# musket-ml/segmentation_training_pipeline

Hardware: AMD Instinct MI355X
Metric: images/sec U-Net/ResNet34 512x512 bs16 training step (higher is better)
Workload: dtype bf16; 1 GPU; U-Net/ResNet34 512x512x3 1-class, batch 16 per GPU, BCE+Dice, Adam, on-device augment S1 (BASELINE.json configs[1]); global_batch=16, parallelism=dp1, hipgraph=True

## Files before the change

### include/stp_hip.h

```cpp
#ifndef STP_HIP_H
#define STP_HIP_H

#include <stddef.h>
#include <stdint.h>

#ifdef __cplusplus
extern "C" {
#endif

#define STP_OK 0
#define STP_E_BADARG (-1)
#define STP_E_LAUNCH (-2)
#define STP_E_WORKSPACE (-3)

#define STP_F32 0
#define STP_BF16 1
#define STP_F16 3

#define STP_SRC_DIRECT 0
#define STP_SRC_NEAREST2X 1
#define STP_SRC_ZEROINS2X 2

int stp_abi_version(void);
int stp_storage_dtype(void);
// ... 3 lines not shown
  const void* src1;
  const void* weight;
  const float* bias;
  const void* residual;
  void* dst0;
  void* dst1;
  int32_t N, Hs0, Ws0, Hv, Wv, C0, C1;
  int32_t src0_mode;
  int32_t KH, KW, stride, pad;
  int32_t Ho, Wo, Cout, Cd0;
  int32_t accumulate0, accumulate1, relu;
  int32_t dtype;
  int32_t tile;
  int32_t stats_tiles;
  float* stats_partial;
  const void* bnb_x;
  const float* bnb_mean;
  const float* bnb_rstd;
  const float* bnb_gamma;
  const float* bnb_beta;
  int32_t bnb_relu;
  int32_t dst_sum2x2;
  int32_t stats_slots;
  const float* src_bn_mean;
  const float* src_bn_rstd;
  const float* src_bn_gamma;
  const float* src_bn_beta;
  int32_t src_bn_relu;
  const void* weight_up;
  const void* fold_src;
  const void* fold_weight;
  int32_t fold_C;
  float* stats_group_out;
  uint32_t* stats_group_counters;
  int32_t stats_group;
  int32_t s2d_dgrad;
} stp_conv_params;
int stp_conv2d_stats_group_for(const stp_conv_params* p);
size_t stp_conv2d_stats_group_counters(const stp_conv_params* p, int32_t G);
int stp_conv2d_fold_ok(const stp_conv_params* p);

int stp_conv2d(const stp_conv_params* p, void* stream);
int stp_weight_prepare_upcollapse(const float* master, void* weight_up, int32_t Cout, int32_t C0, int32_t C1, int32_t dtype,
                                  void* stream);
size_t stp_weight_prepare_upcollapse_desc_bytes(void);
int stp_weight_prepare_upcollapse_batched(const void* desc_dev, int32_t nlayers, int32_t dtype, void* stream);
int stp_weight_prepare_upcollapse_bwd_batched(const void* desc_dev, int32_t nlayers, int32_t dtype, void* stream);
size_t stp_conv2d_stats_floats(const stp_conv_params* p);
int stp_conv2d_tile_for(const stp_conv_params* p);
int stp_conv2d_sc_eligible(const stp_conv_params* p);
int stp_conv2d_sc_stats_tiles(const stp_conv_params* p);
int stp_conv2d_sc(const stp_conv_params* p, void* stream);
int stp_conv2d_scw_eligible(const stp_conv_params* p);
int stp_conv2d_scw_stats_tiles(const stp_conv_params* p);
int stp_conv2d_scw(const stp_conv_params* p, void* stream);
int stp_conv2d_scn_eligible(const stp_conv_params* p);
int stp_conv2d_scn_stats_tiles(const stp_conv_params* p);
int stp_conv2d_scn(const stp_conv_params* p, void* stream);
int stp_conv2d_s64_eligible(const stp_conv_params* p);
int stp_conv2d_s64_stats_tiles(const stp_conv_params* p);
int stp_conv2d_s64(const stp_conv_params* p, void* stream);
int stp_conv2d_stem_eligible(const stp_conv_params* p);
int stp_conv2d_stem(const stp_conv_params* p, void* stream);
int stp_conv2d_halo_variant(const stp_conv_params* p);
int stp_conv2d_halo_tiles(const stp_conv_params* p, int variant);
int stp_conv2d_halo(const stp_conv_params* p, int variant, void* stream);

typedef struct stp_wgrad_params {
  const void* src0;
  const void* src1;
  const void* dy;
  float* dw;
  int32_t N, Hs0, Ws0, Hv, Wv, C0, C1, src0_mode;
  int32_t KH, KW, stride, pad;
  int32_t Ho, Wo, Cout;
  int32_t accumulate;
  int32_t dtype;
  int32_t splits;
  const float* src_bn_mean;
  const float* src_bn_rstd;
  const float* src_bn_gamma;
  const float* src_bn_beta;
  int32_t src_bn_relu;
} stp_wgrad_params;

size_t stp_conv2d_wgrad_workspace_bytes(const stp_wgrad_params* p);
int stp_conv2d_wgrad(const stp_wgrad_params* p, void* workspace, size_t workspace_bytes, void* stream);
int stp_conv2d_wgrad_partial(const stp_wgrad_params* p, void* workspace, size_t workspace_bytes, int32_t variant, void* stream);
int stp_conv2d_wgrad_reduce(const stp_wgrad_params* p, const void* workspace, int32_t variant, void* stream);
int stp_wgrad_sc_eligible(const stp_wgrad_params* p);
int stp_wgrad_sc_slabs(const stp_wgrad_params* p);
int stp_wgrad_sc_partial(const stp_wgrad_params* p, void* workspace, void* stream);
int stp_conv2d_wgrad_kernel_id(const stp_wgrad_params* p);

int stp_wgrad_group_class(const stp_wgrad_params* p);
size_t stp_wgrad_group_table_bytes(const stp_wgrad_params* const* layers, int32_t n);
size_t stp_wgrad_group_workspace_bytes(const stp_wgrad_params* const* layers, int32_t n);
int stp_wgrad_group_build(const stp_wgrad_params* const* layers, int32_t n, void* host_table, size_t table_bytes);
int stp_wgrad_group_partial(const void* host_table, const void* dev_table, void* workspace, size_t workspace_bytes, void* stream);
int stp_wgrad_group_reduce(const void* host_table, const void* dev_table, const void* workspace, void* stream);

int stp_weight_prepare(const float* master, void* fwd, void* bwd, int32_t Cout, int32_t KH, int32_t KW,
                       int32_t Cin, int32_t KWp, int32_t Cinp, int32_t CoutB, int32_t dtype, void* stream);
size_t stp_weight_prepare_desc_bytes(void);
int64_t stp_weight_prepare_desc_fill(void* desc_host, int32_t index, int64_t start, const float* master, void* fwd, void* bwd,
                                     int32_t Cout, int32_t KH, int32_t KW, int32_t Cin, int32_t KWp, int32_t Cinp, int32_t CoutB);
int stp_weight_prepare_batched(const void* desc_dev, int32_t nlayers, int64_t total, int32_t dtype, void* stream);
int stp_weight_grad_unpad(const float* padded, float* grad, int32_t Cout, int32_t KH, int32_t KW,
                          int32_t Cin, int32_t KWp, int32_t Cinp, int32_t accumulate, void* stream);
int stp_stem_beta_grad(const float* padded_dw, const float* master, float* dbeta, int32_t Cout, int32_t KH,
                       int32_t KW, int32_t Cin, int32_t KWp, int32_t Cinp, int32_t one_ch, void* stream);

#define STP_U8 2
size_t stp_bn_workspace_bytes(int32_t C);
int stp_bn_apply_slots(const void* x, void* y, int32_t dtype, int64_t rows, int32_t C, const int64_t* slots, int32_t nslots,
                       float eps, float momentum, float* mean, float* rstd, float* moving_mean, float* moving_var,
                       const float* gamma, const float* beta, int32_t relu, void* stream);
int stp_bn_backward_slots(const void* x, const void* g, void* dx, int32_t dtype, int64_t rows, int32_t C, const float* mean,
                          const float* rstd, const float* gamma, const int64_t* slots, int32_t nslots, float* dgamma,
                          float* dbeta, int32_t accumulate_dx, void* stream);
int stp_zero_bytes(void* p, int64_t bytes, void* stream);
int stp_bn_backward_fused(const void* x, const void* g, void* dx, int32_t dtype, int64_t rows, int32_t C,
                          const float* mean, const float* rstd, const float* gamma, const float* partial, int32_t tiles,
                          float* dgamma, float* dbeta, int32_t accumulate_dx, void* workspace, size_t workspace_bytes,
                          void* stream);
int stp_bn_finalize_apply_ok(int32_t dtype, int64_t rows, int32_t C, int32_t tiles);
int stp_bn_finalize_apply(const float* partial, int32_t tiles, const void* x, void* y, int32_t dtype, int64_t rows, int32_t C,
                          float eps, float momentum, float* mean, float* rstd, float* moving_mean, float* moving_var,
                          const float* gamma, const float* beta, int32_t relu, void* stream);
int stp_bn_backward_fused_add(const void* x, const void* g, void* dx, const void* dadd, int32_t dtype, int64_t rows, int32_t C,
                              const float* mean, const float* rstd, const float* gamma, const float* partial, int32_t tiles,
                              float* dgamma, float* dbeta, int32_t accumulate_dx, void* workspace, size_t workspace_bytes,
                              void* stream);
int stp_bn_stats(const void* x, int32_t xdtype, int64_t rows, int32_t C, float eps, float momentum,
                 float* mean, float* rstd, float* moving_mean, float* moving_var,
                 void* workspace, size_t workspace_bytes, void* stream);
int stp_bn_finalize(const float* partial, int32_t tiles, int64_t rows, int32_t C, float eps, float momentum,
                    float* mean, float* rstd, float* moving_mean, float* moving_var, void* stream);
int stp_bn_apply(const void* x, int32_t xdtype, void* y, int32_t ydtype, int64_t rows, int32_t C, int32_t Cy,
                 const float* mean, const float* rstd, const float* gamma, const float* beta,
                 int32_t relu, float pad_value, void* stream);
int stp_bn_inference(const void* x, int32_t xdtype, void* y, int32_t ydtype, int64_t rows, int32_t C, int32_t Cy,
                     const float* moving_mean, const float* moving_var, float eps,
                     const float* gamma, const float* beta, int32_t relu, float pad_value, void* stream);
int stp_bn_backward(const void* x, const void* dy, void* dx, int32_t dtype, int64_t rows, int32_t C,
                    const float* mean, const float* rstd, const float* gamma, const float* beta,
                    float* dgamma, float* dbeta, int32_t relu, int32_t accumulate_dx,
                    void* workspace, size_t workspace_bytes, void* stream);

int stp_maxpool3x3s2(const void* x, void* y, uint8_t* idx, int32_t N, int32_t H, int32_t W, int32_t C,
                     int32_t dtype, void* stream);
int stp_maxpool3x3s2_bwd(const uint8_t* idx, const void* dy, void* dx, int32_t N, int32_t H, int32_t W, int32_t C,
                         int32_t dtype, int32_t accumulate, void* stream);
int stp_bn_apply_maxpool3x3s2(const void* x, void* yb, void* y, uint8_t* idx, int32_t N, int32_t H, int32_t W, int32_t C, int32_t dtype,
                              const float* mean, const float* rstd, const float* gamma, const float* beta, int32_t relu, void* stream);
int stp_maxpool3x3s2_bwd_bn_tiles(int32_t N, int32_t H, int32_t W, int32_t C, int32_t dtype);
int stp_maxpool3x3s2_bwd_bn(const uint8_t* idx, const void* dy, void* dx, int32_t N, int32_t H, int32_t W, int32_t C, int32_t dtype,
                            int32_t accumulate, const void* bn_x, const float* mean, const float* rstd, const float* gamma,
                            const float* beta, int32_t relu, float* partial, void* stream);
int stp_maxpool2x2(const void* x, void* y, uint8_t* idx, int32_t N, int32_t H, int32_t W, int32_t C, int32_t dtype, void* stream);
int stp_maxpool2x2_bwd(const uint8_t* idx, const void* dy, void* dx, int32_t N, int32_t H, int32_t W, int32_t C, int32_t dtype,
                       int32_t accumulate, void* stream);
size_t stp_avgpool_workspace_bytes(int32_t N, int32_t H, int32_t W, int32_t C, int32_t k);
int stp_avgpool(const void* x, void* y, int32_t N, int32_t H, int32_t W, int32_t C, int32_t k, int32_t dtype, void* workspace,
                size_t workspace_bytes, void* stream);
int stp_avgpool_bwd(const void* dy, void* dx, int32_t N, int32_t H, int32_t W, int32_t C, int32_t k, int32_t dtype,
                    int32_t accumulate, void* stream);
int stp_avgpool_pyramid_ok(int32_t N, int32_t H, int32_t W, int32_t C, int32_t k0, int32_t k1, int32_t k2, int32_t k3, int32_t dtype);
size_t stp_avgpool_pyramid_workspace_bytes(int32_t N, int32_t H, int32_t W, int32_t C, int32_t k0, int32_t dtype);
int stp_avgpool_pyramid(const void* x, void* y0, void* y1, void* y2, void* y3, int32_t k0, int32_t k1, int32_t k2, int32_t k3, int32_t N,
                        int32_t H, int32_t W, int32_t C, int32_t dtype, void* workspace, size_t workspace_bytes, void* stream);
int stp_avgpool_pyramid_bwd(const void* dy0, const void* dy1, const void* dy2, const void* dy3, int32_t k0, int32_t k1, int32_t k2, int32_t k3,
                            void* dx, int32_t N, int32_t H, int32_t W, int32_t C, int32_t dtype, int32_t accumulate, void* stream);
int stp_maxpool_k(const void* x, void* y, int32_t* idx, int32_t N, int32_t H, int32_t W, int32_t C, int32_t k, int32_t dtype, void* stream);
int stp_maxpool_k_bwd(const int32_t* idx, const void* dy, void* dx, int32_t N, int32_t H, int32_t W, int32_t C, int32_t k, int32_t dtype,
                      int32_t accumulate, void* stream);
int stp_relu_bwd(const void* y, void* dy, int64_t count, int32_t dtype, void* stream);

int stp_upsample2x_bwd(const void* dy, void* dx, int32_t N, int32_t H, int32_t W, int32_t C, int32_t ldy,
                       int32_t dtype, int32_t accumulate, void* stream);
int stp_tapsum_fwd(const void* z, void* y, const float* bias, int32_t N, int32_t H, int32_t W, int32_t Cout, int32_t Zc, int32_t Cy, int32_t dtype,
                   void* stream);
int stp_tapsum_bwd(const void* dy, void* dz, int32_t N, int32_t H, int32_t W, int32_t Cout, int32_t Cdy, int32_t Cdz, int32_t dtype, void* stream);
int stp_scatter2x_bwd(const void* t, void* dx, int32_t N, int32_t H, int32_t W, int32_t C, int32_t dtype, int32_t accumulate, void* stream);
int stp_scatter2x_bwd_bn_tiles(int32_t N, int32_t H, int32_t W, int32_t C, int32_t dtype);
int stp_scatter2x_bwd_bn(const void* t, void* dx, int32_t N, int32_t H, int32_t W, int32_t C, int32_t dtype, int32_t accumulate,
                         const void* bn_x, const float* mean, const float* rstd, const float* gamma, const float* beta, int32_t relu,
                         float* partial, void* stream);
int stp_upsample2x_bwd_bn_tiles(int32_t N, int32_t H, int32_t W, int32_t C, int32_t ldy, int32_t dtype);
int stp_upsample2x_bwd_bn(const void* dy, void* dx, int32_t N, int32_t H, int32_t W, int32_t C, int32_t ldy, int32_t dtype,
                          int32_t accumulate, const void* bn_x, const float* mean, const float* rstd, const float* gamma,
                          const float* beta, int32_t relu, float* partial, void* stream);
int stp_upsample2x_add(void* x, const void* m, int32_t N, int32_t H, int32_t W, int32_t C, int32_t dtype, void* stream);
int stp_resize_bilinear(const void* x, void* y, int32_t N, int32_t H, int32_t W, int32_t C, int32_t factor, int32_t ldo,
                        int32_t coff, int32_t dtype, void* stream);
size_t stp_resize_bilinear_bwd_workspace_bytes(int32_t N, int32_t H, int32_t W, int32_t C, int32_t factor);
int stp_resize_bilinear_bwd(const void* dy, void* dx, int32_t N, int32_t H, int32_t W, int32_t C, int32_t factor, int32_t ldo,
                            int32_t coff, int32_t dtype, int32_t accumulate, void* workspace, size_t workspace_bytes, void* stream);
int stp_resize_nearest(const void* x, void* y, int32_t N, int32_t H, int32_t W, int32_t C, int32_t factor, int32_t ldo, int32_t coff,
                       int32_t dtype, void* stream);
int stp_resize_nearest_bwd(const void* dy, void* dx, int32_t N, int32_t H, int32_t W, int32_t C, int32_t factor, int32_t ldo, int32_t coff,
                           int32_t dtype, int32_t accumulate, void* stream);

int stp_channel_sum(const void* x, int32_t dtype, int64_t rows, int32_t C, float* out, int32_t accumulate,
                    void* workspace, size_t workspace_bytes, void* stream);
int stp_add_inplace(void* dst, const void* src, int64_t count, int32_t dtype, void* stream);

size_t stp_loss_workspace_bytes(void);
int stp_sigmoid_bce_dice(const void* logits, const uint8_t* target, int64_t count, int32_t dtype,
                         float w_bce, float w_dice, float* scalars, void* dlogits, int32_t dl_channels,
                         float grad_scale, void* workspace, size_t workspace_bytes, void* stream);
int stp_sigmoid_loss_ex(const void* logits, const uint8_t* target, int64_t count, int32_t dtype, const float* weights5,
                        float* scalars, void* dlogits, int32_t dl_channels, float grad_scale, void* workspace,
                        size_t workspace_bytes, void* stream);
size_t stp_lovasz_workspace_bytes(int64_t count, int32_t images);
int stp_lovasz_hinge(const void* logits, const uint8_t* target, int32_t images, int64_t per_image, int32_t dtype, float weight,
                     float* scalars, void* dlogits, int32_t dl_channels, void* workspace, size_t workspace_bytes, void* stream);
int stp_sigmoid_loss_bias_grad(const void* workspace, int64_t count, float* dbias, int32_t accumulate, void* stream);
int stp_sigmoid(const void* logits, float* probs, int64_t count, int32_t dtype, void* stream);
int stp_sigmoid_multilabel_loss(const void* logits, const uint8_t* target, int64_t pixels, int32_t classes, int32_t ldc,
                                int32_t dtype, const float* weights5, float* scalars, void* dlogits, int32_t dl_channels,
                                float grad_scale, void* workspace, size_t workspace_bytes, void* stream);
int stp_sigmoid_multilabel_bias_grad(const void* workspace, int64_t pixels, int32_t classes, float* dbias, int32_t accumulate,
                                     void* stream);
int stp_softmax_cce_dice(const void* logits, const uint8_t* target, int64_t pixels, int32_t classes, int32_t ldc,
                         int32_t dtype, float w_cce, float w_dice, float* scalars, void* dlogits, int32_t dl_channels,
                         float grad_scale, void* workspace, size_t workspace_bytes, void* stream);
int stp_softmax_loss_ex(const void* logits, const uint8_t* target, int64_t pixels, int32_t classes, int32_t ldc,
                        int32_t dtype, const float* weights5, float* scalars, void* dlogits, int32_t dl_channels,
                        float grad_scale, void* workspace, size_t workspace_bytes, void* stream);
int stp_softmax_loss_masked(const void* logits, const uint8_t* target, int64_t pixels, int32_t classes, int32_t ldc,
// ... 188 lines not shown
```

### segmentation_training_pipeline_amd/_lib.py

```python
import ctypes as C
import os

HERE = os.path.dirname(os.path.abspath(__file__))
LIB_PATH = os.environ.get("STP_LIB") or os.path.join(HERE, "libstp_hip.so")

LIB_F16_PATH = os.environ.get("STP_LIB_F16") or os.path.join(HERE, "libstp_hip_f16.so")

F32, BF16, U8, F16 = 0, 1, 2, 3
SRC_DIRECT, SRC_NEAREST2X, SRC_ZEROINS2X = 0, 1, 2
LOVASZ_SOFTMAX_CHUNK = 4096

vp, i32, i64, f32, sz = C.c_void_p, C.c_int32, C.c_int64, C.c_float, C.c_size_t


class StpError(RuntimeError):
    pass


class ConvParams(C.Structure):
    _fields_ = [("src0", vp), ("src1", vp), ("weight", vp), ("bias", vp), ("residual", vp), ("dst0", vp), ("dst1", vp),
                ("N", i32), ("Hs0", i32), ("Ws0", i32), ("Hv", i32), ("Wv", i32), ("C0", i32), ("C1", i32),
                ("src0_mode", i32), ("KH", i32), ("KW", i32), ("stride", i32), ("pad", i32),
                ("Ho", i32), ("Wo", i32), ("Cout", i32), ("Cd0", i32),
                ("accumulate0", i32), ("accumulate1", i32), ("relu", i32), ("dtype", i32), ("tile", i32),
                ("stats_tiles", i32), ("stats_partial", vp),
                ("bnb_x", vp), ("bnb_mean", vp), ("bnb_rstd", vp), ("bnb_gamma", vp), ("bnb_beta", vp), ("bnb_relu", i32),
                ("dst_sum2x2", i32), ("stats_slots", i32),
                ("src_bn_mean", vp), ("src_bn_rstd", vp), ("src_bn_gamma", vp), ("src_bn_beta", vp), ("src_bn_relu", i32),
                ("weight_up", vp), ("fold_src", vp), ("fold_weight", vp), ("fold_C", i32),
                ("stats_group_out", vp), ("stats_group_counters", vp), ("stats_group", i32), ("s2d_dgrad", i32)]


class WgradParams(C.Structure):
    _fields_ = [("src0", vp), ("src1", vp), ("dy", vp), ("dw", vp),
                ("N", i32), ("Hs0", i32), ("Ws0", i32), ("Hv", i32), ("Wv", i32), ("C0", i32), ("C1", i32),
                ("src0_mode", i32), ("KH", i32), ("KW", i32), ("stride", i32), ("pad", i32),
                ("Ho", i32), ("Wo", i32), ("Cout", i32), ("accumulate", i32), ("dtype", i32), ("splits", i32),
                ("src_bn_mean", vp), ("src_bn_rstd", vp), ("src_bn_gamma", vp), ("src_bn_beta", vp), ("src_bn_relu", i32)]


SIGNATURES = {
    "stp_abi_version": (i32, []),
    "stp_storage_dtype": (i32, []),
    "stp_conv2d": (i32, [C.POINTER(ConvParams), vp]),
    "stp_weight_prepare_upcollapse": (i32, [vp, vp, i32, i32, i32, i32, vp]),
    "stp_weight_prepare_upcollapse_desc_bytes": (sz, []),
    "stp_weight_prepare_upcollapse_batched": (i32, [vp, i32, i32, vp]),
    "stp_weight_prepare_upcollapse_bwd_batched": (i32, [vp, i32, i32, vp]),
    "stp_conv2d_fold_ok": (i32, [C.POINTER(ConvParams)]),
    "stp_conv2d_stats_floats": (sz, [C.POINTER(ConvParams)]),
    "stp_conv2d_stats_group_for": (i32, [C.POINTER(ConvParams)]),
    "stp_conv2d_stats_group_counters": (sz, [C.POINTER(ConvParams), i32]),
    "stp_conv2d_tile_for": (i32, [C.POINTER(ConvParams)]),
    "stp_conv2d_sc_eligible": (i32, [C.POINTER(ConvParams)]),
    "stp_conv2d_sc": (i32, [C.POINTER(ConvParams), vp]),
    "stp_conv2d_sc_stats_tiles": (i32, [C.POINTER(ConvParams)]),
    "stp_conv2d_scw": (i32, [C.POINTER(ConvParams), vp]),
    "stp_conv2d_scw_eligible": (i32, [C.POINTER(ConvParams)]),
    "stp_conv2d_scw_stats_tiles": (i32, [C.POINTER(ConvParams)]),
    "stp_conv2d_scn": (i32, [C.POINTER(ConvParams), vp]),
    "stp_conv2d_scn_eligible": (i32, [C.POINTER(ConvParams)]),
    "stp_conv2d_scn_stats_tiles": (i32, [C.POINTER(ConvParams)]),
    "stp_conv2d_s64": (i32, [C.POINTER(ConvParams), vp]),
    "stp_conv2d_s64_eligible": (i32, [C.POINTER(ConvParams)]),
    "stp_conv2d_s64_stats_tiles": (i32, [C.POINTER(ConvParams)]),
    "stp_conv2d_pw_eligible": (i32, [C.POINTER(ConvParams)]),
    "stp_conv2d_pw_cols": (i32, [C.POINTER(ConvParams)]),
    "stp_conv2d_pw": (i32, [C.POINTER(ConvParams), vp]),
    "stp_conv2d_stem_eligible": (i32, [C.POINTER(ConvParams)]),
    "stp_conv2d_stem": (i32, [C.POINTER(ConvParams), vp]),
    "stp_conv2d_halo_variant": (i32, [C.POINTER(ConvParams)]),
    "stp_conv2d_halo_tiles": (i32, [C.POINTER(ConvParams), i32]),
    "stp_conv2d_halo": (i32, [C.POINTER(ConvParams), i32, vp]),
    "stp_conv2d_wgrad_workspace_bytes": (sz, [C.POINTER(WgradParams)]),
    "stp_conv2d_wgrad": (i32, [C.POINTER(WgradParams), vp, sz, vp]),
    "stp_conv2d_wgrad_partial": (i32, [C.POINTER(WgradParams), vp, sz, i32, vp]),
    "stp_conv2d_wgrad_reduce": (i32, [C.POINTER(WgradParams), vp, i32, vp]),
    "stp_wgrad_reduce_desc_bytes": (sz, []),
    "stp_wgrad_reduce_desc_fill": (i64, [vp, i32, C.POINTER(WgradParams), vp]),
    "stp_wgrad_reduce_batched": (i32, [vp, i32, i64, vp]),
    "stp_wgrad_sc_eligible": (i32, [C.POINTER(WgradParams)]),
    "stp_wgrad_sc_slabs": (i32, [C.POINTER(WgradParams)]),
    "stp_wgrad_sc_partial": (i32, [C.POINTER(WgradParams), vp, vp]),
    "stp_conv2d_wgrad_kernel_id": (i32, [C.POINTER(WgradParams)]),
    "stp_wgrad_group_class": (i32, [C.POINTER(WgradParams)]),
    "stp_wgrad_group_table_bytes": (sz, [vp, i32]),
    "stp_wgrad_group_workspace_bytes": (sz, [vp, i32]),
    "stp_wgrad_group_build": (i32, [vp, i32, vp, sz]),
    "stp_wgrad_group_partial": (i32, [vp, vp, vp, sz, vp]),
    "stp_wgrad_group_reduce": (i32, [vp, vp, vp, vp]),
    "stp_weight_prepare": (i32, [vp, vp, vp, i32, i32, i32, i32, i32, i32, i32, i32, vp]),
    "stp_weight_prepare_desc_bytes": (sz, []),
    "stp_weight_prepare_desc_fill": (i64, [vp, i32, i64, vp, vp, vp, i32, i32, i32, i32, i32, i32, i32]),
    "stp_weight_prepare_batched": (i32, [vp, i32, i64, i32, vp]),
    "stp_weight_grad_unpad": (i32, [vp, vp, i32, i32, i32, i32, i32, i32, i32, vp]),
    "stp_stem_beta_grad": (i32, [vp, vp, vp, i32, i32, i32, i32, i32, i32, i32, vp]),
    "stp_bn_workspace_bytes": (sz, [i32]),
    "stp_bn_stats": (i32, [vp, i32, i64, i32, f32, f32, vp, vp, vp, vp, vp, sz, vp]),
    "stp_bn_finalize": (i32, [vp, i32, i64, i32, f32, f32, vp, vp, vp, vp, vp]),
    "stp_bn_apply": (i32, [vp, i32, vp, i32, i64, i32, i32, vp, vp, vp, vp, i32, f32, vp]),
    "stp_bn_inference": (i32, [vp, i32, vp, i32, i64, i32, i32, vp, vp, f32, vp, vp, i32, f32, vp]),
    "stp_bn_backward": (i32, [vp, vp, vp, i32, i64, i32, vp, vp, vp, vp, vp, vp, i32, i32, vp, sz, vp]),
    "stp_bn_apply_slots": (i32, [vp, vp, i32, i64, i32, vp, i32, f32, f32, vp, vp, vp, vp, vp, vp, i32, vp]),
    "stp_bn_backward_slots": (i32, [vp, vp, vp, i32, i64, i32, vp, vp, vp, vp, i32, vp, vp, i32, vp]),
    "stp_zero_bytes": (i32, [vp, i64, vp]),
    "stp_bn_backward_fused": (i32, [vp, vp, vp, i32, i64, i32, vp, vp, vp, vp, i32, vp, vp, i32, vp, sz, vp]),
    "stp_bn_finalize_apply_ok": (i32, [i32, i64, i32, i32]),
    "stp_bn_finalize_apply": (i32, [vp, i32, vp, vp, i32, i64, i32, f32, f32, vp, vp, vp, vp, vp, vp, i32, vp]),
    "stp_bn_backward_fused_add": (i32, [vp, vp, vp, vp, i32, i64, i32, vp, vp, vp, vp, i32, vp, vp, i32, vp, sz, vp]),
    "stp_maxpool3x3s2": (i32, [vp, vp, vp, i32, i32, i32, i32, i32, vp]),
    "stp_maxpool3x3s2_bwd": (i32, [vp, vp, vp, i32, i32, i32, i32, i32, i32, vp]),
    "stp_bn_apply_maxpool3x3s2": (i32, [vp, vp, vp, vp, i32, i32, i32, i32, i32, vp, vp, vp, vp, i32, vp]),
    "stp_maxpool3x3s2_bwd_bn_tiles": (i32, [i32, i32, i32, i32, i32]),
    "stp_maxpool3x3s2_bwd_bn": (i32, [vp, vp, vp, i32, i32, i32, i32, i32, i32, vp, vp, vp, vp, vp, i32, vp, vp]),
    "stp_maxpool2x2": (i32, [vp, vp, vp, i32, i32, i32, i32, i32, vp]),
    "stp_maxpool2x2_bwd": (i32, [vp, vp, vp, i32, i32, i32, i32, i32, i32, vp]),
    "stp_avgpool_workspace_bytes": (sz, [i32, i32, i32, i32, i32]),
    "stp_avgpool": (i32, [vp, vp, i32, i32, i32, i32, i32, i32, vp, sz, vp]),
    "stp_avgpool_bwd": (i32, [vp, vp, i32, i32, i32, i32, i32, i32, i32, vp]),
    "stp_avgpool_pyramid_ok": (i32, [i32, i32, i32, i32, i32, i32, i32, i32, i32]),
    "stp_avgpool_pyramid_workspace_bytes": (sz, [i32, i32, i32, i32, i32, i32]),
    "stp_avgpool_pyramid": (i32, [vp, vp, vp, vp, vp, i32, i32, i32, i32, i32, i32, i32, i32, i32, vp, sz, vp]),
    "stp_avgpool_pyramid_bwd": (i32, [vp, vp, vp, vp, i32, i32, i32, i32, vp, i32, i32, i32, i32, i32, i32, vp]),
    "stp_maxpool_k": (i32, [vp, vp, vp, i32, i32, i32, i32, i32, i32, vp]),
    "stp_maxpool_k_bwd": (i32, [vp, vp, vp, i32, i32, i32, i32, i32, i32, i32, vp]),
    "stp_relu_bwd": (i32, [vp, vp, i64, i32, vp]),
    "stp_upsample2x_bwd": (i32, [vp, vp, i32, i32, i32, i32, i32, i32, i32, vp]),
    "stp_tapsum_fwd": (i32, [vp, vp, vp, i32, i32, i32, i32, i32, i32, i32, vp]),
    "stp_tapsum_bwd": (i32, [vp, vp, i32, i32, i32, i32, i32, i32, i32, vp]),
    "stp_scatter2x_bwd": (i32, [vp, vp, i32, i32, i32, i32, i32, i32, vp]),
    "stp_scatter2x_bwd_bn_tiles": (i32, [i32, i32, i32, i32, i32]),
    "stp_scatter2x_bwd_bn": (i32, [vp, vp, i32, i32, i32, i32, i32, i32, vp, vp, vp, vp, vp, i32, vp, vp]),
    "stp_upsample2x_bwd_bn_tiles": (i32, [i32, i32, i32, i32, i32, i32]),
    "stp_upsample2x_bwd_bn": (i32, [vp, vp, i32, i32, i32, i32, i32, i32, i32, vp, vp, vp, vp, vp, i32, vp, vp]),
    "stp_upsample2x_add": (i32, [vp, vp, i32, i32, i32, i32, i32, vp]),
    "stp_resize_bilinear": (i32, [vp, vp, i32, i32, i32, i32, i32, i32, i32, i32, vp]),
    "stp_upsample_sum": (i32, [vp, vp, vp, vp, i32, i32, i32, i32, vp, i32, i32, i32, i32, i32, vp]),
    "stp_copy_cols_f32": (i32, [vp, i32, vp, i32, i32, i32, i32, vp]),
    "stp_resize_bilinear_bwd_workspace_bytes": (sz, [i32, i32, i32, i32, i32]),
    "stp_resize_bilinear_bwd": (i32, [vp, vp, i32, i32, i32, i32, i32, i32, i32, i32, i32, vp, sz, vp]),
    "stp_resize_nearest": (i32, [vp, vp, i32, i32, i32, i32, i32, i32, i32, i32, vp]),
    "stp_resize_nearest_bwd": (i32, [vp, vp, i32, i32, i32, i32, i32, i32, i32, i32, i32, vp]),
    "stp_channel_sum": (i32, [vp, i32, i64, i32, vp, i32, vp, sz, vp]),
    "stp_add_inplace": (i32, [vp, vp, i64, i32, vp]),
    "stp_loss_workspace_bytes": (sz, []),
    "stp_sigmoid_bce_dice": (i32, [vp, vp, i64, i32, f32, f32, vp, vp, i32, f32, vp, sz, vp]),
    "stp_sigmoid_loss_ex": (i32, [vp, vp, i64, i32, vp, vp, vp, i32, f32, vp, sz, vp]),
    "stp_sigmoid_loss_bias_grad": (i32, [vp, i64, vp, i32, vp]),
    "stp_sigmoid_multilabel_loss": (i32, [vp, vp, i64, i32, i32, i32, vp, vp, vp, i32, f32, vp, sz, vp]),
    "stp_sigmoid_multilabel_bias_grad": (i32, [vp, i64, i32, vp, i32, vp]),
    "stp_softmax_loss_ex": (i32, [vp, vp, i64, i32, i32, i32, vp, vp, vp, i32, f32, vp, sz, vp]),
    "stp_softmax_loss_masked": (i32, [vp, vp, i64, i32, i32, i32, vp, vp, vp, i32, f32, vp, sz, i32, vp, vp]),
    "stp_lovasz_workspace_bytes": (sz, [i64, i32]),
    "stp_lovasz_hinge": (i32, [vp, vp, i32, i64, i32, f32, vp, vp, i32, vp, sz, vp]),
    "stp_lovasz_softmax_workspace_bytes": (sz, [i64, i32]),
    "stp_lovasz_softmax": (i32, [vp, vp, i64, i32, i32, i32, f32, vp, vp, i32, f32, i32, vp, sz, vp]),
    "stp_sigmoid": (i32, [vp, vp, i64, i32, vp]),
    "stp_softmax_cce_dice": (i32, [vp, vp, i64, i32, i32, i32, f32, f32, vp, vp, i32, f32, vp, sz, vp]),
    "stp_softmax_cce_dice_up_ok": (i32, [i32, i32, i32]),
    "stp_softmax_cce_dice_up_corner_bytes": (sz, [i32, i32, i32, i32]),
    "stp_softmax_cce_dice_up": (i32, [vp, vp, i32, i32, i32, i32, i32, i32, i32, f32, f32, vp, vp, i32, f32, vp, vp, vp, sz, vp, sz, vp]),
    "stp_softmax": (i32, [vp, vp, i64, i32, i32, i32, vp]),
    "stp_class_confusion_workspace_bytes": (sz, [i32]),
    "stp_class_confusion": (i32, [vp, vp, i64, i32, i32, i32, vp, vp, sz, vp]),
    "stp_class_confusion_ignore": (i32, [vp, vp, i64, i32, i32, i32, vp, vp, sz, i32, vp]),
    "stp_class_confusion_up_ok": (i32, [i32, i32, i32]),
    "stp_class_confusion_up": (i32, [vp, vp, i32, i32, i32, i32, i32, i32, i32, vp, vp, sz, vp]),
    "stp_adam": (i32, [vp, vp, vp, vp, i64, vp, f32, f32, f32, vp, vp, vp, f32, vp]),
    "stp_sgd": (i32, [vp, vp, vp, i64, vp, f32, i32, vp, vp, f32, vp]),
    "stp_rmsprop": (i32, [vp, vp, vp, i64, vp, f32, f32, vp, vp, f32, vp]),
    "stp_nadam": (i32, [vp, vp, vp, vp, i64, vp, f32, f32, f32, f32, vp, vp, vp, vp, f32, vp]),
    "stp_grad_global_scale": (i32, [vp, i64, f32, f32, vp, vp, sz, vp]),
    "stp_scale_by_device": (i32, [vp, i64, i32, vp, vp, vp]),
    "stp_grad_global_scale_dls": (i32, [vp, i64, f32, f32, vp, vp, vp, sz, vp]),
    "stp_dwconv": (i32, [vp, vp, vp, i32, i32, i32, i32, i32, i32, i32, i32, i32, i32, i32, i32, vp]),
    "stp_dwconv_dgrad": (i32, [vp, vp, vp, i32, i32, i32, i32, i32, i32, i32, i32, i32, i32, i32, i32, i32, vp]),
    "stp_dwconv_wgrad_workspace_bytes": (sz, [i32, i32]),
    "stp_dwconv_wgrad": (i32, [vp, vp, vp, i32, i32, i32, i32, i32, i32, i32, i32, i32, i32, i32, i32, i32, vp, sz, vp]),
    "stp_resize_bilinear_ac": (i32, [vp, vp, i32, i32, i32, i32, i32, i32, i32, vp]),
    "stp_resize_bilinear_ac_bwd": (i32, [vp, vp, i32, i32, i32, i32, i32, i32, i32, i32, vp]),
    "stp_counter_tick": (i32, [vp, vp]),
    "stp_dropout": (i32, [vp, vp, i64, f32, vp, C.c_uint32, i32, vp]),
    "stp_dropout_spatial": (i32, [vp, vp, i32, i64, i32, f32, vp, C.c_uint32, i32, vp]),
    "stp_sigmoid_act": (i32, [vp, vp, i64, i32, i32, i32, i32, vp]),
    "stp_sigmoid_act_bwd": (i32, [vp, vp, vp, i64, i32, i32, i32, i32, vp]),
# ... 113 lines not shown
```

### segmentation_training_pipeline_amd/csrc/bn.hip

```cpp
#include "stream_ops.h"
#include <cstdlib>

__global__ __launch_bounds__(256) void bn_partial_u8_kernel(const uint8_t* __restrict__ x, int64_t rows, int C, float* partial) {
  __shared__ float rs[256 * 2];
  const int rowLanes = 256 / C;
  const int tcol = threadIdx.x % C, trow = threadIdx.x / C;
  const int64_t rowsPerBlock = (rows + gridDim.x - 1) / gridDim.x;
  const int64_t r0 = (int64_t)blockIdx.x * rowsPerBlock;
  const int64_t r1 = r0 + rowsPerBlock < rows ? r0 + rowsPerBlock : rows;
  float s = 0.f, q = 0.f;
  if (trow < rowLanes)
    for (int64_t r = r0 + trow; r < r1; r += rowLanes) {
      const float v = (float)x[r * C + tcol];
      s += v;
      q += v * v;
    }
  rs[threadIdx.x * 2] = s;
  rs[threadIdx.x * 2 + 1] = q;
  __syncthreads();
  if (trow == 0 && threadIdx.x < C) {
    float a = 0.f, b = 0.f;
    for (int t = 0; t < rowLanes; ++t) { a += rs[(t * C + tcol) * 2]; b += rs[(t * C + tcol) * 2 + 1]; }
    partial[(size_t)blockIdx.x * 2 * C + tcol] = a;
    partial[(size_t)blockIdx.x * 2 * C + C + tcol] = b;
// ... 526 lines not shown
  __syncthreads();
  const int cg = C / V;
  const int64_t total = rows * cg;
  const int64_t stride = (int64_t)gridDim.x * 256;
  if (stride % cg == 0) {
    const int c = (int)(((int64_t)blockIdx.x * 256 + threadIdx.x) % cg) * V;
    float mu[V], rs[V], sc[V], sh[V], k1[V], k2[V];
#pragma unroll
    for (int e = 0; e < V; ++e) {
      mu[e] = ss[c + e]; rs[e] = ss[C + c + e]; sc[e] = ss[2 * C + c + e]; sh[e] = ss[3 * C + c + e];
      k1[e] = ss[4 * C + c + e]; k2[e] = ss[5 * C + c + e];
    }
    auto one = [&](int64_t i, const float (&xv)[V], float (&g)[V], const float (&d)[V]) {
      float o[V];
#pragma unroll
      for (int e = 0; e < V; ++e) {
        if (!bn_act_on(bn_affine(xv[e], sc[e], sh[e]), relu)) g[e] = 0.f;
        const float xh = (xv[e] - mu[e]) * rs[e];
        o[e] = sc[e] * (g[e] - k1[e] - xh * k2[e]);
        if (accumulate) o[e] += d[e];
      }
      stv<T, V>(dx + i * V, o);
    };
    int64_t i = (int64_t)blockIdx.x * 256 + threadIdx.x;
    for (; i + stride < total; i += 2 * stride) {
      float x0[V], g0[V], d0[V], x1[V], g1[V], d1[V];
      ldv<T, V>(x + i * V, x0);
      ldv<T, V>(x + (i + stride) * V, x1);
      ldv<T, V>(dy + i * V, g0);
      ldv<T, V>(dy + (i + stride) * V, g1);
      if (accumulate) { ldv<T, V>(dadd + i * V, d0); ldv<T, V>(dadd + (i + stride) * V, d1); }
      one(i, x0, g0, d0);
      one(i + stride, x1, g1, d1);
    }
    for (; i < total; i += stride) {
      float x0[V], g0[V], d0[V];
      ldv<T, V>(x + i * V, x0);
      ldv<T, V>(dy + i * V, g0);
      if (accumulate) ldv<T, V>(dadd + i * V, d0);
      one(i, x0, g0, d0);
    }
    return;
  }
  for (int64_t i = (int64_t)blockIdx.x * 256 + threadIdx.x; i < total; i += stride) {
    const int c = (int)(i % cg) * V;
    float xv[V], g[V], o[V];
    ldv<T, V>(x + i * V, xv);
    ldv<T, V>(dy + i * V, g);
#pragma unroll
    for (int e = 0; e < V; ++e) {
      if (!bn_act_on(bn_affine(xv[e], ss[2 * C + c + e], ss[3 * C + c + e]), relu)) g[e] = 0.f;
      const float xh = (xv[e] - ss[c + e]) * ss[C + c + e];
      o[e] = ss[2 * C + c + e] * (g[e] - ss[4 * C + c + e] - xh * ss[5 * C + c + e]);
    }
    if (accumulate) {
      float d[V];
      ldv<T, V>(dadd + i * V, d);
#pragma unroll
      for (int e = 0; e < V; ++e) o[e] += d[e];
    }
    stv<T, V>(dx + i * V, o);
  }
}

static int bn_bwd_apply_launch(const void* x, const void* dy, void* dx, int dtype, int64_t rows, int C, const float* mean, const float* rstd,
                               const float* gamma, const float* beta, const float* sums, int relu, int accumulate, const long long* slots, int nslots,
                               float* dgamma, float* dbeta, const void* dadd, hipStream_t s) {
  const bool v8 = dtype == STP_H16 && (C & 7) == 0;
  const size_t lds2 = 6 * (size_t)C * sizeof(float);
  const int g = grid_fixed_channels(grid_for_amortised(rows * (C / (v8 ? 8 : 4)), 8), C / (v8 ? 8 : 4));
  const float inv_rows = (float)(1.0 / (double)rows);
  return launch_tv(dtype, v8, [&](auto tv) {
    using T = typename decltype(tv)::T; constexpr int V = decltype(tv)::V;
    hipLaunchKernelGGL((bn_bwd_apply_kernel<T, V>), dim3(g), dim3(256), lds2, s, (const T*)x, (const T*)dy, (T*)dx, rows, C, mean, rstd, gamma, beta,
                       sums, inv_rows, relu, accumulate, slots, nslots, dgamma, dbeta, (const T*)dadd);
  });
}

extern "C" int stp_bn_backward(const void* x, const void* dy, void* dx, int32_t dtype, int64_t rows, int32_t C,
                               const float* mean, const float* rstd, const float* gamma, const float* beta, float* dgamma,
                               float* dbeta, int32_t relu, int32_t accumulate_dx, void* workspace, size_t workspace_bytes,
                               void* stream) {
  if (!stp_dtype_ok(dtype)) return STP_E_BADARG;
  if (!x || !dy || !dx || !mean || !rstd || !workspace || rows <= 0 || C <= 0 || (C & 3)) return STP_E_BADARG;
  if (workspace_bytes < stp_bn_workspace_bytes(C)) return STP_E_WORKSPACE;
  hipStream_t s = (hipStream_t)stream;
  const int blocks = bn_blocks(rows) > BN_MAX_BLOCKS - 1 ? BN_MAX_BLOCKS - 1 : bn_blocks(rows);
  float* partial = (float*)workspace;
  float* sums = partial + (size_t)(BN_MAX_BLOCKS - 1) * 2 * C;
  const int rc = launch_tv(dtype, dtype == STP_H16 && (C & 7) == 0, [&](auto tv) {
    using T = typename decltype(tv)::T; constexpr int V = decltype(tv)::V;
    hipLaunchKernelGGL((bn_bwd_partial_kernel<T, V>), dim3(blocks), dim3(256), 256 * 2 * V * sizeof(float), s, (const T*)x, (const T*)dy, rows, C,
                       mean, rstd, gamma, beta, relu, partial);
  });
  if (rc) return rc;
  hipLaunchKernelGGL(bn_bwd_finalize_kernel, dim3(ceil_div(C, 4)), dim3(256), 0, s, partial, blocks, C, sums, dgamma, dbeta);
  STP_LAUNCH_CHECK();
  return bn_bwd_apply_launch(x, dy, dx, dtype, rows, C, mean, rstd, gamma, beta, sums, relu, accumulate_dx, nullptr, 0, nullptr, nullptr, nullptr, s);
}

#define BNF_SLAB 64
static bool bn_fused_ok(int dtype, int64_t rows, int C, int tiles) {
  static const bool on = !(getenv("STP_BN_FUSE_FINALIZE") && atoi(getenv("STP_BN_FUSE_FINALIZE")) == 0);
  static const int maxcols = getenv("STP_BN_FUSE_MAXCOLS") ? atoi(getenv("STP_BN_FUSE_MAXCOLS")) : 128;
  return on && dtype == STP_H16 && (C % BNF_SLAB) == 0 && tiles >= 1 && tiles <= maxcols && rows >= 64;
}
static int bn_fused_chunks(int64_t rows, int C) {
  const int slabs = C / BNF_SLAB;
  int64_t want = (rows + 255) / 256;
  const int64_t lo = (2 * 256 + slabs - 1) / slabs;
  if (want < lo) want = lo;
  const int64_t hi = (rows + 31) / 32;
  if (want > hi) want = hi;
  return (int)(want < 1 ? 1 : want);
}

__device__ __forceinline__ void bnf_slab_sums(const float* __restrict__ partial, int tiles, int C, int c0, double& s, double& q) {
  const int cl = threadIdx.x >> 2, j = threadIdx.x & 3;
  const float* ps = partial + (size_t)(c0 + cl) * tiles;
  const float* pq = partial + ((size_t)C + c0 + cl) * tiles;
  s = 0.0; q = 0.0;
  if ((tiles & 3) == 0 && tiles > 128 && tiles <= 256) {
#pragma unroll
    for (int h = 0; h < 2; ++h) {
      f32x4 a[8], b[8];
#pragma unroll
      for (int u = 0; u < 8; ++u) {
        const int t = 4 * j + 16 * (u + 8 * h);
        a[u] = b[u] = f32x4{0.f, 0.f, 0.f, 0.f};
        if (t < tiles) { a[u] = *reinterpret_cast<const f32x4*>(ps + t); b[u] = *reinterpret_cast<const f32x4*>(pq + t); }
      }
#pragma unroll
      for (int u = 0; u < 8; ++u)
        if (4 * j + 16 * (u + 8 * h) < tiles) {
          s += ((double)a[u].x + (double)a[u].y) + ((double)a[u].z + (double)a[u].w);
          q += ((double)b[u].x + (double)b[u].y) + ((double)b[u].z + (double)b[u].w);
        }
    }
  } else if ((tiles & 3) == 0 && tiles <= 128) {
    f32x4 a[8], b[8];
#pragma unroll
    for (int u = 0; u < 8; ++u) {
      const int t = 4 * j + 16 * u;
      a[u] = b[u] = f32x4{0.f, 0.f, 0.f, 0.f};
      if (t < tiles) { a[u] = *reinterpret_cast<const f32x4*>(ps + t); b[u] = *reinterpret_cast<const f32x4*>(pq + t); }
    }
#pragma unroll
    for (int u = 0; u < 8; ++u)
      if (4 * j + 16 * u < tiles) {
        s += ((double)a[u].x + (double)a[u].y) + ((double)a[u].z + (double)a[u].w);
        q += ((double)b[u].x + (double)b[u].y) + ((double)b[u].z + (double)b[u].w);
      }
  } else if ((tiles & 3) == 0) {
    for (int t = 4 * j; t < tiles; t += 16) {
      const f32x4 a = *reinterpret_cast<const f32x4*>(ps + t), b = *reinterpret_cast<const f32x4*>(pq + t);
      s += ((double)a.x + (double)a.y) + ((double)a.z + (double)a.w);
      q += ((double)b.x + (double)b.y) + ((double)b.z + (double)b.w);
    }
  } else {
    for (int t = j; t < tiles; t += 4) { s += (double)ps[t]; q += (double)pq[t]; }
  }
  s += __shfl_xor(s, 1, 64); q += __shfl_xor(q, 1, 64);
  s += __shfl_xor(s, 2, 64); q += __shfl_xor(q, 2, 64);
}

__global__ __launch_bounds__(256) void bn_finalize_apply_kernel(const float* __restrict__ partial, int tiles, const bf16_t* __restrict__ x,
                                                                bf16_t* __restrict__ y, int64_t rows, int C, int chunks, double inv_rows,
                                                                double unbias, float eps, float momentum, float* mean, float* rstd,
                                                                float* mm, float* mv, const float* gamma, const float* beta, int relu) {
  __shared__ float tab[2][BNF_SLAB];
  const int slab = blockIdx.x / chunks, chunk = blockIdx.x - slab * chunks, c0 = slab * BNF_SLAB;
  const int cg = threadIdx.x & 7, r0 = threadIdx.x >> 3;
  const int64_t per = (rows + chunks - 1) / chunks, ra = (int64_t)chunk * per, rb = ra + per < rows ? ra + per : rows;
  const size_t col = (size_t)c0 + cg * 8;
  int64_t r = ra + r0;
  const bool pre = r + 96 < rb;
  u32x4 p0 = {0u, 0u, 0u, 0u}, p1 = p0, p2 = p0, p3 = p0;
  if (pre) {
    p0 = *reinterpret_cast<const u32x4*>(x + (size_t)r * C + col); p1 = *reinterpret_cast<const u32x4*>(x + (size_t)(r + 32) * C + col);
    p2 = *reinterpret_cast<const u32x4*>(x + (size_t)(r + 64) * C + col); p3 = *reinterpret_cast<const u32x4*>(x + (size_t)(r + 96) * C + col);
  }
// ... 211 lines not shown
```

### segmentation_training_pipeline_amd/csrc/conv_sc.h

```cpp
#pragma once
#include "common.h"
#include "launch.h"
#include <cstdlib>
#include <type_traits>
#include <utility>

struct ScArgs {
  const char* src;
  const char* weight;
  const float* bias;
  char* dst;
  int N, H, W, Hs, Ws, Cout, up, accumulate, relu;
  int tiles_x, tiles_y;
  FastDiv divTx, divTy;
  float* stats;
  int stat_slots;
  BnBack bnb;
  int sum2;
  uint32_t src_bytes;
  BnBack pbn;
};

template <typename T> struct ScStageBn;
template <> struct ScStageBn<float> {
// ... 6 lines not shown
    u32x4 o;
#pragma unroll
    for (int e = 0; e < 4; ++e) o[e] = __float_as_uint(bn_act(bn_affine(__uint_as_float(r[e]), sc[e], sh[e]), relu));
    return o;
  }
};
template <> struct ScStageBn<bf16_t> {
  f32x2 sc[4], sh[4];
  __device__ __forceinline__ void load(const BnBack& b, int c) {
    const BnBackCh k0 = bnback_load(b, c), k1 = bnback_load(b, c + 4);
    sc[0] = f32x2{k0.sc[0], k0.sc[1]}; sc[1] = f32x2{k0.sc[2], k0.sc[3]}; sc[2] = f32x2{k1.sc[0], k1.sc[1]}; sc[3] = f32x2{k1.sc[2], k1.sc[3]};
    sh[0] = f32x2{k0.sh[0], k0.sh[1]}; sh[1] = f32x2{k0.sh[2], k0.sh[3]}; sh[2] = f32x2{k1.sh[0], k1.sh[1]}; sh[3] = f32x2{k1.sh[2], k1.sh[3]};
  }
  __device__ __forceinline__ void load_tab(const float* tsc, const float* tsh, int c) {
#pragma unroll
    for (int e = 0; e < 4; ++e) { sc[e] = *reinterpret_cast<const f32x2*>(tsc + c + 2 * e); sh[e] = *reinterpret_cast<const f32x2*>(tsh + c + 2 * e); }
  }
  __device__ __forceinline__ u32x4 apply(const u32x4& r, int relu) const {
    u32x4 o;
#pragma unroll
    for (int e = 0; e < 4; ++e) {
      f32x2 v = {h16lo_to_f32(r[e]), h16hi_to_f32(r[e])};
      v = __builtin_elementwise_fma(v, sc[e], sh[e]);
      o[e] = pack_bf16x2(bn_act(v.x, relu), bn_act(v.y, relu));
    }
    return o;
  }
};


constexpr int SC_TH = 8, SC_TW = 32, SC_HW = SC_TW + 2, SC_HH = SC_TH + 2;

template <int... Ks, typename F>
__device__ __forceinline__ void sc_unroll_seq(std::integer_sequence<int, Ks...>, F&& f) { (f(std::integral_constant<int, Ks>{}), ...); }
template <int N, typename F>
__device__ __forceinline__ void sc_unroll(F&& f) { sc_unroll_seq(std::make_integer_sequence<int, N>{}, f); }
#ifndef SC_RING
#define SC_RING 8
#endif

#ifndef SC_WPE_SMALL
#define SC_WPE_SMALL 4
#endif

static inline bool sc_stream_on() {
  static const bool on = !(getenv("STP_SC_STREAM") && atoi(getenv("STP_SC_STREAM")) == 0);
  return on;
}
static inline int sc_stream_blocks(int dtype, int cin, int cout, int ntiles) {
  const int per_cu = cout <= 16 ? (dtype == STP_H16 && cin <= 16 ? SC_WPE_SMALL : 3) : 2;
  const int64_t b = (int64_t)stp_cu_count() * per_cu;
  return (int)(b < ntiles ? b : ntiles);
}


struct ScWgArgs {
  const char* src;
  const char* dy;
  float* slabs;
  int N, H, W, Hs, Ws, Cout, up;
  int tiles_x, tiles_y, ntiles;
  int ctot, coff;
  uint32_t src_bytes, dy_bytes;
  BnBack pbn;
};

constexpr int ST_HH = (SC_TH - 1) * 2 + 7, ST_HW = 70, ST_WROW = 464, ST_HALO = ST_HH * ST_HW * 8, ST_WBYTES = 64 * ST_WROW;

struct StemArgs {
  const char* src;
  const char* weight;
  char* dst;
  int N, H, W, Ho, Wo, tiles_x, tiles_y;
  FastDiv divTx, divTy;
  float* stats;
  uint32_t src_bytes;
};

bool stem_lean_serves(int N, int H, int W);
int stem_lean_blocks(int ntiles);
int stem_lean_launch(const StemArgs& a, hipStream_t s);
bool stem_wg_lean_serves(int N, int H, int W, int Ho, int Wo);
int stem_wg_lean_blocks(int N, int Ho, int Wo);
int stem_wg_lean_launch(const void* src, const void* dy, float* slabs, int N, int H, int W, int Ho, int Wo, hipStream_t s);

int sc_lean_launch(const ScArgs& a, int cin, int dtype, hipStream_t s);
int sc_wg_lean_launch(const ScWgArgs& a, int cin, int cout, int dtype, int blocks, hipStream_t s);
```

### segmentation_training_pipeline_amd/csrc/conv_sc_lean.hip

```cpp
#include "conv_sc.h"

enum { SCL_STATS = 0, SCL_BNB = 1, SCL_BNB_SUM2 = 2, SCL_HEAD = 3 };

struct TileC { int n, y0, x0; bool interior; };

__device__ __forceinline__ f32x2 scl_unpack(uint32_t w) { return f32x2{h16lo_to_f32(w), h16hi_to_f32(w)}; }

template <int TM>
__device__ __forceinline__ void scl_store(char* p, const u32x2 (&o)[TM]) {
  if constexpr (TM == 2) *reinterpret_cast<u32x4*>(p) = u32x4{o[0].x, o[0].y, o[1].x, o[1].y};
  else *reinterpret_cast<u32x2*>(p) = o[0];
}

template <int CIN, int TM, int EPI, bool PBN, bool UP>
__global__ __launch_bounds__(256, (TM == 1 ? (CIN <= 16 ? SC_WPE_SMALL : 3) : 2)) void conv_sc_lean_kernel(const ScArgs a) {
  typedef bf16_t T;
  constexpr int SZ = 2, VEC = 8, KC = 32, K = 9 * CIN, NCH = (K + KC - 1) / KC, VPP = CIN / VEC, PIXB = CIN * SZ;
  constexpr int HH = UP ? SC_TH / 2 + 2 : SC_HH, HW = UP ? SC_TW / 2 + 2 : SC_HW;
  constexpr int NV = HH * HW * VPP, NPASS = (NV + 255) / 256, BUF = NPASS * 4096;
  constexpr bool PART = (K % KC) != 0;
  constexpr int COUT = EPI == SCL_HEAD ? 1 : TM * 16;
  constexpr int CB = COUT * SZ;
  static_assert(EPI != SCL_HEAD || TM == 1, "head: one output channel");
  static_assert(!PBN || EPI == SCL_STATS || EPI == SCL_HEAD, "producer BatchNormalization: forward only");
// ... 768 lines not shown
        for (int f = 0; f < 4; ++f) { asm volatile("" : "+v"(fb[c & 1][f][0])); asm volatile("" : "+v"(fb[c & 1][f][1])); }
#pragma unroll
        for (int f = 0; f < 4; ++f) {
          const u32x4 vb = {fb[c & 1][f][0].x, fb[c & 1][f][0].y, fb[c & 1][f][1].x, fb[c & 1][f][1].y};
#pragma unroll
          for (int i = 0; i < TM; ++i) acc[i][f] = mfma16_16x16x32(fa[c & 1][i], vb, acc[i][f]);
        }
      });
      ba += cur ? (uint32_t)(-STL_BUF) : (uint32_t)STL_BUF;

#if defined(STP_STEM_WAIT_LATE)
      __builtin_amdgcn_s_waitcnt(0x0f70);
      asm volatile("" ::: "memory");
#endif
      char* ob = a.dst + (((size_t)t.n * a.Ho + t.y0) * a.Wo + t.x0) * (COUT * 2);
      const bool st = a.stats != nullptr;
      auto epilogue = [&](const bool EDGE) __attribute__((always_inline)) {
#pragma unroll
        for (int f = 0; f < 4; ++f) {
          char* of = ob + (size_t)(((f >> 1) * a.Wo + (f & 1) * 16) * (COUT * 2));
          const bool ok = !EDGE || (t.y0 + wave * 2 + (f >> 1) < a.Ho && t.x0 + (f & 1) * 16 + lr < a.Wo);
#pragma unroll
          for (int h = 0; h < 2; ++h) {
            const f32x4 v0 = acc[2 * h][f], v1 = acc[2 * h + 1][f];
            const u32x4 o = {pack_bf16x2(v0.x, v0.y), pack_bf16x2(v0.z, v0.w), pack_bf16x2(v1.x, v1.y), pack_bf16x2(v1.z, v1.w)};
            if (ok) {
              *reinterpret_cast<u32x4*>(of + so + h * 64) = o;
              if (st) {
#pragma unroll
                for (int u = 0; u < 2; ++u) {
                  const f32x2 s0 = scl_unpack(o[2 * u]), s1 = scl_unpack(o[2 * u + 1]);
                  const f32x4 sv = {s0.x, s0.y, s1.x, s1.y};
                  ss[2 * h + u] += sv;
                  qq[2 * h + u] += sv * sv;
                }
              }
            }
          }
        }
      };
      if (t.interior) epilogue(false); else epilogue(true);
    }
  }
  if (a.stats) {
    __builtin_amdgcn_s_waitcnt(0x0f70);
#pragma unroll
    for (int i = 0; i < TM; ++i)
#pragma unroll
      for (int e = 0; e < 4; ++e) {
        const float sv = row_sum16_to_lane15(ss[i][e]), qv = row_sum16_to_lane15(qq[i][e]);
        if (lr == 15) {
          const int cl = (i >> 1) * 32 + lg * 8 + (i & 1) * 4 + e;
          red[(wave * COUT + cl) * 2] = sv;
          red[(wave * COUT + cl) * 2 + 1] = qv;
        }
      }
    lds_barrier();
    if (tid < COUT) {
      float sv = 0.f, qv = 0.f;
#pragma unroll
      for (int w = 0; w < 4; ++w) { sv += red[(w * COUT + tid) * 2]; qv += red[(w * COUT + tid) * 2 + 1]; }
      a.stats[(size_t)tid * gridDim.x + blockIdx.x] = sv;
      a.stats[((size_t)COUT + tid) * gridDim.x + blockIdx.x] = qv;
    }
  }
}

bool stem_lean_serves(int N, int H, int W) {
  static const bool on = !(getenv("STP_STEM_LEAN") && atoi(getenv("STP_STEM_LEAN")) == 0);
  return on && !(W & 1) && (uint64_t)N * H * W * 8 < 0x80000000ull;
}
int stem_lean_blocks(int ntiles) {
  const int64_t b = (int64_t)stp_cu_count() * 2;
  return (int)(b < ntiles ? b : ntiles);
}
int stem_lean_launch(const StemArgs& a, hipStream_t s) {
  if (!stem_lean_serves(a.N, a.H, a.W) || !a.src_bytes) return 1;
  return stp_launch_lds(conv_stem_lean_kernel, dim3(stem_lean_blocks(a.N * a.tiles_x * a.tiles_y)), dim3(256), STL_LDS, s, a);
}

constexpr int SWG_TH = 4, SWG_PH = 2 * (SWG_TH - 1) + 7;
constexpr int SWG_NVX = SWG_PH * STL_VPR, SWG_NPX = (SWG_NVX + 255) / 256;
constexpr int SWG_NVD = SWG_TH * SC_TW * 8, SWG_NPD = (SWG_NVD + 255) / 256;
constexpr int SWG_XBUF = SWG_NPX * 4096, SWG_BUF = SWG_XBUF + SWG_NPD * 4096;

struct StemWgArgs {
  const char* src;
  const char* dy;
  float* slabs;
  int N, H, W, Ho, Wo, tiles_x, tiles_y, ntiles;
  uint32_t src_bytes, dy_bytes;
};

__global__ __launch_bounds__(256, 2) void conv_stem_wgrad_lean_kernel(const StemWgArgs a) {
  constexpr int COUT = 64, K = 224, NF = 14;
  extern __shared__ __attribute__((aligned(16))) char smem[];
  const int tid = threadIdx.x, lane = tid & 63;
  const int wave = __builtin_amdgcn_readfirstlane(tid >> 6);
  const int lr = lane & 15, lg = lane >> 4;

  int t_first, t_step, t_end;
  if ((gridDim.x & 7) == 0) {
    const int q = a.ntiles >> 3, r = a.ntiles & 7, x = blockIdx.x & 7;
    const int start = x < r ? x * (q + 1) : r * (q + 1) + (x - r) * q;
    t_first = start + (int)(blockIdx.x >> 3); t_step = (int)(gridDim.x >> 3); t_end = start + q + (x < r ? 1 : 0);
  } else {
    t_first = (int)blockIdx.x; t_step = (int)gridDim.x; t_end = a.ntiles;
  }
  f32x4 acc[NF];
#pragma unroll
  for (int f = 0; f < NF; ++f) acc[f] = f32x4{0.f, 0.f, 0.f, 0.f};

  if (t_first < t_end) {
    const __amdgpu_buffer_rsrc_t rsx = __builtin_amdgcn_make_buffer_rsrc((void*)a.src, 0, a.src_bytes, 0x00020000);
    const __amdgpu_buffer_rsrc_t rsd = __builtin_amdgcn_make_buffer_rsrc((void*)a.dy, 0, a.dy_bytes, 0x00020000);
    int hyx[SWG_NPX], pyx[SWG_NPD];
    uint32_t lox[SWG_NPX], lod[SWG_NPD];
#pragma unroll
    for (int p = 0; p < SWG_NPX; ++p) {
      const int v = p * 256 + tid, hy = v / STL_VPR, vx = v - hy * STL_VPR;
      hyx[p] = v < SWG_NVX ? (hy << 16 | vx) : -1;
      lox[p] = v < SWG_NVX ? (uint32_t)((hy * a.W + 2 * vx) * 8) : 0x80000000u;
    }
#pragma unroll
    for (int p = 0; p < SWG_NPD; ++p) {
      const int v = p * 256 + tid, pix = v >> 3, py = pix / SC_TW, px = pix % SC_TW;
      pyx[p] = v < SWG_NVD ? (py << 16 | px) : -1;
      lod[p] = v < SWG_NVD ? (uint32_t)((py * a.Wo + px) * (COUT * 2) + (v & 7) * 16) : 0x80000000u;
    }
    const uint32_t cvd = (uint32_t)(tid & 7) * 16u;
    auto decode = [&](int tile) -> TileC {
      int b = tile;
      const int tx = b % a.tiles_x; b /= a.tiles_x;
      const int ty = b % a.tiles_y;
      TileC t;
      t.n = b / a.tiles_y; t.y0 = ty * SWG_TH; t.x0 = tx * SC_TW;
      t.interior = 2 * t.y0 >= 3 && 2 * t.x0 >= 4 && 2 * t.y0 - 3 + SWG_PH <= a.H && 2 * t.x0 + 65 < a.W && t.y0 + SWG_TH <= a.Ho && t.x0 + SC_TW <= a.Wo;
      return t;
    };
    auto issue_tile = [&](const TileC& t, int bsel, bool live) {
      char* xb = smem + bsel * SWG_BUF;
      if (live && t.interior) {
        const uint32_t tbx = (uint32_t)(((t.n * a.H + 2 * t.y0 - 3) * a.W + 2 * t.x0 - 4) * 8);
        const uint32_t tbd = (uint32_t)(((t.n * a.Ho + t.y0) * a.Wo + t.x0) * (COUT * 2));
#pragma unroll
        for (int p = 0; p < SWG_NPX; ++p)
          __builtin_amdgcn_raw_ptr_buffer_load_lds(rsx, (__attribute__((address_space(3))) void*)(xb + p * 4096 + wave * 1024), 16, (int)(tbx + lox[p]), 0, 0, 0);
#pragma unroll
        for (int p = 0; p < SWG_NPD; ++p)
          __builtin_amdgcn_raw_ptr_buffer_load_lds(rsd, (__attribute__((address_space(3))) void*)(xb + SWG_XBUF + p * 4096 + wave * 1024), 16, (int)(tbd + lod[p]), 0, 0, 0);
      } else {
#pragma unroll
        for (int p = 0; p < SWG_NPX; ++p) {
          const int gy = 2 * t.y0 - 3 + (hyx[p] >> 16), gx = 2 * t.x0 - 4 + 2 * (hyx[p] & 0xffff);
          const bool ok = live && hyx[p] >= 0 && (unsigned)gy < (unsigned)a.H && (unsigned)gx < (unsigned)a.W;
          const uint32_t off = ok ? (uint32_t)(((t.n * a.H + gy) * a.W + gx) * 8) : 0x80000000u;
          __builtin_amdgcn_raw_ptr_buffer_load_lds(rsx, (__attribute__((address_space(3))) void*)(xb + p * 4096 + wave * 1024), 16, (int)off, 0, 0, 0);
        }
#pragma unroll
        for (int p = 0; p < SWG_NPD; ++p) {
          const int gy = t.y0 + (pyx[p] >> 16), gx = t.x0 + (pyx[p] & 0xffff);
          const bool ok = live && pyx[p] >= 0 && gy < a.Ho && gx < a.Wo;
          const uint32_t off = ok ? (uint32_t)(((t.n * a.Ho + gy) * a.Wo + gx) * (COUT * 2)) + cvd : 0x80000000u;
          __builtin_amdgcn_raw_ptr_buffer_load_lds(rsd, (__attribute__((address_space(3))) void*)(xb + SWG_XBUF + p * 4096 + wave * 1024), 16, (int)off, 0, 0, 0);
        }
      }
    };
    TileC tc = decode(t_first);
    issue_tile(tc, 0, true);
    const int xl = lg * 4 + (lr >> 2), qd = lr & 3;
    uint32_t aA = (uint32_t)(uintptr_t)smem + (uint32_t)(SWG_XBUF + (xl * COUT + wave * 16) * 2 + qd * 8);
    uint32_t aB = (uint32_t)(uintptr_t)smem + (uint32_t)((2 * xl + 1 + qd) * 8);

    int cur = 0;
    for (int tile = t_first; tile < t_end; tile += t_step, cur ^= 1) {
      __builtin_amdgcn_s_waitcnt(0x0f70);
      asm volatile("" ::: "memory");
      lds_barrier();
      const int next = tile + t_step;
      const bool live = next < t_end;
      if (live) tc = decode(next);
      issue_tile(tc, cur ^ 1, live);

      u32x2 fa[SWG_TH][2];
      u32x2 fb[2][2][2];
      sc_unroll<SWG_TH * 2>([&fa, aA](auto kc) {
        constexpr int k = decltype(kc)::value, r = k >> 1, hl = k & 1;
        asm volatile("ds_read_b64_tr_b16 %0, %1 offset:%2" : "=v"(fa[r][hl]) : "v"(aA), "n"((r * SC_TW + hl * 16) * COUT * 2));
      });
      auto issue_b = [&fb, aB](auto rc) {
        constexpr int pr = decltype(rc)::value;
        sc_unroll<4>([&fb, aB](auto kc) {
          constexpr int k = decltype(kc)::value, kwh = k >> 1, hl = k & 1;
          asm volatile("ds_read_b64_tr_b16 %0, %1 offset:%2" : "=v"(fb[pr & 1][kwh][hl]) : "v"(aB), "n"(pr * STL_ROW + kwh * 32 + hl * 32 * 8));
        });
      };
      issue_b(std::integral_constant<int, 0>{});
      sc_unroll<SWG_PH>([&](auto rc) {
        constexpr int pr = decltype(rc)::value;
        if constexpr (pr + 1 < SWG_PH) issue_b(std::integral_constant<int, pr + 1>{});
        asm volatile("s_waitcnt lgkmcnt(%0)" ::"n"(pr + 1 < SWG_PH ? 4 : 0) : "memory");
        if constexpr (pr == 0) {
#pragma unroll
          for (int r = 0; r < SWG_TH; ++r) { asm volatile("" : "+v"(fa[r][0])); asm volatile("" : "+v"(fa[r][1])); }
        }
#pragma unroll
        for (int kwh = 0; kwh < 2; ++kwh) { asm volatile("" : "+v"(fb[pr & 1][kwh][0])); asm volatile("" : "+v"(fb[pr & 1][kwh][1])); }
#pragma unroll
        for (int r = 0; r < SWG_TH; ++r) {
          const int kh = pr - 2 * r;
          if (kh < 0 || kh > 6) continue;
          const u32x4 va = {fa[r][0].x, fa[r][0].y, fa[r][1].x, fa[r][1].y};
#pragma unroll
          for (int kwh = 0; kwh < 2; ++kwh) {
            const u32x4 vb = {fb[pr & 1][kwh][0].x, fb[pr & 1][kwh][0].y, fb[pr & 1][kwh][1].x, fb[pr & 1][kwh][1].y};
            acc[kh * 2 + kwh] = mfma16_16x16x32(va, vb, acc[kh * 2 + kwh]);
          }
        }
      });
      const uint32_t flip = cur ? (uint32_t)(-SWG_BUF) : (uint32_t)SWG_BUF;
      aA += flip; aB += flip;
    }
  }
  float* out = a.slabs + (size_t)blockIdx.x * COUT * K;
#pragma unroll
  for (int f = 0; f < NF; ++f)
#pragma unroll
    for (int r = 0; r < 4; ++r) out[(size_t)(wave * 16 + lg * 4 + r) * K + (f >> 1) * 32 + (f & 1) * 16 + lr] = acc[f][r];
}

bool stem_wg_lean_serves(int N, int H, int W, int Ho, int Wo) {
  static const bool on = !(getenv("STP_STEM_WG_LEAN") && atoi(getenv("STP_STEM_WG_LEAN")) == 0);
  return on && !(W & 1) && (uint64_t)N * H * W * 8 < 0x80000000ull && (uint64_t)N * Ho * Wo * 128 < 0x80000000ull;
}
int stem_wg_lean_blocks(int N, int Ho, int Wo) {
  const int64_t tiles = (int64_t)N * ((Ho + SWG_TH - 1) / SWG_TH) * ((Wo + SC_TW - 1) / SC_TW), b = (int64_t)stp_cu_count() * 2;
  return (int)(b < tiles ? b : tiles);
}
int stem_wg_lean_launch(const void* src, const void* dy, float* slabs, int N, int H, int W, int Ho, int Wo, hipStream_t s) {
  StemWgArgs a;
  a.src = (const char*)src; a.dy = (const char*)dy; a.slabs = slabs;
  a.N = N; a.H = H; a.W = W; a.Ho = Ho; a.Wo = Wo;
  a.tiles_x = (Wo + SC_TW - 1) / SC_TW; a.tiles_y = (Ho + SWG_TH - 1) / SWG_TH; a.ntiles = N * a.tiles_x * a.tiles_y;
  a.src_bytes = (uint32_t)((uint64_t)N * H * W * 8); a.dy_bytes = (uint32_t)((uint64_t)N * Ho * Wo * 128);
  hipLaunchKernelGGL(conv_stem_wgrad_lean_kernel, dim3(stem_wg_lean_blocks(N, Ho, Wo)), dim3(256), 2 * SWG_BUF, s, a);
  STP_LAUNCH_CHECK();
  return STP_OK;
}
```

### segmentation_training_pipeline_amd/csrc/conv_sc_wgrad.hip

```cpp
#include "conv_sc.h"

typedef short s16x4_t __attribute__((ext_vector_type(4)));


template <typename T, int CIN, int COUT>
__global__ __launch_bounds__(256) void conv_sc_wgrad_stream_kernel(const ScWgArgs a) {
  constexpr int SZ = (int)sizeof(T);
  constexpr int VEC = Elem<T>::VEC;
  constexpr int TMo = (COUT + 15) / 16, TNi = CIN / 16;
  constexpr int PIXB = CIN * SZ, DYB = COUT * SZ;
  constexpr int HALO_BYTES = SC_HH * SC_HW * PIXB;
  static_assert(CIN % 16 == 0 && COUT % VEC == 0, "channel granularity");

  extern __shared__ __attribute__((aligned(16))) char smem[];
  const int tid = threadIdx.x, lane = tid & 63;
  const int wave = __builtin_amdgcn_readfirstlane(tid >> 6);
  const int lr = lane & 15, lg = lane >> 4;
  const int sh = a.up ? 1 : 0;

  static_assert(256 % (CIN / VEC) == 0, "a thread stages the same channel vector in every pass");
  const bool pbn = a.pbn.mean != nullptr;
  ScStageBn<T> sbn;
  if (pbn) sbn.load(a.pbn, (tid % (CIN / VEC)) * VEC);

// ... 209 lines not shown
    __syncthreads();

#pragma unroll 1
    for (int row = 0; row < SC_TH; ++row) {
      if constexpr (sizeof(T) == 2) {
        const int xl = lg * 4 + (lr >> 2), qb = (lr & 3) * 8;
        u32x4 fa[TMo];
#pragma unroll
        for (int i = 0; i < TMo; ++i) {
          const char* p = dyt + ((row * SC_TW + xl) * COUT + i * 16) * SZ + qb;
          const s16x4_t lo = __builtin_amdgcn_ds_read_tr16_b64_v4i16((__attribute__((address_space(3))) s16x4_t*)p);
          const s16x4_t hi = __builtin_amdgcn_ds_read_tr16_b64_v4i16((__attribute__((address_space(3))) s16x4_t*)(p + 16 * DYB));
          const u32x2 l2 = __builtin_bit_cast(u32x2, lo), h2 = __builtin_bit_cast(u32x2, hi);
          fa[i] = u32x4{l2.x, l2.y, h2.x, h2.y};
        }
#pragma unroll
        for (int t = 0; t < 3; ++t) {
          const int tap = wave + 4 * t;
          if (tap < 9) {
            const int kh = tap / 3, kw = tap - kh * 3;
#pragma unroll
            for (int j = 0; j < TNi; ++j) {
              const char* p = halo + (((row + kh) * SC_HW + xl + kw) * CIN + j * 16) * SZ + qb;
              const s16x4_t lo = __builtin_amdgcn_ds_read_tr16_b64_v4i16((__attribute__((address_space(3))) s16x4_t*)p);
              const s16x4_t hi = __builtin_amdgcn_ds_read_tr16_b64_v4i16((__attribute__((address_space(3))) s16x4_t*)(p + 16 * PIXB));
              const u32x2 l2 = __builtin_bit_cast(u32x2, lo), h2 = __builtin_bit_cast(u32x2, hi);
              const u32x4 fb = u32x4{l2.x, l2.y, h2.x, h2.y};
#pragma unroll
              for (int i = 0; i < TMo; ++i)
                acc[t][i][j] = mfma16_16x16x32(fa[i], fb, acc[t][i][j]);
            }
          }
        }
      } else {
#pragma unroll
        for (int s = 0; s < 8; ++s) {
          const int x = s * 4 + lg;
          float fa[TMo];
#pragma unroll
          for (int i = 0; i < TMo; ++i) fa[i] = *reinterpret_cast<const float*>(dyt + ((row * SC_TW + x) * COUT + i * 16 + lr) * SZ);
#pragma unroll
          for (int t = 0; t < 3; ++t) {
            const int tap = wave + 4 * t;
            if (tap < 9) {
              const int kh = tap / 3, kw = tap - kh * 3;
#pragma unroll
              for (int j = 0; j < TNi; ++j) {
                const float fb = *reinterpret_cast<const float*>(halo + (((row + kh) * SC_HW + x + kw) * CIN + j * 16 + lr) * SZ);
#pragma unroll
                for (int i = 0; i < TMo; ++i) acc[t][i][j] = __builtin_amdgcn_mfma_f32_16x16x4f32(fa[i], fb, acc[t][i][j], 0, 0, 0);
              }
            }
          }
        }
      }
    }
  }

  float* out = a.slabs + (size_t)blockIdx.x * a.Cout * (9 * a.ctot);
#pragma unroll
  for (int t = 0; t < 3; ++t) {
    const int tap = wave + 4 * t;
    if (tap >= 9) continue;
#pragma unroll
    for (int i = 0; i < TMo; ++i)
#pragma unroll
      for (int j = 0; j < TNi; ++j)
#pragma unroll
        for (int r = 0; r < 4; ++r) {
          const int co = i * 16 + lg * 4 + r;
          if (co < a.Cout) out[(size_t)co * (9 * a.ctot) + tap * a.ctot + a.coff + j * 16 + lr] = acc[t][i][j][r];
        }
  }
}

#define SC_WG_MAX_BLOCKS 1024

static bool wgrad_stem_shape(const stp_wgrad_params* p) {
  return p->dtype == STP_H16 && p->C0 == 4 && p->C1 == 0 && p->KH == 7 && p->KW == 8 && p->stride == 2 && p->pad == 3 && p->Cout == 64 &&
         p->src0_mode == STP_SRC_DIRECT && p->Hs0 == p->Hv && p->Ws0 == p->Wv && p->Ho == (p->Hv - 1) / 2 + 1 && p->Wo == (p->Wv - 1) / 2 + 1 &&
         !p->src_bn_mean && stem_wg_lean_serves(p->N, p->Hv, p->Wv, p->Ho, p->Wo);
}

extern "C" int stp_wgrad_sc_eligible(const stp_wgrad_params* p) {
  if (!p || !stp_dtype_ok(p->dtype)) return 0;
  if (wgrad_stem_shape(p)) return 1;
  const int vec = p->dtype == STP_H16 ? 8 : 4;
  const bool c0ok = p->C0 == 16 || p->C0 == 32 || (p->C0 == 64 && vec == 8);
  const bool c1ok = p->C1 == 0 || p->C1 == 16 || p->C1 == 32 || (p->C1 == 64 && vec == 8);
  return p->KH == 3 && p->KW == 3 && p->stride == 1 && p->pad == 1 && c0ok && c1ok &&
         (p->Cout == 8 || p->Cout == 16 || p->Cout == 32 || (p->Cout == 4 && vec == 4)) && (p->Cout % vec) == 0 &&
         p->Ho == p->Hv && p->Wo == p->Wv &&
         (p->src0_mode == STP_SRC_DIRECT || (p->src0_mode == STP_SRC_NEAREST2X && p->Hv == 2 * p->Hs0 && p->Wv == 2 * p->Ws0));
}

extern "C" int stp_wgrad_sc_slabs(const stp_wgrad_params* p) {
  if (wgrad_stem_shape(p)) return stem_wg_lean_blocks(p->N, p->Ho, p->Wo);
  const int64_t tiles = (int64_t)p->N * ceil_div(p->Hv, SC_TH) * ceil_div(p->Wv, SC_TW);
  static const int max_blocks = getenv("STP_SC_WG_BLOCKS") ? atoi(getenv("STP_SC_WG_BLOCKS")) : SC_WG_MAX_BLOCKS;
  const int vec = p->dtype == STP_H16 ? 8 : 4, cin = p->C0 > p->C1 ? p->C0 : p->C1;
  const int64_t npx = ((int64_t)SC_HH * SC_HW * (cin / vec) + 255) / 256, npd = ((int64_t)SC_TH * SC_TW * ((p->Cout + vec - 1) / vec) + 255) / 256;
  const int64_t lds = 2 * (npx + npd) * 4096;
  int per_cu = (int)((160 * 1024) / (lds > 0 ? lds : 1));
  per_cu = per_cu < 1 ? 1 : per_cu > 4 ? 4 : per_cu;
  int64_t blocks = (int64_t)stp_cu_count() * per_cu;
  if (blocks > max_blocks) blocks = max_blocks;
  return (int)(tiles < blocks ? tiles : blocks);
}

template <typename T, int CIN, int COUT>
static int launch_sc_wg(const ScWgArgs& a, int blocks, hipStream_t s) {
  if (sc_stream_on() && a.src_bytes && a.dy_bytes) {
    constexpr int VEC = Elem<T>::VEC;
    constexpr int NPX = (SC_HH * SC_HW * (CIN / VEC) + 255) / 256, NPD = (SC_TH * SC_TW * (COUT / VEC) + 255) / 256;
    const size_t lds = (size_t)2 * (NPX + NPD) * 4096;
    return stp_launch_lds(conv_sc_wgrad_stream_kernel<T, CIN, COUT>, dim3(blocks), dim3(256), lds, s, a);
  }
  const size_t lds = (size_t)SC_HH * SC_HW * CIN * sizeof(T) + (size_t)SC_TH * SC_TW * COUT * sizeof(T) + 64;
  hipLaunchKernelGGL((conv_sc_wgrad_kernel<T, CIN, COUT>), dim3(blocks), dim3(256), lds, s, a);
  STP_LAUNCH_CHECK();
  return STP_OK;
}

template <typename T>
static int sc_wg_dispatch(const ScWgArgs& a, int cin, int cout, int blocks, hipStream_t s) {
  {
    const int r = sc_wg_lean_launch(a, cin, cout, Elem<T>::DTYPE, blocks, s);
    if (r != 1) return r;
  }
  const int key = cin * 64 + cout;
  if constexpr (sizeof(T) == 2) {
    switch (key) {
      case 16 * 64 + 8: return launch_sc_wg<T, 16, 8>(a, blocks, s);
      case 16 * 64 + 16: return launch_sc_wg<T, 16, 16>(a, blocks, s);
      case 16 * 64 + 32: return launch_sc_wg<T, 16, 32>(a, blocks, s);
      case 32 * 64 + 8: return launch_sc_wg<T, 32, 8>(a, blocks, s);
      case 32 * 64 + 16: return launch_sc_wg<T, 32, 16>(a, blocks, s);
      case 32 * 64 + 32: return launch_sc_wg<T, 32, 32>(a, blocks, s);
      case 64 * 64 + 8: return launch_sc_wg<T, 64, 8>(a, blocks, s);
      case 64 * 64 + 16: return launch_sc_wg<T, 64, 16>(a, blocks, s);
      case 64 * 64 + 32: return launch_sc_wg<T, 64, 32>(a, blocks, s);
      default: return STP_E_BADARG;
    }
  } else {
    switch (key) {
      case 16 * 64 + 4: return launch_sc_wg<T, 16, 4>(a, blocks, s);
      case 16 * 64 + 8: return launch_sc_wg<T, 16, 8>(a, blocks, s);
      case 16 * 64 + 16: return launch_sc_wg<T, 16, 16>(a, blocks, s);
      case 16 * 64 + 32: return launch_sc_wg<T, 16, 32>(a, blocks, s);
      case 32 * 64 + 4: return launch_sc_wg<T, 32, 4>(a, blocks, s);
      case 32 * 64 + 8: return launch_sc_wg<T, 32, 8>(a, blocks, s);
      case 32 * 64 + 16: return launch_sc_wg<T, 32, 16>(a, blocks, s);
      case 32 * 64 + 32: return launch_sc_wg<T, 32, 32>(a, blocks, s);
      default: return STP_E_BADARG;
    }
  }
}

extern "C" int stp_wgrad_sc_partial(const stp_wgrad_params* p, void* workspace, void* stream) {
  if (!stp_wgrad_sc_eligible(p) || !p->src0 || !p->dy || !workspace || (p->C1 > 0 && !p->src1)) return STP_E_BADARG;
  if (wgrad_stem_shape(p)) return stem_wg_lean_launch(p->src0, p->dy, (float*)workspace, p->N, p->Hv, p->Wv, p->Ho, p->Wo, (hipStream_t)stream);
  ScWgArgs a;
  a.dy = (const char*)p->dy; a.slabs = (float*)workspace;
  a.N = p->N; a.H = p->Hv; a.W = p->Wv; a.Cout = p->Cout;
  a.tiles_x = ceil_div(a.W, SC_TW); a.tiles_y = ceil_div(a.H, SC_TH); a.ntiles = a.N * a.tiles_x * a.tiles_y;
  a.ctot = p->C0 + p->C1;
  a.pbn.x = nullptr; a.pbn.mean = p->src_bn_mean; a.pbn.rstd = p->src_bn_rstd; a.pbn.gamma = p->src_bn_gamma; a.pbn.beta = p->src_bn_beta;
  a.pbn.relu = p->src_bn_relu;
  if (a.pbn.mean && (!a.pbn.rstd || p->C1 > 0)) return STP_E_BADARG;
  const int blocks = stp_wgrad_sc_slabs(p);
  hipStream_t s = (hipStream_t)stream;
  const uint64_t szb = p->dtype == STP_H16 ? 2 : 4, lim = 0x80000000ull;
  const uint64_t dyb = (uint64_t)p->N * p->Hv * p->Wv * p->Cout * szb, b0 = (uint64_t)p->N * p->Hs0 * p->Ws0 * p->C0 * szb;
  const uint64_t b1 = (uint64_t)p->N * p->Hv * p->Wv * p->C1 * szb;
  a.dy_bytes = dyb < lim ? (uint32_t)dyb : 0u;
  a.src_bytes = b0 < lim ? (uint32_t)b0 : 0u;
  a.src = (const char*)p->src0; a.Hs = p->Hs0; a.Ws = p->Ws0; a.up = p->src0_mode == STP_SRC_NEAREST2X; a.coff = 0;
  int rc = p->dtype == STP_H16 ? sc_wg_dispatch<bf16_t>(a, p->C0, p->Cout, blocks, s) : sc_wg_dispatch<float>(a, p->C0, p->Cout, blocks, s);
  if (rc != STP_OK || p->C1 == 0) return rc;
  a.pbn.mean = nullptr;
  a.src = (const char*)p->src1; a.Hs = p->Hv; a.Ws = p->Wv; a.up = 0; a.coff = p->C0;
  a.src_bytes = b1 < lim ? (uint32_t)b1 : 0u;
  return p->dtype == STP_H16 ? sc_wg_dispatch<bf16_t>(a, p->C1, p->Cout, blocks, s) : sc_wg_dispatch<float>(a, p->C1, p->Cout, blocks, s);
}
```

### segmentation_training_pipeline_amd/csrc/conv_wgrad.hip

```cpp
#include "common.h"
#include "launch.h"
#include <cstdlib>
#include <cstring>
#include <vector>
#include <type_traits>

typedef short s16x4 __attribute__((ext_vector_type(4)));

struct WgradArgs {
  const char* src0;
  const char* src1;
  const char* dy;
  float* out;
  int N, Hs0, Ws0, Hv, Wv, C0, C1, Ctot, mode;
  int KH, KW, stride, pad, Ho, Wo, Cout;
  int K, P, HoWo;
  int ntile_m, ntile_n, steps_per_split, nsteps;
  int xcd;
  int rowu;
  uint32_t bytes0, bytes1, bytesdy;
  FastDiv divC, divKW, divHoWo, divWo;
  BnBack pbn;
};

// ... 1207 lines not shown
  f32x4 s = {0.f, 0.f, 0.f, 0.f};
  if (e < per_split)
    for (int k = sl; k < splits; k += SL) s += slabs[(size_t)k * per_split + e];
  if (SL > 1) {
    sh[sl][ev] = s;
    __syncthreads();
#pragma unroll
    for (int w = SL / 2; w > 0; w >>= 1) {
      if (sl < w) sh[sl][ev] += sh[sl + w][ev];
      __syncthreads();
    }
    s = sh[0][ev];
  }
  if (sl != 0 || e >= per_split) return;
  constexpr int PERT = BM * 192 / 4;
  const int t = (int)(e / PERT);
  int col, co;
  row_slab_decode<BM, WM, WN>((int)(e - (int64_t)t * PERT), co, col);
  const int tile_m = t % ntile_m, tile_n = t / ntile_m;
  const int ncib = C0 >> 6, kh = tile_n / ncib, cib = tile_n - kh * ncib;
  const int kc = (kh * 3 + (col >> 6)) * C0 + cib * 64 + (col & 63);
  co += tile_m * BM;
#pragma unroll
  for (int r = 0; r < 4; ++r)
    if (co + r < Cout) {
      float* d = dw + (size_t)(co + r) * K + kc;
      *d = accumulate ? *d + s[r] : s[r];
    }
}

__global__ __launch_bounds__(256) void wgrad_reduce_kernel(const float* __restrict__ slabs, float* __restrict__ dw, int64_t count,
                                                           int splits, int accumulate) {
  const int64_t i = ((int64_t)blockIdx.x * 256 + threadIdx.x) * 4;
  if (i >= count) return;
  f32x4 s = *reinterpret_cast<const f32x4*>(slabs + i);
  int k = 1;
  for (; k + 3 < splits; k += 4) {
    const f32x4 a0 = *reinterpret_cast<const f32x4*>(slabs + (size_t)k * count + i), a1 = *reinterpret_cast<const f32x4*>(slabs + (size_t)(k + 1) * count + i);
    const f32x4 a2 = *reinterpret_cast<const f32x4*>(slabs + (size_t)(k + 2) * count + i), a3 = *reinterpret_cast<const f32x4*>(slabs + (size_t)(k + 3) * count + i);
    s += a0; s += a1; s += a2; s += a3;
  }
  for (; k < splits; ++k) s += *reinterpret_cast<const f32x4*>(slabs + (size_t)k * count + i);
  if (accumulate) s += *reinterpret_cast<const f32x4*>(dw + i);
  *reinterpret_cast<f32x4*>(dw + i) = s;
}

__global__ __launch_bounds__(256) void wgrad_reduce_wide_kernel(const float* __restrict__ slabs, float* __restrict__ dw, int64_t count,
                                                                int splits, int accumulate) {
  __shared__ f32x4 sh[16][16];
  const int ev = threadIdx.x & 15, sl = threadIdx.x >> 4;
  const int64_t i = ((int64_t)blockIdx.x * 16 + ev) * 4;
  f32x4 s = {0.f, 0.f, 0.f, 0.f};
  if (i < count) {
    int k = sl;
    for (; k + 112 < splits; k += 128) {
      f32x4 a[8];
#pragma unroll
      for (int u = 0; u < 8; ++u) a[u] = *reinterpret_cast<const f32x4*>(slabs + (size_t)(k + 16 * u) * count + i);
#pragma unroll
      for (int u = 0; u < 8; ++u) s += a[u];
    }
    for (; k < splits; k += 16) s += *reinterpret_cast<const f32x4*>(slabs + (size_t)k * count + i);
  }
  sh[sl][ev] = s;
  __syncthreads();
  for (int w = 8; w > 0; w >>= 1) {
    if (sl < w) sh[sl][ev] += sh[sl + w][ev];
    __syncthreads();
  }
  if (sl == 0 && i < count) {
    f32x4 r = sh[0][ev];
    if (accumulate) r += *reinterpret_cast<const f32x4*>(dw + i);
    *reinterpret_cast<f32x4*>(dw + i) = r;
  }
}

struct WgradPlan {
  int tile, bm, bn, ntile_m, ntile_n, splits, steps_per_split, nsteps;
};

extern "C" int stp_wgrad_sc_eligible(const stp_wgrad_params* p);
extern "C" int stp_wgrad_sc_slabs(const stp_wgrad_params* p);
extern "C" int stp_wgrad_sc_partial(const stp_wgrad_params* p, void* workspace, void* stream);
#define WG_TILE_SC 100

static WgradPlan plan_wgrad(const stp_wgrad_params* p) {
  WgradPlan w;
  if (p->splits == 0 && stp_wgrad_sc_eligible(p)) {
    w.tile = WG_TILE_SC; w.bm = w.bn = 0; w.ntile_m = w.ntile_n = 1;
    w.splits = stp_wgrad_sc_slabs(p); w.steps_per_split = 0; w.nsteps = 0;
    return w;
  }
  const int K = p->KH * p->KW * (p->C0 + p->C1);
  const int pk = p->dtype == STP_H16 ? 64 : 32;
  const int64_t P = (int64_t)p->N * p->Ho * p->Wo;
  if (p->Cout <= 16) { w.tile = 4; w.bm = 16; w.bn = 256; }
  else if (p->Cout <= 32) { w.tile = 3; w.bm = 32; w.bn = 256; }
  else if (p->Cout <= 64) { w.tile = 2; w.bm = 64; w.bn = 128; }
  else { w.tile = 1; w.bm = 128; w.bn = 128; }
  w.ntile_m = ceil_div(p->Cout, w.bm);
  w.ntile_n = ceil_div(K, w.bn);
  w.nsteps = ceil_div(P, pk);
  const int tiles = w.ntile_m * w.ntile_n;
  int splits = p->splits;
  if (splits <= 0) {
    const int cus = stp_cu_count();
    static const int target = getenv("STP_WGRAD_BLOCKS") ? atoi(getenv("STP_WGRAD_BLOCKS")) : 0;
    const int slots = target > 0 ? target : cus * (w.bm == 64 ? 3 : 2);
    splits = slots / tiles;
    if (splits < 1) splits = 1;
    const int max_by_steps = w.nsteps / 8 > 0 ? w.nsteps / 8 : 1;
    if (splits > max_by_steps) splits = max_by_steps;
    if (splits > 512) splits = 512;
  }
  if (splits > w.nsteps) splits = w.nsteps;
  if (splits < 1) splits = 1;
  w.steps_per_split = ceil_div(w.nsteps, splits);
  w.splits = ceil_div(w.nsteps, w.steps_per_split);
  return w;
}

static WgradPlan plan_wgrad_gemm(const stp_wgrad_params* p);

#define WG_TILE_ROW128 5
#define WG_TILE_ROW64 6
static bool wgrad_row_eligible(const stp_wgrad_params* p) {
  if (!p || p->dtype != STP_H16 || p->KH != 3 || p->KW != 3 || p->stride != 1 || p->pad != 1 || (p->C0 & 63) || (p->C1 & 63) ||
      p->Ho != p->Hv || p->Wo != p->Wv || (p->Cout & 7))
    return false;
  if (p->src_bn_mean && (!p->src_bn_rstd || p->C1 != 0 || p->src0_mode != STP_SRC_DIRECT)) return false;
  if (p->src0_mode == STP_SRC_DIRECT ? (p->Hs0 != p->Hv || p->Ws0 != p->Wv)
                                     : (p->src0_mode != STP_SRC_NEAREST2X || p->Hv != 2 * p->Hs0 || p->Wv != 2 * p->Ws0))
    return false;
  const int hw = p->Ho * p->Wo;
  return (p->Wo % 64 == 0) || (p->Wo >= 16 && 64 % p->Wo == 0 && hw % 64 == 0);
}
static bool wgrad_row_auto(const stp_wgrad_params* p) {
  static const bool on = !(getenv("STP_WGRAD_ROW") && atoi(getenv("STP_WGRAD_ROW")) == 0);
  return on && p->splits == 0 && wgrad_row_eligible(p);
}
static WgradPlan plan_wgrad_row(const stp_wgrad_params* p) {
  WgradPlan w;
  w.bm = p->Cout <= 64 ? 64 : 128; w.bn = 192;
  w.tile = w.bm == 64 ? WG_TILE_ROW64 : WG_TILE_ROW128;
  w.ntile_m = ceil_div(p->Cout, w.bm);
  w.ntile_n = 3 * ((p->C0 + p->C1) / 64);
  const int64_t P = (int64_t)p->N * p->Ho * p->Wo;
  w.nsteps = (int)(P / 64);
  const int tiles = w.ntile_m * w.ntile_n;
  int splits = p->splits;
  if (splits <= 0) {
    const int cus = stp_cu_count();
    static const int target = getenv("STP_WGRAD_ROW_BLOCKS") ? atoi(getenv("STP_WGRAD_ROW_BLOCKS")) : 0;
    const int slots = target > 0 ? target : cus * (w.bm == 64 ? 3 : 2);
    splits = slots / tiles;
    if (splits < 1) splits = 1;
    const int max_by_steps = w.nsteps / 8 > 0 ? w.nsteps / 8 : 1;
    if (splits > max_by_steps) splits = max_by_steps;
    if (splits > 512) splits = 512;
  }
  if (splits > w.nsteps) splits = w.nsteps;
  if (splits < 1) splits = 1;
  w.steps_per_split = ceil_div(w.nsteps, splits);
  w.splits = ceil_div(w.nsteps, w.steps_per_split);
  return w;
}
// ... 52 lines not shown
        case 1: return launch_wgrad<T, 128, 128, 2, 2, false>(a, w.splits, s);
        case 2: return launch_wgrad<T, 64, 128, 1, 4, false>(a, w.splits, s);
        case 3: return launch_wgrad<T, 32, 256, 1, 4, false>(a, w.splits, s);
        case 4: return launch_wgrad<T, 16, 256, 1, 4, false>(a, w.splits, s);
        default: return STP_E_BADARG;
      }
    }
    if constexpr (sizeof(T) == 2) {
      switch (w.tile * 4 + v) {
        case 1 * 4 + 2: return launch_wgrad_dma<T, 128, 128, 2, 2, 2>(a, w.splits, s);
        case 1 * 4 + 3: return launch_wgrad_dma<T, 128, 128, 2, 2, 3>(a, w.splits, s);
        case 2 * 4 + 2: return launch_wgrad_dma<T, 64, 128, 1, 4, 2>(a, w.splits, s);
        case 2 * 4 + 3: return launch_wgrad_dma<T, 64, 128, 1, 4, 3>(a, w.splits, s);
        case 3 * 4 + 2: return launch_wgrad_dma<T, 32, 256, 1, 4, 2>(a, w.splits, s);
        case 3 * 4 + 3: return launch_wgrad_dma<T, 32, 256, 1, 4, 3>(a, w.splits, s);
        case 4 * 4 + 2: return launch_wgrad_dma<T, 16, 256, 1, 4, 2>(a, w.splits, s);
        case 4 * 4 + 3: return launch_wgrad_dma<T, 16, 256, 1, 4, 3>(a, w.splits, s);
        default: return STP_E_BADARG;
      }
    } else {
      switch (w.tile * 4 + v) {
        case 1 * 4 + 2: return launch_wgrad_dma<T, 128, 128, 2, 2, 2>(a, w.splits, s);
        case 1 * 4 + 3: return launch_wgrad_dma<T, 128, 128, 2, 2, 3>(a, w.splits, s);
        case 2 * 4 + 2: return launch_wgrad_dma<T, 64, 128, 1, 4, 2>(a, w.splits, s);
        case 2 * 4 + 3: return launch_wgrad_dma<T, 64, 128, 1, 4, 3>(a, w.splits, s);
        default: return STP_E_BADARG;
      }
    }
  }
}

static WgradPlan plan_wgrad_gemm(const stp_wgrad_params* p) {
  stp_wgrad_params q = *p;
  if (q.splits == 0 && stp_wgrad_sc_eligible(p)) q.splits = -1;
  WgradPlan w = plan_wgrad(&q);
  return w;
}

static int wgrad_fill(const stp_wgrad_params* p, void* workspace, size_t workspace_bytes, WgradArgs& a, WgradPlan& w, bool* c4_out,
                      bool* dma_out) {
  if (!p || !p->src0 || !p->dy || !p->dw || !workspace) return STP_E_BADARG;
  if (p->dtype != STP_F32 && p->dtype != STP_H16) return STP_E_BADARG;
  const int vec = p->dtype == STP_H16 ? 8 : 4;
  const int sz = p->dtype == STP_H16 ? 2 : 4;
  const bool c4 = (p->dtype == STP_H16) && p->C0 == 4 && p->C1 == 0;
  if (c4) {
    if ((p->KW & 1) || p->src0_mode != STP_SRC_DIRECT) return STP_E_BADARG;
  } else if ((p->C0 % vec) || (p->C1 % vec)) {
    return STP_E_BADARG;
  }
  if (p->Cout % vec) return STP_E_BADARG;
  if (p->C1 > 0 && !p->src1) return STP_E_BADARG;
  if (stp_conv2d_wgrad_workspace_bytes(p) > workspace_bytes) return STP_E_WORKSPACE;
  w = plan_wgrad_gemm(p);
  if ((size_t)w.splits * p->Cout * p->KH * p->KW * (p->C0 + p->C1) * sizeof(float) > workspace_bytes) return STP_E_WORKSPACE;
  a.src0 = (const char*)p->src0; a.src1 = (const char*)p->src1; a.dy = (const char*)p->dy; a.out = (float*)workspace;
  a.N = p->N; a.Hs0 = p->Hs0; a.Ws0 = p->Ws0; a.Hv = p->Hv; a.Wv = p->Wv; a.C0 = p->C0; a.C1 = p->C1;
  a.Ctot = p->C0 + p->C1; a.mode = p->src0_mode;
  a.KH = p->KH; a.KW = p->KW; a.stride = p->stride; a.pad = p->pad; a.Ho = p->Ho; a.Wo = p->Wo; a.Cout = p->Cout;
  a.K = p->KH * p->KW * a.Ctot;
  const int64_t P = (int64_t)p->N * p->Ho * p->Wo;
  if (P >= (1ll << 31)) return STP_E_BADARG;
  a.P = (int)P; a.HoWo = p->Ho * p->Wo;
  a.ntile_m = w.ntile_m; a.ntile_n = w.ntile_n; a.steps_per_split = w.steps_per_split; a.nsteps = w.nsteps;
  a.xcd = w.ntile_m == 1;
  {
    const int pk = 128 / sz;
    a.rowu = (p->Wo % pk == 0) || (pk % p->Wo == 0 && a.HoWo % pk == 0);
  }
  a.divC = make_fastdiv((uint32_t)a.Ctot); a.divKW = make_fastdiv((uint32_t)a.KW);
  a.divHoWo = make_fastdiv((uint32_t)a.HoWo); a.divWo = make_fastdiv((uint32_t)a.Wo);
  const int64_t lim = 1ll << 31;
  const int64_t b0 = (int64_t)p->N * p->Hs0 * p->Ws0 * p->C0 * sz, b1 = (int64_t)p->N * p->Hv * p->Wv * p->C1 * sz;
  const int64_t bd = P * p->Cout * sz;
  a.bytes0 = (uint32_t)(b0 < lim ? b0 : 0); a.bytes1 = (uint32_t)(b1 < lim ? b1 : 0); a.bytesdy = (uint32_t)(bd < lim ? bd : 0);
  *c4_out = c4;
  *dma_out = !c4 && b0 < lim && b1 < lim && bd < lim;
  a.pbn.x = nullptr; a.pbn.mean = p->src_bn_mean; a.pbn.rstd = p->src_bn_rstd; a.pbn.gamma = p->src_bn_gamma; a.pbn.beta = p->src_bn_beta;
  a.pbn.relu = p->src_bn_relu;
  return STP_OK;
}

static int wg_group_bm(const stp_wgrad_params* p) {
  if (!p || !wgrad_row_eligible(p) || p->splits != 0) return 0;
  const int64_t lim = 1ll << 31;
  const int64_t P = (int64_t)p->N * p->Ho * p->Wo;
  if ((int64_t)p->N * p->Hs0 * p->Ws0 * p->C0 * 2 >= lim || (int64_t)p->N * p->Hv * p->Wv * p->C1 * 2 >= lim || P * p->Cout * 2 >= lim) return 0;
  return p->Cout <= 32 ? 32 : p->Cout <= 64 ? 64 : 128;
}
extern "C" int stp_wgrad_group_class(const stp_wgrad_params* p) { return wg_group_bm(p); }

struct WgGroupPlan {
  int bm = 0, max_slots_per_tile = 1;
  bool taps9 = false;
  std::vector<int> ntile_m, ntile_n, nsteps, tile0;
  std::vector<WgSeg> segs;
  std::vector<int> first;
  std::vector<WgTile> tiles;
  std::vector<int> slot_list;
};

static int wg_group_slots(int bm, bool taps9) {
  const int cus = stp_cu_count();
  static const int target = getenv("STP_WGRAD_GROUP_SLOTS") ? atoi(getenv("STP_WGRAD_GROUP_SLOTS")) : 0;
  if (target > 0) return target;
  if (taps9) return cus;
  return cus * (bm == 128 ? 2 : bm == 64 ? 3 : 4);
}
static bool wg_group_taps9(const stp_wgrad_params* const* L, int n) {
  static const int mode = getenv("STP_WGRAD_TAPS9") ? atoi(getenv("STP_WGRAD_TAPS9")) : 1;
  if (!mode) return false;
  if (mode != 2 && wg_group_bm(L[0]) != 128) return false;
  for (int l = 0; l < n; ++l)
    if (L[l]->src_bn_mean || !(L[l]->Wo == 16 || L[l]->Wo == 32 || L[l]->Wo % 64 == 0)) return false;
  return true;
}

static int wg_group_plan(const stp_wgrad_params* const* L, int n, WgGroupPlan& g) {
  if (!L || n <= 0) return STP_E_BADARG;
  g.bm = wg_group_bm(L[0]);
  if (!g.bm) return STP_E_BADARG;
  g.taps9 = wg_group_taps9(L, n);
  int64_t total = 0;
  int ntiles = 0;
  for (int l = 0; l < n; ++l) {
    if (wg_group_bm(L[l]) != g.bm || !L[l]->src0 || !L[l]->dy || !L[l]->dw) return STP_E_BADARG;
    const int tm = ceil_div(L[l]->Cout, g.bm), tn = (g.taps9 ? 1 : 3) * ((L[l]->C0 + L[l]->C1) / 64);
    const int ns = (int)((int64_t)L[l]->N * L[l]->Ho * L[l]->Wo / 64);
    g.ntile_m.push_back(tm); g.ntile_n.push_back(tn); g.nsteps.push_back(ns); g.tile0.push_back(ntiles);
    ntiles += tm * tn;
    total += (int64_t)tm * tn * ns;
  }
  const int slots = wg_group_slots(g.bm, g.taps9);
  const int MINSEG = 8;
  int64_t chunk = (total + slots - 1) / slots;
  if (chunk < 2 * MINSEG) chunk = 2 * MINSEG;
  std::vector<std::vector<int>> lists;
  for (;; ++chunk) {
    g.segs.clear(); g.first.clear();
    lists.assign(ntiles, std::vector<int>());
    int l = 0, r = 0, t = 0, s = 0;
    auto ranges_of = [&](int l_) { int64_t nr = (g.nsteps[l_] + chunk / 2) / chunk; return (int)(nr < 1 ? 1 : nr); };
    auto rlen_of = [&](int l_) { return ceil_div(g.nsteps[l_], ranges_of(l_)); };
    while (l < n) {
      g.first.push_back((int)g.segs.size());
      int64_t rem = chunk;
      int mine = 0;
      while (rem > 0 && l < n) {
        const int R = rlen_of(l), i0 = r * R, i1 = (i0 + R < g.nsteps[l]) ? i0 + R : g.nsteps[l];
        const int avail = i1 - i0 - s;
        int take = (int)(rem < avail ? rem : avail);
        if (avail - take > 0 && avail - take < MINSEG) take = avail;
        if (take < MINSEG && take < avail && mine > 0) break;
        WgSeg sg = {l, t, i0 + s, i0 + s + take, (int)g.segs.size(), 0, 0, 0};
        lists[g.tile0[l] + t].push_back(sg.slot);
        g.segs.push_back(sg);
        ++mine;
        rem -= take; s += take;
        if (s == i1 - i0) {
          s = 0;
          if (++t == g.ntile_m[l] * g.ntile_n[l]) { t = 0; if (++r == ranges_of(l)) { r = 0; ++l; } }
        }
      }
    }
    g.first.push_back((int)g.segs.size());
    if ((int)g.first.size() - 1 <= slots) break;
  }
// ... 72 lines not shown
    memcpy(tb + hd.off_layers + sizeof(WgLayer) * l, &wl, sizeof(wl));
  }
  memcpy(tb + hd.off_segs, g.segs.data(), sizeof(WgSeg) * g.segs.size());
  memcpy(tb + hd.off_first, g.first.data(), sizeof(int) * g.first.size());
  memcpy(tb + hd.off_tiles, g.tiles.data(), sizeof(WgTile) * g.tiles.size());
  memcpy(tb + hd.off_slots, g.slot_list.data(), sizeof(int) * g.slot_list.size());
  return STP_OK;
}

static const WgGroupHeader* wg_group_header(const void* host_table) {
  const WgGroupHeader* hd = (const WgGroupHeader*)host_table;
  return (hd && hd->magic == WG_GROUP_MAGIC && (hd->bm == 32 || hd->bm == 64 || hd->bm == 128) && hd->n_wg > 0 && hd->n_tiles > 0) ? hd : nullptr;
}

extern "C" int stp_wgrad_group_partial(const void* host_table, const void* dev_table, void* workspace, size_t workspace_bytes, void* stream) {
  const WgGroupHeader* hd = wg_group_header(host_table);
  if (!hd || !dev_table || !workspace) return STP_E_BADARG;
  if ((size_t)hd->n_segs * hd->bm * (hd->taps9 ? 576 : 192) * sizeof(float) > workspace_bytes) return STP_E_WORKSPACE;
  hipStream_t s = (hipStream_t)stream;
  if (hd->taps9) {
    const size_t lds9 = (size_t)3 * ((hd->bm == 128 ? 16384 : 8192) + 256 * 128);
    static_assert((size_t)3 * (8192 + 256 * 128) > STP_LDS_DEFAULT, "every launch of these kernels needs the grant");
    auto launch9 = [&](auto kern) { return stp_launch_lds(kern, dim3(hd->n_wg), dim3(512), lds9, s, (const char*)dev_table, (f32x4*)workspace); };
    if (hd->bm == 128 && hd->taps9 == 2) return launch9(conv_wgrad_taps9_group_kernel<128, 3, true>);
    if (hd->bm == 128) return launch9(conv_wgrad_taps9_group_kernel<128, 3>);
    if (hd->bm == 64) return launch9(conv_wgrad_taps9_group_kernel<64, 3>);
    return launch9(conv_wgrad_taps9_group_kernel<32, 3>);
  }
  const size_t lds = (size_t)3 * (64 * hd->bm * 2 + 72 * 128);
  auto launch = [&](auto kern, auto kern_pbn) {
    return stp_launch_lds(hd->pbn ? kern_pbn : kern, dim3(hd->n_wg), dim3(256), lds, s, (const char*)dev_table, (f32x4*)workspace);
  };
  if (hd->bm == 128) return launch(conv_wgrad_row_group_kernel<128, 2, 2, 3>, conv_wgrad_row_group_pbn_kernel<128, 2, 2, 3>);
  if (hd->bm == 64) return launch(conv_wgrad_row_group_kernel<64, 1, 4, 3>, conv_wgrad_row_group_pbn_kernel<64, 1, 4, 3>);
  return launch(conv_wgrad_row_group_kernel<32, 1, 4, 3>, conv_wgrad_row_group_pbn_kernel<32, 1, 4, 3>);
}

extern "C" int stp_wgrad_group_reduce(const void* host_table, const void* dev_table, const void* workspace, void* stream) {
  const WgGroupHeader* hd = wg_group_header(host_table);
  if (!hd || !dev_table || !workspace) return STP_E_BADARG;
  hipStream_t s = (hipStream_t)stream;
  const int sl = hd->reduce_lanes == 4 ? 4 : 1;
  if (hd->taps9) {
    const dim3 grid9(hd->n_tiles * (hd->bm * 576 / 4 / (256 / sl)));
#define STP_GROUP9_REDUCE(BM_)                                                                                                                       \
  do {                                                                                                                                               \
    if (sl == 4) hipLaunchKernelGGL((wgrad_group9_reduce_kernel<BM_, 4>), grid9, dim3(256), 0, s, (const char*)dev_table, (const f32x4*)workspace);  \
    else hipLaunchKernelGGL((wgrad_group9_reduce_kernel<BM_, 1>), grid9, dim3(256), 0, s, (const char*)dev_table, (const f32x4*)workspace);          \
  } while (0)
    if (hd->bm == 128 && hd->taps9 == 2) {
      if (sl == 4) hipLaunchKernelGGL((wgrad_group9_reduce_kernel<128, 4, true>), grid9, dim3(256), 0, s, (const char*)dev_table, (const f32x4*)workspace);
      else hipLaunchKernelGGL((wgrad_group9_reduce_kernel<128, 1, true>), grid9, dim3(256), 0, s, (const char*)dev_table, (const f32x4*)workspace);
    } else if (hd->bm == 128) STP_GROUP9_REDUCE(128);
    else if (hd->bm == 64) STP_GROUP9_REDUCE(64);
    else STP_GROUP9_REDUCE(32);
#undef STP_GROUP9_REDUCE
    STP_LAUNCH_CHECK();
    return STP_OK;
  }
  const int bpt = hd->bm * 192 / 4 / (256 / sl);
  const dim3 grid(hd->n_tiles * bpt);
#define STP_GROUP_REDUCE(BM_, WM_, WN_)                                                                                                     \
  do {                                                                                                                                      \
    if (sl == 4) hipLaunchKernelGGL((wgrad_group_reduce_kernel<BM_, WM_, WN_, 4>), grid, dim3(256), 0, s, (const char*)dev_table, (const f32x4*)workspace); \
    else hipLaunchKernelGGL((wgrad_group_reduce_kernel<BM_, WM_, WN_, 1>), grid, dim3(256), 0, s, (const char*)dev_table, (const f32x4*)workspace);         \
  } while (0)
  if (hd->bm == 128) STP_GROUP_REDUCE(128, 2, 2);
  else if (hd->bm == 64) STP_GROUP_REDUCE(64, 1, 4);
  else STP_GROUP_REDUCE(32, 1, 4);
#undef STP_GROUP_REDUCE
  STP_LAUNCH_CHECK();
  return STP_OK;
}

extern "C" int stp_conv2d_wgrad_kernel_id(const stp_wgrad_params* p) {
  if (!p) return 0;
  if (p->splits == 0 && stp_wgrad_sc_eligible(p)) return 1;
  if (wgrad_row_auto(p)) return p->Cout <= 64 ? 3 : 2;
  return 0;
}

extern "C" int stp_conv2d_wgrad_partial(const stp_wgrad_params* p, void* workspace, size_t workspace_bytes, int32_t variant,
                                        void* stream) {
  if (p && variant == 0 && p->splits == 0 && stp_wgrad_sc_eligible(p)) {
    if (!workspace || stp_conv2d_wgrad_workspace_bytes(p) > workspace_bytes) return STP_E_WORKSPACE;
    return stp_wgrad_sc_partial(p, workspace, stream);
  }
  if (p && p->src_bn_mean && !(variant == 4 || (variant == 0 && wgrad_row_auto(p)))) return STP_E_BADARG;
  WgradArgs a;
  WgradPlan w;
  bool c4, dma;
  const int rc = wgrad_fill(p, workspace, workspace_bytes, a, w, &c4, &dma);
  if (rc != STP_OK) return rc;
  hipStream_t s = (hipStream_t)stream;
  if (variant == 4 || (variant == 0 && wgrad_row_auto(p))) {
    if (!wgrad_row_eligible(p) || !dma) return STP_E_BADARG;
    w = plan_wgrad_row(p);
    a.ntile_m = w.ntile_m; a.ntile_n = w.ntile_n; a.steps_per_split = w.steps_per_split; a.nsteps = w.nsteps;
    a.xcd = w.ntile_m == 1;
    static const int stages = getenv("STP_WGRAD_ROW_STAGES") ? atoi(getenv("STP_WGRAD_ROW_STAGES")) : 3;
    const size_t lds = (size_t)(stages == 2 ? 2 : 3) * (64 * w.bm * 2 + 72 * 128);
    if (stages == 2) {
      if (a.pbn.mean) return STP_E_BADARG;
      if (w.tile == WG_TILE_ROW128) return launch_wg(conv_wgrad_row_kernel<128, 2, 2, 2>, a, lds, w.splits, s);
      return launch_wg(conv_wgrad_row_kernel<64, 1, 4, 2>, a, lds, w.splits, s);
    }
    if (a.pbn.mean) {
      if (w.tile == WG_TILE_ROW128) return launch_wg(conv_wgrad_row_pbn_kernel<128, 2, 2, 3>, a, lds, w.splits, s);
      return launch_wg(conv_wgrad_row_pbn_kernel<64, 1, 4, 3>, a, lds, w.splits, s);
    }
    if (w.tile == WG_TILE_ROW128) return launch_wg(conv_wgrad_row_kernel<128, 2, 2, 3>, a, lds, w.splits, s);
    return launch_wg(conv_wgrad_row_kernel<64, 1, 4, 3>, a, lds, w.splits, s);
  }
  if (p->dtype == STP_H16)
    return c4 ? launch_wgrad_tile<bf16_t, true>(a, w, dma, variant, s) : launch_wgrad_tile<bf16_t, false>(a, w, dma, variant, s);
  return launch_wgrad_tile<float, false>(a, w, dma, variant, s);
}

extern "C" int stp_conv2d_wgrad_reduce(const stp_wgrad_params* p, const void* workspace, int32_t variant, void* stream) {
  if (!p || !p->dw || !workspace) return STP_E_BADARG;
  if (variant == 4 || (variant == 0 && wgrad_row_auto(p) && !stp_wgrad_sc_eligible(p))) {
    if (!wgrad_row_eligible(p)) return STP_E_BADARG;
    const WgradPlan r = plan_wgrad_row(p);
    const int64_t per_split = (int64_t)r.ntile_m * r.ntile_n * r.bm * 192 / 4;
    const int K = 9 * (p->C0 + p->C1);
    const int sl = r.splits >= 32 ? 16 : r.splits >= 8 ? 4 : 1;
    const dim3 grid(ceil_div(per_split, 256 / sl));
    hipStream_t s = (hipStream_t)stream;
    const f32x4* slabs = (const f32x4*)workspace;
#define STP_ROW_REDUCE(BM_, WM_, WN_, SL_) \
    hipLaunchKernelGGL((wgrad_reduce_row_kernel<BM_, WM_, WN_, SL_>), grid, dim3(256), 0, s, slabs, p->dw, per_split, r.splits, p->accumulate, \
                       r.ntile_m, p->C0 + p->C1, p->Cout, K)
    if (r.bm == 128) { if (sl == 16) STP_ROW_REDUCE(128, 2, 2, 16); else if (sl == 4) STP_ROW_REDUCE(128, 2, 2, 4); else STP_ROW_REDUCE(128, 2, 2, 1); }
    else { if (sl == 16) STP_ROW_REDUCE(64, 1, 4, 16); else if (sl == 4) STP_ROW_REDUCE(64, 1, 4, 4); else STP_ROW_REDUCE(64, 1, 4, 1); }
#undef STP_ROW_REDUCE
    STP_LAUNCH_CHECK();
    return STP_OK;
  }
  const WgradPlan w = variant == 0 ? plan_wgrad(p) : plan_wgrad_gemm(p);
  const int64_t count = (int64_t)p->Cout * p->KH * p->KW * (p->C0 + p->C1);
  if ((w.splits >= 64 && count <= (1 << 16)) || (w.splits >= 32 && count <= (1 << 19)))
    hipLaunchKernelGGL(wgrad_reduce_wide_kernel, dim3(ceil_div(count, 64)), dim3(256), 0, (hipStream_t)stream,
                       (const float*)workspace, p->dw, count, w.splits, p->accumulate);
  else
    hipLaunchKernelGGL(wgrad_reduce_kernel, dim3(ceil_div(count, 1024)), dim3(256), 0, (hipStream_t)stream, (const float*)workspace,
                       p->dw, count, w.splits, p->accumulate);
  STP_LAUNCH_CHECK();
  return STP_OK;
}

struct WgReduceDesc {
  const float* slabs;
  float* dw;
  int64_t count;
  int32_t splits, accumulate;
};

__global__ __launch_bounds__(256) void wgrad_reduce_batched_kernel(const WgReduceDesc* __restrict__ D) {
  const WgReduceDesc d = D[blockIdx.y];
  if ((int64_t)blockIdx.x * 64 >= d.count) return;
  __shared__ f32x4 sh[16][16];
  const int ev = threadIdx.x & 15, sl = threadIdx.x >> 4;
  const int64_t i = ((int64_t)blockIdx.x * 16 + ev) * 4;
  f32x4 s = {0.f, 0.f, 0.f, 0.f};
  if (i < d.count) {
    int k = sl;
// ... 48 lines not shown
```

### segmentation_training_pipeline_amd/graph.py

```python
import os
import ctypes as C
from collections import OrderedDict

import numpy as np
import torch

from . import _lib, ops

_TD = {"bf16": torch.bfloat16, "fp16": torch.float16, "fp32": torch.float32}


class StpShapeError(ValueError):
    pass


def _rup(a, b):
    return (a + b - 1) // b * b


class DT(object):
    __slots__ = ("name", "N", "H", "W", "C", "buf", "grad", "_grad_ready", "grad_writes", "needs_grad", "gradC", "meta")

    def __init__(self, name, N, H, W, Cn, buf=None, needs_grad=False):
        self.name, self.N, self.H, self.W, self.C = name, N, H, W, Cn
        self.buf, self.grad, self._grad_ready, self.needs_grad = buf, None, False, needs_grad
        self.grad_writes = 0
        self.gradC = Cn
        self.meta = {}

    @property
    def grad_ready(self):
        return self._grad_ready

    @grad_ready.setter
    def grad_ready(self, v):
        self._grad_ready = bool(v)
        if v:
            self.grad_writes += 1

    @property
    def rows(self):
        return self.N * self.H * self.W


class ParamInfo(object):
    __slots__ = ("name", "offset", "numel", "shape", "kind", "trainable", "pending_slices")

    def __init__(self, name, offset, shape, kind, trainable):
        self.name, self.offset, self.shape, self.kind, self.trainable = name, offset, tuple(shape), kind, trainable
        self.numel = int(np.prod(shape))
        self.pending_slices = 0

    @property
    def end(self):
        return self.offset + self.numel


class Plan(object):
    def __init__(self, batch, dtype="bf16", device="cuda", training=True, class_metrics=False):
        if dtype not in _TD:
            raise ValueError("dtype must be 'bf16', 'fp16' or 'fp32'")
        self.device = torch.device(device)
        if self.device.type == "cuda" and not torch.cuda.is_available():
            raise _lib.StpError("the HIP training path needs a GPU; there is no CPU fallback")
        self.lib = _lib.load("fp16" if dtype == "fp16" else "bf16")
        self.loss_scale = 1.0
        self.dls = None
        self.N = batch
        self.dtype = dtype
        self.tdt = _TD[dtype]
        self.cdt = {"bf16": ops.BF16, "fp16": ops.F16, "fp32": ops.F32}[dtype]
        self.vec = 4 if dtype == "fp32" else 8
        self.training = training
        self.params = OrderedDict()
        self.states = OrderedDict()
        self._poff = 0
        self._soff = 0
        self.dry = True
        self.frozen_prefixes = ()
        self._keep = []
        self.tensors = OrderedDict()
        self.P = self.G = self.S = None
        self.prep, self.fwd, self.bwd, self.opt = [], [], [], []
        self._tape = []
        self._goffs = []
        self.bwd_marks, self.bwd_monotone = [], True
        self._prep_layers = []
        self._upc_layers = []
        self._upc4_layers = []
        self._wg_ws_bytes = 0
        self._bn_ws_c = 4
        self.bn_momentum = 0.99
        self.fuse_bn_backward = os.environ.get("STP_FUSE_BN_BACKWARD", "1") != "0"
        self.fuse_bn_backward_last = os.environ.get("STP_FUSE_BN_BACKWARD_LAST", "1") != "0"
        self.fold_upsample_grad = os.environ.get("STP_FOLD_UPSAMPLE_GRAD", "1") != "0"
        self.wgrad_group_gflop = float(os.environ.get("STP_WGRAD_GROUP_GFLOP", "300"))
        self.wgrad_lone_group_gflop = float(os.environ.get("STP_WGRAD_LONE_GROUP_GFLOP", "600"))
        self.reduce_batch = int(os.environ.get("STP_WGRAD_REDUCE_BATCH", "0"))
        self._pending_reduces, self._pending_reduce_hi = [], 0
        self._wgroup, self._wgroup_cls, self._wgroup_flops, self._wgroup_hi = [], 0, 0.0, 0
        self._wgroup_reads = set()
        self.wgroups = []
        self._dw_ws_bytes = 0
        self.step_state = None
        self.bn_slots = os.environ.get("STP_BN_SLOTS", "0") == "1"
        self.fuse_bn_sc = os.environ.get("STP_FUSE_BN_SC", "1") != "0"
        self.fuse_bn_halo = os.environ.get("STP_FUSE_BN_HALO", "0") != "0" and os.environ.get("STP_HALO", "1") != "0"
        self.bn_slots_max_rows = int(os.environ.get("STP_BN_SLOTS_MAXROWS", "1073741824"))
        self._slot_need = 0
        self._slot_used = 0
        self.slot_arena = None
        self.loss_scalars = None
        self.class_metrics = bool(class_metrics)
        self.masked_loss = None
        self.lovasz_softmax = 0.0
        self.class_weights = None
        self.class_counts = None
        self.inputs = {}

    def define(self, net_fn, share=None):
        self.dry = True
        net_fn(self)
        n = _rup(self._poff, 4)
        if share is not None:
            if [(k, v.offset, v.shape) for k, v in share.params.items()] != [(k, v.offset, v.shape) for k, v in self.params.items()] \
                    or list(share.states.items()) != list(self.states.items()):
                raise StpShapeError("plans that share weights must declare identical parameters")
            self.P, self.S, self.G = share.P, share.S, None
        else:
            self.P = torch.zeros(n, dtype=torch.float32, device=self.device)
            self.G = torch.zeros(n, dtype=torch.float32, device=self.device) if self.training else None
            self.S = torch.zeros(max(_rup(self._soff, 4), 4), dtype=torch.float32, device=self.device)
        self.mask = torch.ones(n, dtype=torch.uint8, device=self.device)
        self.ws_wgrad = torch.empty(max(self._wg_ws_bytes // 4, 4) + 4, dtype=torch.float32, device=self.device)
        self.ws_bn = torch.empty(ops.bn_workspace_bytes(_rup(self._bn_ws_c, 4)) // 4, dtype=torch.float32, device=self.device)
        self.ws_loss = torch.empty(ops.loss_workspace_bytes() // 4, dtype=torch.float32, device=self.device)
        self.ws_dw = torch.empty(max(self._dw_ws_bytes // 4, 4), dtype=torch.float32, device=self.device)
        if self.training and self.bn_slots and self._slot_need:
            self.slot_arena = torch.zeros(_rup(self._slot_need, 2), dtype=torch.int64, device=self.device)
        self.dry = False
        self._tape = []
        self._prep_layers = []
        self._upc_layers = []
        self._upc4_layers = []
        self.tensors = OrderedDict()
        net_fn(self)
        self._fuse_bn_finalize(self._fuse_bn_into_consumers())
        self._finish_prep()
        if self.training:
            self.bwd_marks, self.bwd_monotone = [], True
            low = self.G.numel() if self.G is not None else 0
            for back in reversed(self._tape):
                self._goffs = []
                back()
                if self._goffs:
                    if max(e for _, e in self._goffs) > low:
                        self.bwd_monotone = False
                    low = min(low, min(o for o, _ in self._goffs))
                self.bwd_marks.append((len(self.bwd), max(low, self._wgroup_hi, self._pending_reduce_hi)))
            if self._wgroup or self._pending_reduces:
                self._flush_wgroup()
                self._flush_reduces()
                self.bwd_marks.append((len(self.bwd), low))
        self._tape = []
        return self

    @staticmethod
    def _nslots(Cn):
        n = 16
        while n > 1 and n * Cn > 1024:
            n //= 2
        return n

    def _slots(self, Cn):
        n = self._nslots(Cn)
        off = self._slot_used
        self._slot_used += 2 * Cn * n
        if self._slot_used > self.slot_arena.numel():
# ... 80 lines not shown
    def _use(*ts):
        for t in ts:
            if t is not None:
                t.meta["uses"] = t.meta.get("uses", 0) + 1

    def _completes_grad(self, t, acc, promoted=False, last_ok=True):
        uses = t.meta.get("uses", 0)
        sole = (uses == 1 or (promoted and uses == 2 and t.grad_writes == 1)) and not acc
        return bool(sole or (last_ok and self.fuse_bn_backward_last and uses > 1 and t.grad_writes == uses - 1 and acc))

    def _emit_grad_pass(self, fname, t, acc, tile_args, args, enabled=True):
        bnm = t.meta.get("bn")
        ntl = int(getattr(self.lib, fname + "_bn_tiles")(*tile_args)) if (
            self.fuse_bn_backward and bnm is not None and self._completes_grad(t, acc) and self.slot_arena is None and enabled) else 0
        if ntl > 0:
            st = self._alloc((2 * t.C * ntl,), torch.float32)
            self._emit(self.bwd, fname + "_bn", *args, *bnm, st.data_ptr())
            t.meta["bnb"] = (st, ntl)
        else:
            self._emit(self.bwd, fname, *args)

    def _emit(self, lst, fname, *args):
        lst.append((getattr(self.lib, fname), args, fname, None))

    @staticmethod
    def _set_src_bn(p, bn):
        p.src_bn_mean, p.src_bn_rstd, p.src_bn_gamma, p.src_bn_beta, p.src_bn_relu = bn[1:]

    @staticmethod
    def _set_bnb(q, bn):
        q.bnb_x, q.bnb_mean, q.bnb_rstd, q.bnb_gamma, q.bnb_beta, q.bnb_relu = bn or (None, None, None, None, None, 0)

    def _fuse_bn_into_consumers(self):
        drop, kept = set(), set()
        for t in self.tensors.values():
            rec, sc, halo = t.meta.get("apply_rec"), t.meta.get("sc_consumers") or [], t.meta.get("halo_consumers") or []
            if rec is None or not (sc or halo) or len(sc) + len(halo) != t.meta.get("uses", 0):
                continue
            bn = t.meta["bn"]
            halo_full = bool(halo) and all(ok for _, _, ok in halo)
            for cp, wp in sc + [h[:2] for h in halo]:
                cp.src0 = bn[0]
                self._set_src_bn(cp, bn)
                if not halo or halo_full:
                    self._set_src_bn(wp, bn)
            if halo and not halo_full:
                kept.add(id(rec))
            else:
                t.meta["deferred"] = rec
                t.meta["src_override"] = bn[0]
                drop.add(id(rec))
        self.fwd = [r for r in self.fwd if id(r) not in drop]
        return kept

    def _fuse_bn_finalize(self, keep=()):
        if os.environ.get("STP_BN_FUSE_FINALIZE", "1") == "0":
            return
        out, i, fwd = [], 0, self.fwd
        while i < len(fwd):
            r = fwd[i]
            nxt = fwd[i + 1] if i + 1 < len(fwd) else None
            if (r[2] == "stp_bn_finalize" and nxt is not None and nxt[2] == "stp_bn_apply" and id(nxt) not in keep
                    and nxt[1][7] == r[1][6] and nxt[1][8] == r[1][7] and nxt[1][1] == nxt[1][3] == self.cdt and nxt[1][5] == nxt[1][6] == r[1][3]
                    and nxt[1][12] == 0.0):
                part, tiles, rows, Cn, eps, mom, mean, rstd, mm, mv = r[1]
                x, _, y, _, rows2, _, _, _, _, gp, beta, relu, _ = nxt[1]
                if rows2 == rows and int(self.lib.stp_bn_finalize_apply_ok(self.cdt, rows, Cn, tiles)):
                    out.append((self.lib.stp_bn_finalize_apply, (part, tiles, x, y, self.cdt, rows, Cn, eps, mom, mean, rstd, mm, mv, gp, beta, relu),
                                "stp_bn_finalize_apply", None))
                    i += 2
                    continue
            out.append(r)
            i += 1
        self.fwd = out

    def tensor(self, name):
        t = self.tensors[name]
        rec = t.meta.get("deferred")
        if rec is not None:
            fn, args = rec[0], rec[1]
            rc = fn(*args, torch.cuda.current_stream().cuda_stream)
            if rc != 0:
                raise _lib.StpError("%s failed with %d" % (rec[2], rc))
        return t

    def _scratch(self, nbytes):
        nbytes = int(nbytes)
        if nbytes <= 0:
            return None, 0
        buf = self._alloc((nbytes // 4,), torch.float32)
        return buf.data_ptr(), nbytes

    def _group_stats(self, p, st, Cs):
        cols = int(self.lib.stp_conv2d_stats_floats(C.byref(p))) // (2 * Cs)
        G = int(self.lib.stp_conv2d_stats_group_for(C.byref(p)))
        if G < 2:
            return st, cols
        ng = -(-cols // G)
        out = self._alloc((2 * Cs * ng,), torch.float32)
        cnt = torch.zeros((max(1, int(self.lib.stp_conv2d_stats_group_counters(C.byref(p), G))),), dtype=torch.int32, device=self.device)
        self._keep.append(cnt)
        p.stats_group_out, p.stats_group_counters, p.stats_group = out.data_ptr(), cnt.data_ptr(), G
        return out, ng

    def _emit_conv(self, lst, p, meta=None):
        self._keep.append(p)
        if meta is not None and meta.get("tile") == 512:
            meta = dict(meta, sc=(int(p.C0), 1 if p.Cout <= 16 else 2))
        if meta is not None and meta.get("tile") == 800:
            meta = dict(meta, pw=(int(p.C0), int(p.Cout)))
        lst.append((self.lib.stp_conv2d, (C.byref(p),), "stp_conv2d", meta))

    def _emit_wgrad(self, p, name, flops, defer_hi=0):
        lst = self.bwd
        self._keep.append(p)
        meta = {"layer": name, "pass": "wgrad", "flops": flops, "cout": p.Cout, "sc": bool(self.lib.stp_wgrad_sc_eligible(C.byref(p))),
                "kernel_id": int(self.lib.stp_conv2d_wgrad_kernel_id(C.byref(p)))}
        if defer_hi > 0 and self.reduce_batch > 0:
            db = int(self.lib.stp_wgrad_reduce_desc_bytes())
            wsb = int(self.lib.stp_conv2d_wgrad_workspace_bytes(C.byref(p)))
            ws = self._alloc((max(wsb // 4, 4) + 4,), torch.float32)
            desc = (C.c_char * db)()
            count = int(self.lib.stp_wgrad_reduce_desc_fill(C.addressof(desc), 0, C.byref(p), ws.data_ptr()))
            if count > 0:
                lst.append((self.lib.stp_conv2d_wgrad_partial, (C.byref(p), ws.data_ptr(), ws.numel() * 4, 0), "stp_conv2d_wgrad", meta))
                self._pending_reduces.append((bytes(desc), count))
                self._pending_reduce_hi = max(self._pending_reduce_hi, int(defer_hi))
                if len(self._pending_reduces) >= self.reduce_batch:
                    self._flush_reduces()
                return
            self._keep = [t for t in self._keep if t is not ws]
        lst.append((self.lib.stp_conv2d_wgrad_partial, (C.byref(p), self.ws_wgrad.data_ptr(), self.ws_wgrad.numel() * 4, 0),
                    "stp_conv2d_wgrad", meta))
        lst.append((self.lib.stp_conv2d_wgrad_reduce, (C.byref(p), self.ws_wgrad.data_ptr(), 0), "stp_conv2d_wgrad_reduce", None))

    def _flush_reduces(self):
        if not self._pending_reduces:
            return
        table = b"".join(d for d, _ in self._pending_reduces)
        dev = self._table(table)
        n, maxc = len(self._pending_reduces), max(c for _, c in self._pending_reduces)
        self.bwd.append((self.lib.stp_wgrad_reduce_batched, (dev.data_ptr(), n, maxc), "stp_wgrad_reduce_batched", {"layers": n}))
        self._pending_reduces, self._pending_reduce_hi = [], 0

    def _flush_wgroup(self):
        if not self._wgroup:
            return
        layers, cls = self._wgroup, self._wgroup_cls
        self._wgroup, self._wgroup_cls, self._wgroup_flops, self._wgroup_hi, self._wgroup_reads = [], 0, 0.0, 0, set()
        n = len(layers)
        lone_group = cls == 128 and 0 < self.wgrad_lone_group_gflop * 1e9 <= layers[0][2]
        if n == 1 and cls != 32 and not lone_group:
            self._emit_wgrad(*layers[0])
            return
        arr = (C.POINTER(_lib.WgradParams) * n)(*[C.pointer(wp) for wp, _, _ in layers])
        tb = int(self.lib.stp_wgrad_group_table_bytes(arr, n))
        wsb = int(self.lib.stp_wgrad_group_workspace_bytes(arr, n))
        if tb <= 0 or wsb <= 0:
            raise StpShapeError("grouped weight gradient: the layers %s do not form a group" % [nm for _, nm, _ in layers])
        host = (C.c_char * tb)()
        _lib.check(self.lib.stp_wgrad_group_build(arr, n, C.addressof(host), tb), "stp_wgrad_group_build")
        dev = self._table(bytes(host))
        ws = self._alloc((wsb // 4,), torch.float32)
        self._keep += [arr, host] + [wp for wp, _, _ in layers]
        names = [nm for _, nm, _ in layers]
        self.wgroups.append((names, cls))
# ... 13 lines not shown
            raise StpShapeError("input_bn handles up to 7 image channels")
        Cp = 4 if x.C <= 3 else 8
        beta = self.param(name + "/beta", (x.C,), "beta")
        mm = self.state(name + "/moving_mean", x.C, 0.0)
        mv = self.state(name + "/moving_variance", x.C, 1.0)
        out = self._new(name, x.H, x.W, Cp, False)
        out.meta["real_c"] = x.C
        out.meta["input_bn_beta"] = beta
        if self.dry:
            return out
        if self.training:
            mean, rstd = self._alloc((x.C,), torch.float32), self._alloc((x.C,), torch.float32)
            self._emit(self.fwd, "stp_bn_stats", x.buf.data_ptr(), ops.U8, x.rows, x.C, eps, self.bn_momentum,
                       mean.data_ptr(), rstd.data_ptr(), self._sptr(mm), self._sptr(mv), self.ws_bn.data_ptr(),
                       self.ws_bn.numel() * 4)
            self._emit(self.fwd, "stp_bn_apply", x.buf.data_ptr(), ops.U8, out.buf.data_ptr(), self.cdt, x.rows, x.C, Cp,
                       mean.data_ptr(), rstd.data_ptr(), None, self._pptr(beta), 0, 1.0)
        else:
            self._emit(self.fwd, "stp_bn_inference", x.buf.data_ptr(), ops.U8, out.buf.data_ptr(), self.cdt, x.rows, x.C, Cp,
                       self._sptr(mm), self._sptr(mv), eps, None, self._pptr(beta), 0, 1.0)
        return out

    def input_cast(self, name, x):
        if x.C > 7:
            raise StpShapeError("input_cast handles up to 7 image channels")
        Cp = 4 if x.C <= 3 else 8
        out = self._new(name, x.H, x.W, Cp, False)
        out.meta["real_c"] = x.C
        if self.dry:
            return out
        zero, one = self._alloc((8,), torch.float32), self._alloc((8,), torch.float32)
        zero.zero_(); one.fill_(1.0)
        self._emit(self.fwd, "stp_bn_apply", x.buf.data_ptr(), ops.U8, out.buf.data_ptr(), self.cdt, x.rows, x.C, Cp,
                   zero.data_ptr(), one.data_ptr(), None, None, 0, 0.0)
        return out

    def bn(self, name, x, eps, relu=True, scale=True, momentum=None):
        Cn = x.C
        relu = int(relu)
        momentum = self.bn_momentum if momentum is None else float(momentum)
        gamma = self.param(name + "/gamma", (Cn,), "gamma") if scale else None
        beta = self.param(name + "/beta", (Cn,), "beta")
        mm = self.state(name + "/moving_mean", Cn, 0.0)
        mv = self.state(name + "/moving_variance", Cn, 1.0)
        out = self._new(name, x.H, x.W, Cn, x.needs_grad or beta.trainable)
        self._bn_ws_c = max(self._bn_ws_c, Cn)
        self._use(x)
        if self.dry:
            self._slot_need += 4 * Cn * self._nslots(Cn)
            return out
        gp = self._pptr(gamma) if gamma else None
        if not self.training:
            self._emit(self.fwd, "stp_bn_inference", x.buf.data_ptr(), self.cdt, out.buf.data_ptr(), self.cdt, x.rows, Cn, Cn,
                       self._sptr(mm), self._sptr(mv), eps, gp, self._pptr(beta), int(relu), 0.0)
            return out
        mean, rstd = self._alloc((Cn,), torch.float32), self._alloc((Cn,), torch.float32)
        table = x.meta.get("stats_table")
        slots = x.meta.get("stats_slots")
        if slots is not None:
            self._emit(self.fwd, "stp_bn_apply_slots", x.buf.data_ptr(), out.buf.data_ptr(), self.cdt, x.rows, Cn, slots[0], slots[1], eps,
                       momentum, mean.data_ptr(), rstd.data_ptr(), self._sptr(mm), self._sptr(mv), gp, self._pptr(beta), int(relu))
        elif table is not None:
            self._emit(self.fwd, "stp_bn_finalize", table[0].data_ptr(), table[1], x.rows, Cn, eps, momentum, mean.data_ptr(),
                       rstd.data_ptr(), self._sptr(mm), self._sptr(mv))
        else:
            self._emit(self.fwd, "stp_bn_stats", x.buf.data_ptr(), self.cdt, x.rows, Cn, eps, momentum, mean.data_ptr(),
                       rstd.data_ptr(), self._sptr(mm), self._sptr(mv), self.ws_bn.data_ptr(), self.ws_bn.numel() * 4)
        if slots is None:
            self._emit(self.fwd, "stp_bn_apply", x.buf.data_ptr(), self.cdt, out.buf.data_ptr(), self.cdt, x.rows, Cn, Cn,
                       mean.data_ptr(), rstd.data_ptr(), gp, self._pptr(beta), int(relu), 0.0)
        out.meta["bn"] = (x.buf.data_ptr(), mean.data_ptr(), rstd.data_ptr(), gp, self._pptr(beta), int(relu))
        if self.fuse_bn_sc and slots is None:
            out.meta["apply_rec"] = self.fwd[-1]
            out.meta["sc_consumers"], out.meta["halo_consumers"] = [], []

        def back():
            if not out.needs_grad or not out.grad_ready:
                return
            bslots = out.meta.get("bnb_slots")
            dadd = None
            if (x.needs_grad and x.grad_ready and x.grad is not None and x.grad.data_ptr() in self._wgroup_reads and bslots is None
                    and out.meta.get("bnb") is not None):
                dadd, x.grad = x.grad, None
            dx = self._gradbuf(x) if x.needs_grad else self._alloc((x.N, x.H, x.W, Cn))
            if bslots is not None:
                self._emit(self.bwd, "stp_bn_backward_slots", x.buf.data_ptr(), out.grad.data_ptr(), dx.data_ptr(), self.cdt, x.rows, Cn,
                           mean.data_ptr(), rstd.data_ptr(), gp, bslots[0], bslots[1], self._gptr(gamma) if gamma else None,
                           self._gptr(beta), int(x.grad_ready and x.needs_grad))
            elif out.meta.get("bnb") is not None:
                st, q = out.meta["bnb"]
                tiles = q if isinstance(q, int) else int(self.lib.stp_conv2d_stats_floats(C.byref(q))) // (2 * Cn)
                if dadd is not None:
                    self._emit(self.bwd, "stp_bn_backward_fused_add", x.buf.data_ptr(), out.grad.data_ptr(), dx.data_ptr(), dadd.data_ptr(),
                               self.cdt, x.rows, Cn, mean.data_ptr(), rstd.data_ptr(), gp, st.data_ptr(), tiles,
                               self._gptr(gamma) if gamma else None, self._gptr(beta), 1, self.ws_bn.data_ptr(), self.ws_bn.numel() * 4)
                else:
                    self._emit(self.bwd, "stp_bn_backward_fused", x.buf.data_ptr(), out.grad.data_ptr(), dx.data_ptr(), self.cdt,
                               x.rows, Cn, mean.data_ptr(), rstd.data_ptr(), gp, st.data_ptr(), tiles,
                               self._gptr(gamma) if gamma else None, self._gptr(beta), int(x.grad_ready and x.needs_grad),
                               self.ws_bn.data_ptr(), self.ws_bn.numel() * 4)
            else:
                self._emit(self.bwd, "stp_bn_backward", x.buf.data_ptr(), out.grad.data_ptr(), dx.data_ptr(), self.cdt, x.rows, Cn,
                           mean.data_ptr(), rstd.data_ptr(), gp, self._pptr(beta), self._gptr(gamma) if gamma else None,
                           self._gptr(beta), int(relu), int(x.grad_ready and x.needs_grad), self.ws_bn.data_ptr(), self.ws_bn.numel() * 4)
            if x.needs_grad:
                x.grad_ready = True

        self._tape.append(back)
        return out

    def _emit_bias_grad(self, dy, rows, gradC, Cout, b):
        tmp = self._alloc((gradC,), torch.float32)
        self._emit(self.bwd, "stp_channel_sum", dy.data_ptr(), self.cdt, rows, gradC, tmp.data_ptr(), 0, self.ws_bn.data_ptr(), self.ws_bn.numel() * 4)
        self._emit(self.bwd, "stp_weight_grad_unpad", tmp.data_ptr(), self._gptr(b), Cout, 1, 1, 1, 1, 1, 0)

    def conv3x3_taps(self, name, x, Cout, bias=False):
        cin = x.meta.get("real_c", x.C)
        z = self.conv(name + "_taps", x, 9 * Cout, 1, param_name=name, param_shape=(Cout, 3, 3, cin), cout_pad=64 if self.dtype != "fp32" else None)
        b = self.param(name + "/bias", (Cout,), "bias") if bias else None
        out = self._new(name, x.H, x.W, Cout, z.needs_grad or (b is not None and b.trainable))
        out.gradC = _rup(Cout, self.vec)
        if bias:
            self._bn_ws_c = max(self._bn_ws_c, out.gradC)
        self._use(z)
        if self.dry:
            return out
        self._emit(self.fwd, "stp_tapsum_fwd", z.buf.data_ptr(), out.buf.data_ptr(), self._pptr(b) if b is not None else None, self.N, x.H, x.W,
                   Cout, z.C, Cout, self.cdt)
        if not self.training:
            return out

        def back():
            if not out.grad_ready:
                return
            dy = out.grad
            if b is not None and b.trainable:
                self._emit_bias_grad(dy, out.rows, out.gradC, Cout, b)
            if z.needs_grad:
                self._emit(self.bwd, "stp_tapsum_bwd", dy.data_ptr(), self._gradbuf(z).data_ptr(), self.N, x.H, x.W, Cout, out.gradC, z.gradC, self.cdt)
                z.grad_ready = True

        self._tape.append(back)
        return out

    def conv(self, name, x, Cout, k, stride=1, pad=0, src1=None, upsample=False, bias=False, residual=None, bn_stats=False,
             transpose=False, relu=False, same_tf=False, fold_shortcut=None, param_name=None, param_shape=None, cout_pad=None,
             param_cols=None, flops_as=None):
        L = ConvLayer(self, name, x, Cout, k, stride, pad, src1, upsample, residual, transpose, relu, same_tf, fold_shortcut, param_cols)
        L.declare(param_name, param_shape, cout_pad, bias)
        if self.dry:
            return L.out
        L.forward(bn_stats, flops_as)
        if self.training:
            self._tape.append(L.backward)
        return L.out

    def add(self, name, y, skip):
        if (y.H, y.W, y.C) != (skip.H, skip.W, skip.C):
            raise StpShapeError("%s: cannot add %dx%dx%d and %dx%dx%d" % (name, y.H, y.W, y.C, skip.H, skip.W, skip.C))
        out = DT(name, self.N, y.H, y.W, y.C, y.buf, y.needs_grad or skip.needs_grad)
        out.gradC = y.gradC
        self.tensors[name] = out
        self._use(y, skip)
        if self.dry:
            return out
        self._emit(self.fwd, "stp_add_inplace", y.buf.data_ptr(), skip.buf.data_ptr(), y.rows * y.C, self.cdt)
# ... 732 lines not shown
class ConvLayer(object):

    def __init__(self, plan, name, x, Cout, k, stride, pad, src1, upsample, residual, transpose, relu, same_tf, fold_shortcut, param_cols):
        if transpose:
            if stride != 1 or upsample or src1 is not None or residual is not None or k % 2:
                raise StpShapeError("transpose=True is the plain stride-2 'same' Conv2DTranspose with an even kernel")
            pad = k - 1 - (k // 2 - 1)
        real_c0 = x.meta.get("real_c", x.C)
        stem = real_c0 != x.C
        if stem and (src1 is not None or upsample):
            raise StpShapeError("padded-channel input supports a plain conv only")
        C0, C1 = x.C, (src1.C if src1 is not None else 0)
        if not stem and (C0 % plan.vec or C1 % plan.vec):
            raise StpShapeError("%s: input channels (%d,%d) must be multiples of %d for dtype %s" % (name, C0, C1, plan.vec, plan.dtype))
        Hv, Wv = (2 * x.H, 2 * x.W) if upsample else ((2 * x.H - 1, 2 * x.W - 1) if transpose else (x.H, x.W))
        if src1 is not None and (src1.H, src1.W) != (Hv, Wv):
            raise StpShapeError("%s: skip tensor is %dx%d, expected %dx%d" % (name, src1.H, src1.W, Hv, Wv))
        Ho, Wo = (Hv + 2 * pad - k) // stride + 1, (Wv + 2 * pad - k) // stride + 1
        if same_tf:
            Ho, Wo = -(-Hv // stride), -(-Wv // stride)
            pad = max((Ho - 1) * stride + k - Hv, 0) // 2
            if max((Wo - 1) * stride + k - Wv, 0) // 2 != pad:
                raise StpShapeError("%s: 'same' padding differs between height and width" % name)
        self.KWp = k + (k & 1) if (stem and x.C == 4) else k
        self.plan, self.name, self.x, self.src1, self.residual, self.fs, self.param_cols = plan, name, x, src1, residual, fold_shortcut, param_cols
        self.Cout, self.k, self.stride, self.pad, self.upsample, self.transpose, self.relu = Cout, k, stride, pad, upsample, transpose, relu
        self.real_c0, self.stem, self.C0, self.C1, self.Hv, self.Wv, self.Ho, self.Wo = real_c0, stem, C0, C1, Hv, Wv, Ho, Wo
        self.Cin_master, self.Cinp = real_c0 + C1, C0 + C1
        self.src_mode = ops.SRC_NEAREST2X if upsample else (ops.SRC_ZEROINS2X if transpose else ops.SRC_DIRECT)

    def declare(self, param_name, param_shape, cout_pad, bias):
        pl, name, x, src1, residual, Cout, k, Cin_master, param_cols = self.plan, self.name, self.x, self.src1, self.residual, self.Cout, self.k, self.Cin_master, self.param_cols
        if param_cols is not None:
            if k != 1 or self.stem or self.transpose or self.C1 or Cout % pl.vec or Cin_master % 4 or param_cols[0] % 4 or param_cols[1] % 4 \
                    or param_cols[0] + Cin_master > param_cols[1]:
                raise StpShapeError("%s: a column range of a shared kernel serves a plain 1x1 convolution with aligned channel counts" % name)
            param_shape = None
        w = pl.param((param_name or name) + "/kernel", (Cout, 1, 1, param_cols[1]) if param_cols is not None else (param_shape or (Cout, k, k, Cin_master)),
                     "tkernel" if self.transpose else "kernel")
        if param_shape is not None and int(np.prod(param_shape)) != Cout * k * k * Cin_master:
            raise StpShapeError("%s: parameter view of %s does not match %d x %d x %d x %d" % (name, param_shape, Cout, k, k, Cin_master))
        self.w, self.b = w, (pl.param(name + "/bias", (Cout,), "bias") if bias else None)
        CoutB = self.CoutB = _rup(Cout, cout_pad or pl.vec)
        self.x_ng, self.s_ng = x.needs_grad, (src1.needs_grad if src1 is not None else False)
        self.out = pl._new(name, self.Ho, self.Wo, Cout, self.x_ng or self.s_ng or w.trainable or (residual is not None and residual.needs_grad))
        self.out.gradC = CoutB
        if bias:
            pl._bn_ws_c = max(pl._bn_ws_c, CoutB)
        pl._use(x, src1, residual)
        wp = self.wp = _lib.WgradParams()
        wp.N, wp.Hs0, wp.Ws0, wp.Hv, wp.Wv, wp.C0, wp.C1, wp.src0_mode = pl.N, x.H, x.W, self.Hv, self.Wv, self.C0, self.C1, self.src_mode
        wp.KH, wp.KW, wp.stride, wp.pad, wp.Ho, wp.Wo, wp.Cout = k, self.KWp, self.stride, self.pad, self.Ho, self.Wo, CoutB
        wp.accumulate, wp.dtype, wp.splits = 0, pl.cdt, 0
        if pl.training and w.trainable:
            pl._wg_ws_bytes = max(pl._wg_ws_bytes, int(pl.lib.stp_conv2d_wgrad_workspace_bytes(C.byref(wp))))

    def forward(self, bn_stats, flops_as):
        pl, x, src1, residual, out, k, Cout = self.plan, self.x, self.src1, self.residual, self.out, self.k, self.Cout
        self._weight_copies()
        p = self.p = ops.conv_params(x.buf, self.wf, out.buf, N=pl.N, Hs0=x.H, Ws0=x.W, Hv=self.Hv, Wv=self.Wv, C0=self.C0, C1=self.C1,
                                     src1=src1.buf if src1 is not None else None,
                                     mode=self.src_mode, KH=k, KW=self.KWp, stride=self.stride, pad=self.pad,
                                     Ho=self.Ho, Wo=self.Wo, Cout=Cout, dtype=pl.cdt, residual=residual.buf if residual is not None else None)
        self._collapsed_copies()
        self._register_bn_consumer()
        if self.b is not None:
            p.bias = pl._pptr(self.b)
        if self.relu:
            if self.CoutB != Cout:
                raise StpShapeError("%s: a fused ReLU needs Cout to be a multiple of %d" % (self.name, pl.vec))
            p.relu = 1
        if bn_stats and pl.training and pl.slot_arena is not None and pl.N * self.Ho * self.Wo <= pl.bn_slots_max_rows:
            p.stats_partial, p.stats_slots = out.meta["stats_slots"] = pl._slots(Cout)
        elif bn_stats and pl.training:
            nfl = int(pl.lib.stp_conv2d_stats_floats(C.byref(p)))
            st = pl._alloc((max(nfl, 4),), torch.float32)
            p.stats_partial = st.data_ptr()
            out.meta["stats_table"] = pl._group_stats(p, st, Cout)
        self.flops = 2.0 * pl.N * self.Ho * self.Wo * Cout * k * k * self.Cin_master / (4.0 if self.transpose else 1.0)
        if flops_as is not None:
            self.flops = float(flops_as)
        pl._emit_conv(pl.fwd, p, {"layer": self.name, "pass": "fwd", "flops": self.flops, "tile": int(pl.lib.stp_conv2d_tile_for(C.byref(p))),
                                  "src2": bool(self.C1 or self.upsample)})

    def _weight_copies(self):
        pl, w, Cout, k, KWp, Cinp, Cin_master, param_cols = self.plan, self.w, self.Cout, self.k, self.KWp, self.Cinp, self.Cin_master, self.param_cols
        wf = self.wf = pl._alloc((_rup(Cout, 16) * k * KWp * Cinp,))
        self.need_dgrad = pl.training and (self.x_ng or self.s_ng) and not self.stem
        wb = self.wb = pl._alloc((_rup(Cinp, 16) * k * k * self.CoutB,)) if self.need_dgrad else None
        self.out.meta["wb"] = wb
        wsrc = pl._pptr(w)
        if param_cols is not None:
            w.pending_slices += 1
            wm = pl._alloc((Cout * Cin_master,), torch.float32)
            pl._emit(pl.prep, "stp_copy_cols_f32", wm.data_ptr(), Cin_master, wsrc + 4 * int(param_cols[0]), int(param_cols[1]), Cout, Cin_master, 0)
            wsrc = wm.data_ptr()
        self.out.meta["w_master"] = (wsrc, Cout, Cin_master, k)
        pl._prep_layers.append((wsrc, wf.data_ptr(), wb.data_ptr() if wb is not None else None, Cout, k, k, Cin_master, KWp, Cinp, self.CoutB))

    def _collapsed_copies(self):
        pl, p, C0, C1, rows_f = self.plan, self.p, self.C0, self.C1, _rup(self.Cout, 16)
        self.w4 = None
        if not (self.upsample and self.src1 is not None and self.k == 3 and self.KWp == 3 and self.stride == 1 and self.pad == 1
                and self.Cinp == self.Cin_master == C0 + C1
                and os.environ.get("STP_UPCOLLAPSE", "1") != "0" and not pl.lib.stp_conv2d_scn_eligible(C.byref(p))
                and int(pl.lib.stp_conv2d_halo_variant(C.byref(p))) < 0):
            return
        wup = pl._alloc((rows_f * 16 * C0,))
        pl._upc_layers.append((pl._pptr(self.w), wup.data_ptr(), self.Cout, rows_f, C0, C0 + C1))
        p.weight_up = wup.data_ptr()
        if self.need_dgrad and self.x_ng and C0 % 16 == 0 and os.environ.get("STP_UPCOLLAPSE_BWD", "0") == "1":
            self.w4 = pl._alloc((C0 * 16 * self.CoutB,))
            pl._upc4_layers.append((pl._pptr(self.w), self.w4.data_ptr(), self.Cout, self.CoutB, C0, C0 + C1))

    def _register_bn_consumer(self):
        pl, x, p, wp, w = self.plan, self.x, self.p, self.wp, self.w
        if not pl.training or x.meta.get("apply_rec") is None or self.src1 is not None or self.transpose or self.stem:
            return
        if self.residual is None and pl.lib.stp_conv2d_sc_eligible(C.byref(p)) and (not w.trainable or pl.lib.stp_wgrad_sc_eligible(C.byref(wp))):
            x.meta["sc_consumers"].append((p, wp))
        elif pl.fuse_bn_halo and not self.upsample and pl.lib.stp_conv2d_halo_variant(C.byref(p)) >= 0:
            x.meta["halo_consumers"].append((p, wp, (not w.trainable) or int(pl.lib.stp_conv2d_wgrad_kernel_id(C.byref(wp))) in (2, 3)))

    def backward(self):
        pl, out, residual, b = self.plan, self.out, self.residual, self.b
        if not out.needs_grad or not out.grad_ready:
            return
        dy = self.dy = out.grad
        if self.relu:
            pl._guard_write(dy)
            pl._emit(pl.bwd, "stp_relu_bwd", out.buf.data_ptr(), dy.data_ptr(), out.rows * out.gradC, pl.cdt)
        if residual is not None and residual.needs_grad:
            if not residual.grad_ready and residual.gradC == out.gradC:
                residual.grad = dy
                residual.grad_ready = True
            else:
                pl._emit(pl.bwd, "stp_add_inplace", pl._gradbuf(residual).data_ptr(), dy.data_ptr(), out.rows * out.gradC, pl.cdt)
        if self.w.trainable:
            self._weight_grad()
        if b is not None and b.trainable and out.meta.get("loss_bias_grad") and self.Cout == 1:
            pl._emit(pl.bwd, "stp_sigmoid_loss_bias_grad", pl.ws_loss.data_ptr(), out.rows, pl._gptr(b), 0)
        elif b is not None and b.trainable and out.meta.get("loss_bias_grad") == "multilabel":
            pl._emit(pl.bwd, "stp_sigmoid_multilabel_bias_grad", pl.ws_loss.data_ptr(), out.rows, self.Cout, pl._gptr(b), 0)
        elif b is not None and b.trainable:
            pl._emit_bias_grad(dy, out.rows, self.CoutB, self.Cout, b)
        if self.need_dgrad and not out.meta.get("dgrad_folded"):
            self._data_grad()

    def _weight_grad(self):
        pl, x, src1, w, wp, k, Cout, Cin_master, param_cols = self.plan, self.x, self.src1, self.w, self.wp, self.k, self.Cout, self.Cin_master, self.param_cols
        padded, gcols = self.stem or self.CoutB != Cout, None
        if padded:
            dwp = pl._alloc((self.CoutB * k * self.KWp * self.Cinp,), torch.float32)
            wp.dw = dwp.data_ptr()
        elif param_cols is not None:
            gcols = pl._alloc((Cout * Cin_master,), torch.float32)
            wp.dw = gcols.data_ptr()
        else:
            wp.dw = pl._gptr(w)
        wp.src0, wp.src1, wp.dy = x.meta.get("src_override") or x.buf.data_ptr(), (src1.buf.data_ptr() if src1 is not None else None), self.dy.data_ptr()
        cls = int(pl.lib.stp_wgrad_group_class(C.byref(wp))) if (pl.wgrad_group_gflop > 0 and not padded and gcols is None) else 0
        if cls:
            self._wgrad_join_group(cls)
        else:
            pl._flush_wgroup()
            pl._emit_wgrad(wp, self.name, self.flops, defer_hi=0 if (padded or gcols is not None) else w.end)
        if gcols is not None:
            w.pending_slices -= 1
            gbase = pl._gptr(w) if w.pending_slices == 0 else pl.G.data_ptr() + 4 * w.offset
            pl._emit(pl.bwd, "stp_copy_cols_f32", gbase + 4 * int(param_cols[0]), int(param_cols[1]), gcols.data_ptr(), Cin_master, Cout, Cin_master, 0)
        if padded:
            pl._emit(pl.bwd, "stp_weight_grad_unpad", dwp.data_ptr(), pl._gptr(w), Cout, k, k, Cin_master, self.KWp, self.Cinp, 0)
        beta = x.meta.get("input_bn_beta")
        if self.stem and beta is not None and beta.trainable:
            pl._emit(pl.bwd, "stp_stem_beta_grad", dwp.data_ptr(), pl._pptr(w), pl._gptr(beta), Cout, k, k, self.real_c0, self.KWp, self.Cinp, self.real_c0)

    def _wgrad_join_group(self, cls):
        pl = self.plan
        if pl._wgroup and pl._wgroup_cls != cls:
            pl._flush_wgroup()
        pl._wgroup.append((self.wp, self.name, self.flops))
        pl._wgroup_cls = cls
        pl._wgroup_flops += self.flops
        pl._wgroup_hi = max(pl._wgroup_hi, self.w.end)
        pl._wgroup_reads.add(self.dy.data_ptr())
        if pl._wgroup_flops >= pl.wgrad_group_gflop * 1e9:
            pl._flush_wgroup()

    def _data_grad(self):
        pl, x = self.plan, self.x
        self._dgrad_dests()
        q = self._dgrad_plain()
        if self.stride not in (1, 2):
            raise StpShapeError("data gradient supports stride 1 and 2")
        if self._form_scatter():
            return
        form = (self._form_s2d() or self._form_parity_fold(q) or self._form_fold1(q) or self._form_collapsed()
                or self._form_sum2x2_stream(q) or self._form_sum2x2_halo(q) or Dgrad(q, self))
        if form.folded_up and self.d0_hires is not None:
            pl._keep = [t for t in pl._keep if t is not self.d0_hires]
            self.d0 = self.d0_hires = None
        self._attach_bn_sums(form)
        pl._emit_conv(pl.bwd, form.q, {"layer": self.name, "pass": "dgrad", "flops": form.flops,
                                       "tile": int(pl.lib.stp_conv2d_tile_for(C.byref(form.q))), "s2d": form.s2d, "fold1": form.fold1})
        if self.upsample and self.x_ng and not form.folded_up:
            acc = int(x.grad_ready)
            pl._emit_grad_pass("stp_upsample2x_bwd", x, acc, (pl.N, x.H, x.W, self.C0, self.C0, pl.cdt),
                               (self.d0.data_ptr(), pl._gradbuf(x).data_ptr(), pl.N, x.H, x.W, self.C0, self.C0, pl.cdt, acc),
                               os.environ.get("STP_FUSE_UP_BN", "1") != "0")
        if self.x_ng:
            x.grad_ready = True
        if self.s_ng:
            self.src1.grad_ready = True

    def _dgrad_dests(self):
        pl, x, src1, shape = self.plan, self.x, self.src1, (self.plan.N, self.Hv, self.Wv)
        self.d0_hires = None
        if self.upsample:
            d0 = self.d0_hires = pl._alloc(shape + (self.C0,)) if self.x_ng else None
            self.acc0 = 0
        else:
            d0 = pl._gradbuf(x) if self.x_ng else None
            self.acc0 = int(x.grad_ready)
        d1 = pl._gradbuf(src1) if self.s_ng else None
        self.acc1 = int(src1.grad_ready) if self.s_ng else 0
        if d0 is None:
            d0 = pl._alloc(shape + (self.C0,))
        if self.C1 and d1 is None:
            d1 = pl._alloc(shape + (self.C1,))
        self.d0, self.d1 = d0, d1

    def _dgrad_plain(self):
        pl, x, k, stride, Ho, Wo, C0 = self.plan, self.x, self.k, self.stride, self.Ho, self.Wo, self.C0
        if self.transpose:
            return ops.conv_params(self.dy, self.wb, self.d0, N=pl.N, Hs0=Ho, Ws0=Wo, Hv=Ho, Wv=Wo, C0=self.CoutB, mode=ops.SRC_DIRECT, KH=k, KW=k,
                                   stride=2, pad=k - 1 - self.pad, Ho=x.H, Wo=x.W, Cout=C0, dtype=pl.cdt, accumulate0=self.acc0)
        return ops.conv_params(self.dy, self.wb, self.d0, N=pl.N, Hs0=Ho, Ws0=Wo,
                               Hv=(2 * Ho - 1 if stride == 2 else Ho), Wv=(2 * Wo - 1 if stride == 2 else Wo),
                               C0=self.CoutB, mode=(ops.SRC_ZEROINS2X if stride == 2 else ops.SRC_DIRECT), KH=k, KW=k, stride=1,
                               pad=k - 1 - self.pad, Ho=self.Hv, Wo=self.Wv, Cout=C0 + self.C1, dtype=pl.cdt, dst1=self.d1, Cd0=C0,
                               accumulate0=self.acc0, accumulate1=self.acc1)

    def _form_scatter(self):
# ... 119 lines not shown
```

### segmentation_training_pipeline_amd/ops.py

```python
import ctypes as C

import torch

from . import _lib
from ._lib import BF16, F16, F32, U8, SRC_DIRECT, SRC_NEAREST2X, SRC_ZEROINS2X

_DT = {torch.float32: F32, torch.bfloat16: BF16, torch.float16: F16, torch.uint8: U8}


def dt(t):
    return _DT[t.dtype]


def ptr(t):
    return None if t is None else t.data_ptr()


def stream():
    return torch.cuda.current_stream().cuda_stream


def _dev(t):
    if t is not None and not t.is_cuda:
        raise _lib.StpError("tensor must live on the GPU (no CPU fallback)")
# ... 37 lines not shown

def conv2d_wgrad(p, workspace, st=None):
    _lib.check(_lib.load().stp_conv2d_wgrad(C.byref(p), ptr(workspace), workspace.numel() * workspace.element_size(),
                                            stream() if st is None else st), "stp_conv2d_wgrad")


def conv2d_wgrad_partial(p, workspace, variant=0):
    _lib.check(_lib.load().stp_conv2d_wgrad_partial(C.byref(p), ptr(workspace), workspace.numel() * workspace.element_size(),
                                                    variant, stream()), "stp_conv2d_wgrad_partial")


def conv2d_wgrad_reduce(p, workspace, variant=0):
    _lib.check(_lib.load().stp_conv2d_wgrad_reduce(C.byref(p), ptr(workspace), variant, stream()), "stp_conv2d_wgrad_reduce")


class WgradGroup(object):

    def __init__(self, params, device="cuda"):
        lib = _lib.load()
        self.params = list(params)
        n = len(self.params)
        self.arr = (C.POINTER(_lib.WgradParams) * n)(*[C.pointer(p) for p in self.params])
        tb = int(lib.stp_wgrad_group_table_bytes(self.arr, n))
        wsb = int(lib.stp_wgrad_group_workspace_bytes(self.arr, n))
        if tb <= 0 or wsb <= 0:
            raise _lib.StpError("the layers do not form a weight-gradient group")
        self.host = (C.c_char * tb)()
        _lib.check(lib.stp_wgrad_group_build(self.arr, n, C.addressof(self.host), tb), "stp_wgrad_group_build")
        self.dev = torch.frombuffer(bytearray(bytes(self.host)), dtype=torch.uint8).to(device)
        self.ws = torch.empty(wsb // 4, dtype=torch.float32, device=device)
        self.header = list((C.c_int32 * 16).from_buffer_copy(bytes(self.host)[:64]))

    def partial(self):
        _lib.check(_lib.load().stp_wgrad_group_partial(C.addressof(self.host), self.dev.data_ptr(), self.ws.data_ptr(), self.ws.numel() * 4, stream()),
                   "stp_wgrad_group_partial")

    def reduce(self):
        _lib.check(_lib.load().stp_wgrad_group_reduce(C.addressof(self.host), self.dev.data_ptr(), self.ws.data_ptr(), stream()), "stp_wgrad_group_reduce")

    def run(self):
        self.partial()
        self.reduce()


def wgrad_group_class(p):
    return int(_lib.load().stp_wgrad_group_class(C.byref(p)))


def weight_prepare(master, fwd, bwd, Cout, KH, KW, Cin, KWp, Cinp, CoutB, dtype):
    _lib.call("stp_weight_prepare", ptr(master), ptr(fwd), ptr(bwd), Cout, KH, KW, Cin, KWp, Cinp, CoutB, dtype, stream())


def weight_grad_unpad(padded, grad, Cout, KH, KW, Cin, KWp, Cinp, accumulate=0):
    _lib.call("stp_weight_grad_unpad", ptr(padded), ptr(grad), Cout, KH, KW, Cin, KWp, Cinp, accumulate, stream())


def stem_beta_grad(padded_dw, master, dbeta, Cout, KH, KW, Cin, KWp, Cinp, one_ch):
    _lib.call("stp_stem_beta_grad", ptr(padded_dw), ptr(master), ptr(dbeta), Cout, KH, KW, Cin, KWp, Cinp, one_ch, stream())


def bn_workspace_bytes(Cn):
    return int(_lib.load().stp_bn_workspace_bytes(Cn))


def bn_stats(x, rows, Cn, eps, momentum, mean, rstd, moving_mean, moving_var, workspace):
    _lib.call("stp_bn_stats", ptr(_dev(x)), dt(x), rows, Cn, eps, momentum, ptr(mean), ptr(rstd), ptr(moving_mean),
              ptr(moving_var), ptr(workspace), workspace.numel() * workspace.element_size(), stream())


def bn_apply(x, y, rows, Cn, Cy, mean, rstd, gamma, beta, relu, pad_value=0.0):
    _lib.call("stp_bn_apply", ptr(x), dt(x), ptr(y), dt(y), rows, Cn, Cy, ptr(mean), ptr(rstd), ptr(gamma), ptr(beta),
              int(relu), float(pad_value), stream())


def bn_inference(x, y, rows, Cn, Cy, mm, mv, eps, gamma, beta, relu, pad_value=0.0):
    _lib.call("stp_bn_inference", ptr(x), dt(x), ptr(y), dt(y), rows, Cn, Cy, ptr(mm), ptr(mv), float(eps), ptr(gamma),
              ptr(beta), int(relu), float(pad_value), stream())


def bn_backward(x, dy, dx, rows, Cn, mean, rstd, gamma, beta, dgamma, dbeta, relu, accumulate_dx, workspace):
    _lib.call("stp_bn_backward", ptr(x), ptr(dy), ptr(dx), dt(x), rows, Cn, ptr(mean), ptr(rstd), ptr(gamma), ptr(beta),
              ptr(dgamma), ptr(dbeta), int(relu), int(accumulate_dx), ptr(workspace),
              workspace.numel() * workspace.element_size(), stream())


def bn_backward_fused(x, g, dx, rows, Cn, mean, rstd, gamma, partial, tiles, dgamma, dbeta, accumulate_dx, workspace):
    _lib.call("stp_bn_backward_fused", ptr(x), ptr(g), ptr(dx), dt(x), rows, Cn, ptr(mean), ptr(rstd), ptr(gamma), ptr(partial),
              int(tiles), ptr(dgamma), ptr(dbeta), int(accumulate_dx), ptr(workspace),
              workspace.numel() * workspace.element_size(), stream())


def maxpool3x3s2(x, y, idx, N, H, W, Cn):
    _lib.call("stp_maxpool3x3s2", ptr(x), ptr(y), ptr(idx), N, H, W, Cn, dt(x), stream())


def maxpool3x3s2_bwd(idx, dy, dx, N, H, W, Cn, accumulate=0):
    _lib.call("stp_maxpool3x3s2_bwd", ptr(idx), ptr(dy), ptr(dx), N, H, W, Cn, dt(dy), int(accumulate), stream())


def maxpool2x2(x, y, idx, N, H, W, Cn):
    _lib.call("stp_maxpool2x2", ptr(x), ptr(y), ptr(idx), N, H, W, Cn, dt(x), stream())


def maxpool2x2_bwd(idx, dy, dx, N, H, W, Cn, accumulate=0):
    _lib.call("stp_maxpool2x2_bwd", ptr(idx), ptr(dy), ptr(dx), N, H, W, Cn, dt(dy), int(accumulate), stream())


def maxpool_k(x, y, idx, N, H, W, Cn, k):
    _lib.call("stp_maxpool_k", ptr(x), ptr(y), ptr(idx), N, H, W, Cn, k, dt(x), stream())


def maxpool_k_bwd(idx, dy, dx, N, H, W, Cn, k, accumulate=0):
    _lib.call("stp_maxpool_k_bwd", ptr(idx), ptr(dy), ptr(dx), N, H, W, Cn, k, dt(dy), int(accumulate), stream())


def relu_bwd(y, dy, count):
    _lib.call("stp_relu_bwd", ptr(y), ptr(dy), count, dt(dy), stream())


def zero_bytes(t, nbytes):
    _lib.call("stp_zero_bytes", ptr(t), nbytes, stream())


def resize_nearest(x, y, N, H, W, Cn, factor, ldo, coff):
    _lib.call("stp_resize_nearest", ptr(x), ptr(y), N, H, W, Cn, factor, ldo, coff, dt(x), stream())


def resize_nearest_bwd(dy, dx, N, H, W, Cn, factor, ldo, coff, accumulate=0):
    _lib.call("stp_resize_nearest_bwd", ptr(dy), ptr(dx), N, H, W, Cn, factor, ldo, coff, dt(dy), int(accumulate), stream())


def dropout_spatial(x, y, N, HW, Cn, rate, state, salt):
    _lib.call("stp_dropout_spatial", ptr(x), ptr(y), N, HW, Cn, float(rate), ptr(state), int(salt), dt(x), stream())


def softmax_act(z, p, rows, classes, ldz, ldp):
    _lib.call("stp_softmax_act", ptr(z), ptr(p), rows, classes, ldz, ldp, dt(z), stream())


def softmax_act_bwd(p, dp, dz, rows, classes, ldp, ldg):
    _lib.call("stp_softmax_act_bwd", ptr(p), ptr(dp), ptr(dz), rows, classes, ldp, ldg, dt(p), stream())


def prob_cce_dice(probs, target, pixels, classes, ldc, w_cce, w_dice, scalars, dprobs, dl_channels, workspace):
    _lib.call("stp_prob_cce_dice", ptr(probs), ptr(target), pixels, classes, ldc, dt(probs), float(w_cce), float(w_dice), ptr(scalars),
              ptr(dprobs), dl_channels, ptr(workspace), workspace.numel() * workspace.element_size(), stream())


def upsample2x_bwd(dy, dx, N, H, W, Cn, ldy, accumulate=0):
    _lib.call("stp_upsample2x_bwd", ptr(dy), ptr(dx), N, H, W, Cn, ldy, dt(dy), int(accumulate), stream())


def channel_sum(x, rows, Cn, out, accumulate, workspace):
    _lib.call("stp_channel_sum", ptr(x), dt(x), rows, Cn, ptr(out), int(accumulate), ptr(workspace),
              workspace.numel() * workspace.element_size(), stream())


def add_inplace(dst, src, count):
    _lib.call("stp_add_inplace", ptr(dst), ptr(src), count, dt(dst), stream())


def se_chunks(N, HW, Cn):
    return int(_lib.load().stp_se_chunks(N, HW, Cn))


def se_workspace_bytes(N, HW, Cn):
# ... 388 lines not shown
```

Baseline: 2558 images/sec.

## Fuse stem BN backward dx into stem weight-gradient kernel

For the stem conv followed by BN, the BN backward now computes only the reductions (dgamma/dbeta and sums) and skips writing dx. The stem wgrad kernel then recomputes the BN input-gradient on the fly from BN input, mean, rstd and sums while staging dy tiles in LDS. The full BN dx is still produced later, but only if something actually reads the stem output gradient. This removes a full write and reread of the largest activation gradient, at the cost of an extra LDS buffer, an extra global load stream and per-tile ALU work in the wgrad kernel, which may lower occupancy.

```diff
diff --git a/include/stp_hip.h b/include/stp_hip.h
--- a/include/stp_hip.h
+++ b/include/stp_hip.h
@@ -109,6 +109,15 @@
   const float* src_bn_gamma;
   const float* src_bn_beta;
   int32_t src_bn_relu;
+  const void* dyb_x;
+  const float* dyb_mean;
+  const float* dyb_rstd;
+  const float* dyb_gamma;
+  const float* dyb_beta;
+  const float* dyb_sums;
+  float dyb_inv_rows;
+  int32_t dyb_relu;
+  float* dyb_keep;
 } stp_wgrad_params;
 
 size_t stp_conv2d_wgrad_workspace_bytes(const stp_wgrad_params* p);
@@ -118,6 +127,7 @@
 int stp_wgrad_sc_eligible(const stp_wgrad_params* p);
 int stp_wgrad_sc_slabs(const stp_wgrad_params* p);
 int stp_wgrad_sc_partial(const stp_wgrad_params* p, void* workspace, void* stream);
+int stp_wgrad_stem_dxb_ok(const stp_wgrad_params* p);
 int stp_conv2d_wgrad_kernel_id(const stp_wgrad_params* p);
 
 int stp_wgrad_group_class(const stp_wgrad_params* p);
@@ -174,6 +184,7 @@
                     const float* mean, const float* rstd, const float* gamma, const float* beta,
                     float* dgamma, float* dbeta, int32_t relu, int32_t accumulate_dx,
                     void* workspace, size_t workspace_bytes, void* stream);
+const float* stp_bn_backward_sums(const void* workspace, int32_t C);
 
 int stp_maxpool3x3s2(const void* x, void* y, uint8_t* idx, int32_t N, int32_t H, int32_t W, int32_t C,
                      int32_t dtype, void* stream);
diff --git a/segmentation_training_pipeline_amd/_lib.py b/segmentation_training_pipeline_amd/_lib.py
--- a/segmentation_training_pipeline_amd/_lib.py
+++ b/segmentation_training_pipeline_amd/_lib.py
@@ -36,7 +36,9 @@
                 ("N", i32), ("Hs0", i32), ("Ws0", i32), ("Hv", i32), ("Wv", i32), ("C0", i32), ("C1", i32),
                 ("src0_mode", i32), ("KH", i32), ("KW", i32), ("stride", i32), ("pad", i32),
                 ("Ho", i32), ("Wo", i32), ("Cout", i32), ("accumulate", i32), ("dtype", i32), ("splits", i32),
-                ("src_bn_mean", vp), ("src_bn_rstd", vp), ("src_bn_gamma", vp), ("src_bn_beta", vp), ("src_bn_relu", i32)]
+                ("src_bn_mean", vp), ("src_bn_rstd", vp), ("src_bn_gamma", vp), ("src_bn_beta", vp), ("src_bn_relu", i32),
+                ("dyb_x", vp), ("dyb_mean", vp), ("dyb_rstd", vp), ("dyb_gamma", vp), ("dyb_beta", vp), ("dyb_sums", vp),
+                ("dyb_inv_rows", f32), ("dyb_relu", i32), ("dyb_keep", vp)]
 
 
 SIGNATURES = {
@@ -82,6 +84,7 @@
     "stp_wgrad_sc_eligible": (i32, [C.POINTER(WgradParams)]),
     "stp_wgrad_sc_slabs": (i32, [C.POINTER(WgradParams)]),
     "stp_wgrad_sc_partial": (i32, [C.POINTER(WgradParams), vp, vp]),
+    "stp_wgrad_stem_dxb_ok": (i32, [C.POINTER(WgradParams)]),
     "stp_conv2d_wgrad_kernel_id": (i32, [C.POINTER(WgradParams)]),
     "stp_wgrad_group_class": (i32, [C.POINTER(WgradParams)]),
     "stp_wgrad_group_table_bytes": (sz, [vp, i32]),
@@ -101,6 +104,7 @@
     "stp_bn_apply": (i32, [vp, i32, vp, i32, i64, i32, i32, vp, vp, vp, vp, i32, f32, vp]),
     "stp_bn_inference": (i32, [vp, i32, vp, i32, i64, i32, i32, vp, vp, f32, vp, vp, i32, f32, vp]),
     "stp_bn_backward": (i32, [vp, vp, vp, i32, i64, i32, vp, vp, vp, vp, vp, vp, i32, i32, vp, sz, vp]),
+    "stp_bn_backward_sums": (vp, [vp, i32]),
     "stp_bn_apply_slots": (i32, [vp, vp, i32, i64, i32, vp, i32, f32, f32, vp, vp, vp, vp, vp, vp, i32, vp]),
     "stp_bn_backward_slots": (i32, [vp, vp, vp, i32, i64, i32, vp, vp, vp, vp, i32, vp, vp, i32, vp]),
     "stp_zero_bytes": (i32, [vp, i64, vp]),
diff --git a/segmentation_training_pipeline_amd/csrc/bn.hip b/segmentation_training_pipeline_amd/csrc/bn.hip
--- a/segmentation_training_pipeline_amd/csrc/bn.hip
+++ b/segmentation_training_pipeline_amd/csrc/bn.hip
@@ -632,7 +632,7 @@
                                float* dbeta, int32_t relu, int32_t accumulate_dx, void* workspace, size_t workspace_bytes,
                                void* stream) {
   if (!stp_dtype_ok(dtype)) return STP_E_BADARG;
-  if (!x || !dy || !dx || !mean || !rstd || !workspace || rows <= 0 || C <= 0 || (C & 3)) return STP_E_BADARG;
+  if (!x || !dy || !mean || !rstd || !workspace || rows <= 0 || C <= 0 || (C & 3) || (!dx && accumulate_dx)) return STP_E_BADARG;
   if (workspace_bytes < stp_bn_workspace_bytes(C)) return STP_E_WORKSPACE;
   hipStream_t s = (hipStream_t)stream;
   const int blocks = bn_blocks(rows) > BN_MAX_BLOCKS - 1 ? BN_MAX_BLOCKS - 1 : bn_blocks(rows);
@@ -646,7 +646,13 @@
   if (rc) return rc;
   hipLaunchKernelGGL(bn_bwd_finalize_kernel, dim3(ceil_div(C, 4)), dim3(256), 0, s, partial, blocks, C, sums, dgamma, dbeta);
   STP_LAUNCH_CHECK();
+  if (!dx) return STP_OK;
   return bn_bwd_apply_launch(x, dy, dx, dtype, rows, C, mean, rstd, gamma, beta, sums, relu, accumulate_dx, nullptr, 0, nullptr, nullptr, nullptr, s);
+}
+
+extern "C" const float* stp_bn_backward_sums(const void* workspace, int32_t C) {
+  if (!workspace || C <= 0) return nullptr;
+  return (const float*)workspace + (size_t)(BN_MAX_BLOCKS - 1) * 2 * C;
 }
 
 #define BNF_SLAB 64
diff --git a/segmentation_training_pipeline_amd/csrc/conv_sc.h b/segmentation_training_pipeline_amd/csrc/conv_sc.h
--- a/segmentation_training_pipeline_amd/csrc/conv_sc.h
+++ b/segmentation_training_pipeline_amd/csrc/conv_sc.h
@@ -112,7 +112,14 @@
 int stem_lean_launch(const StemArgs& a, hipStream_t s);
 bool stem_wg_lean_serves(int N, int H, int W, int Ho, int Wo);
 int stem_wg_lean_blocks(int N, int Ho, int Wo);
-int stem_wg_lean_launch(const void* src, const void* dy, float* slabs, int N, int H, int W, int Ho, int Wo, hipStream_t s);
+struct StemWgDxb {
+  const void* x;
+  const float *mean, *rstd, *gamma, *beta, *sums;
+  float inv_rows;
+  int relu;
+  float* keep;
+};
+int stem_wg_lean_launch(const void* src, const void* dy, float* slabs, int N, int H, int W, int Ho, int Wo, const StemWgDxb* dxb, hipStream_t s);
 
 int sc_lean_launch(const ScArgs& a, int cin, int dtype, hipStream_t s);
 int sc_wg_lean_launch(const ScWgArgs& a, int cin, int cout, int dtype, int blocks, hipStream_t s);
diff --git a/segmentation_training_pipeline_amd/csrc/conv_sc_lean.hip b/segmentation_training_pipeline_amd/csrc/conv_sc_lean.hip
--- a/segmentation_training_pipeline_amd/csrc/conv_sc_lean.hip
+++ b/segmentation_training_pipeline_amd/csrc/conv_sc_lean.hip
@@ -874,7 +874,8 @@
 constexpr int SWG_TH = 4, SWG_PH = 2 * (SWG_TH - 1) + 7;
 constexpr int SWG_NVX = SWG_PH * STL_VPR, SWG_NPX = (SWG_NVX + 255) / 256;
 constexpr int SWG_NVD = SWG_TH * SC_TW * 8, SWG_NPD = (SWG_NVD + 255) / 256;
-constexpr int SWG_XBUF = SWG_NPX * 4096, SWG_BUF = SWG_XBUF + SWG_NPD * 4096;
+constexpr int SWG_XBUF = SWG_NPX * 4096, SWG_DBUF = SWG_NPD * 4096, SWG_BUF = SWG_XBUF + SWG_DBUF;
+constexpr int SWG_BUF_DXB = SWG_BUF + SWG_DBUF;
 
 struct StemWgArgs {
   const char* src;
@@ -882,10 +883,29 @@
   float* slabs;
   int N, H, W, Ho, Wo, tiles_x, tiles_y, ntiles;
   uint32_t src_bytes, dy_bytes;
+  const char* bx;
+  const float *mean, *rstd, *gamma, *beta, *sums;
+  float inv_rows;
+  int relu;
+  float* keep;
 };
 
-__global__ __launch_bounds__(256, 2) void conv_stem_wgrad_lean_kernel(const StemWgArgs a) {
+template <int ACT>
+__device__ __forceinline__ f32x2 bn_bwd_dx_pair(f32x2 x, f32x2 g, f32x2 mu, f32x2 rs, f32x2 sc, f32x2 sh, f32x2 k1, f32x2 k2) {
+  if constexpr (ACT != 0) {
+    const f32x2 t = __builtin_elementwise_fma(x, sc, sh);
+    g.x = (t.x > 0.f && (ACT == 1 || t.x < 6.f)) ? g.x : 0.f;
+    g.y = (t.y > 0.f && (ACT == 1 || t.y < 6.f)) ? g.y : 0.f;
+  }
+  const f32x2 xh = (x - mu) * rs;
+  const f32x2 d = g - k1;
+  return sc * __builtin_elementwise_fma(-xh, k2, d);
+}
+
+template <bool DXB>
+__device__ __forceinline__ void conv_stem_wgrad_lean_body(const StemWgArgs& a) {
   constexpr int COUT = 64, K = 224, NF = 14;
+  constexpr int SWG_BUF = DXB ? SWG_BUF_DXB : ::SWG_BUF;
   extern __shared__ __attribute__((aligned(16))) char smem[];
   const int tid = threadIdx.x, lane = tid & 63;
   const int wave = __builtin_amdgcn_readfirstlane(tid >> 6);
@@ -906,6 +926,7 @@
   if (t_first < t_end) {
     const __amdgpu_buffer_rsrc_t rsx = __builtin_amdgcn_make_buffer_rsrc((void*)a.src, 0, a.src_bytes, 0x00020000);
     const __amdgpu_buffer_rsrc_t rsd = __builtin_amdgcn_make_buffer_rsrc((void*)a.dy, 0, a.dy_bytes, 0x00020000);
+    const __amdgpu_buffer_rsrc_t rsb = __builtin_amdgcn_make_buffer_rsrc((void*)(DXB ? a.bx : a.dy), 0, a.dy_bytes, 0x00020000);
     int hyx[SWG_NPX], pyx[SWG_NPD];
     uint32_t lox[SWG_NPX], lod[SWG_NPD];
 #pragma unroll
@@ -930,7 +951,8 @@
       t.interior = 2 * t.y0 >= 3 && 2 * t.x0 >= 4 && 2 * t.y0 - 3 + SWG_PH <= a.H && 2 * t.x0 + 65 < a.W && t.y0 + SWG_TH <= a.Ho && t.x0 + SC_TW <= a.Wo;
       return t;
     };
-    auto issue_tile = [&](const TileC& t, int bsel, bool live) {
+    auto issue_tile = [&](const TileC& t, int bsel, bool live) -> uint32_t {
+      uint32_t inside = 0;
       char* xb = smem + bsel * SWG_BUF;
       if (live && t.interior) {
         const uint32_t tbx = (uint32_t)(((t.n * a.H + 2 * t.y0 - 3) * a.W + 2 * t.x0 - 4) * 8);
@@ -941,6 +963,12 @@
 #pragma unroll
         for (int p = 0; p < SWG_NPD; ++p)
           __builtin_amdgcn_raw_ptr_buffer_load_lds(rsd, (__attribute__((address_space(3))) void*)(xb + SWG_XBUF + p * 4096 + wave * 1024), 16, (int)(tbd + lod[p]), 0, 0, 0);
+        if constexpr (DXB) {
+#pragma unroll
+          for (int p = 0; p < SWG_NPD; ++p)
+            __builtin_amdgcn_raw_ptr_buffer_load_lds(rsb, (__attribute__((address_space(3))) void*)(xb + SWG_XBUF + SWG_DBUF + p * 4096 + wave * 1024), 16, (int)(tbd + lod[p]), 0, 0, 0);
+        }
+        inside = (1u << SWG_NPD) - 1u;
       } else {
 #pragma unroll
         for (int p = 0; p < SWG_NPX; ++p) {
@@ -954,12 +982,31 @@
           const int gy = t.y0 + (pyx[p] >> 16), gx = t.x0 + (pyx[p] & 0xffff);
           const bool ok = live && pyx[p] >= 0 && gy < a.Ho && gx < a.Wo;
           const uint32_t off = ok ? (uint32_t)(((t.n * a.Ho + gy) * a.Wo + gx) * (COUT * 2)) + cvd : 0x80000000u;
+          inside |= ok ? (1u << p) : 0u;
           __builtin_amdgcn_raw_ptr_buffer_load_lds(rsd, (__attribute__((address_space(3))) void*)(xb + SWG_XBUF + p * 4096 + wave * 1024), 16, (int)off, 0, 0, 0);
-        }
-      }
+          if constexpr (DXB)
+            __builtin_amdgcn_raw_ptr_buffer_load_lds(rsb, (__attribute__((address_space(3))) void*)(xb + SWG_XBUF + SWG_DBUF + p * 4096 + wave * 1024), 16, (int)off, 0, 0, 0);
+        }
+      }
+      return inside;
     };
     TileC tc = decode(t_first);
-    issue_tile(tc, 0, true);
+    uint32_t inside_cur = issue_tile(tc, 0, true);
+    f32x2 bmu[4], brs[4], bsc[4], bsh[4], bk1[4], bk2[4];
+    if constexpr (DXB) {
+      const int c = (tid & 7) * 8;
+#pragma unroll
+      for (int e = 0; e < 8; ++e) {
+        const float m = a.mean[c + e], r = a.rstd[c + e];
+        const float ga = a.gamma ? a.gamma[c + e] : 1.f, be = a.beta ? a.beta[c + e] : 0.f;
+        const float k = a.gamma ? r * ga : r;
+        bmu[e >> 1][e & 1] = m; brs[e >> 1][e & 1] = r; bsc[e >> 1][e & 1] = k;
+        bsh[e >> 1][e & 1] = __builtin_fmaf(-m, k, be);
+        bk1[e >> 1][e & 1] = a.sums[c + e] * a.inv_rows;
+        bk2[e >> 1][e & 1] = a.sums[COUT + c + e] * a.inv_rows;
+        if (a.keep && blockIdx.x == 0 && tid < 8) { a.keep[c + e] = ga; a.keep[COUT + c + e] = be; }
+      }
+    }
     const int xl = lg * 4 + (lr >> 2), qd = lr & 3;
     uint32_t aA = (uint32_t)(uintptr_t)smem + (uint32_t)(SWG_XBUF + (xl * COUT + wave * 16) * 2 + qd * 8);
     uint32_t aB = (uint32_t)(uintptr_t)smem + (uint32_t)((2 * xl + 1 + qd) * 8);
@@ -968,11 +1015,35 @@
     for (int tile = t_first; tile < t_end; tile += t_step, cur ^= 1) {
       __builtin_amdgcn_s_waitcnt(0x0f70);
       asm volatile("" ::: "memory");
+      if constexpr (DXB) {
+        char* gt = smem + cur * SWG_BUF + SWG_XBUF + tid * 16;
+        u32x4 gv[SWG_NPD], xv[SWG_NPD];
+#pragma unroll
+        for (int p = 0; p < SWG_NPD; ++p) {
+          gv[p] = *reinterpret_cast<const u32x4*>(gt + p * 4096);
+          xv[p] = *reinterpret_cast<const u32x4*>(gt + SWG_DBUF + p * 4096);
+        }
+        auto transform = [&](auto act) __attribute__((always_inline)) {
+#pragma unroll
+          for (int p = 0; p < SWG_NPD; ++p) {
+            u32x4 o;
+#pragma unroll
+            for (int e = 0; e < 4; ++e) {
+              const f32x2 d = bn_bwd_dx_pair<decltype(act)::value>(scl_unpack(xv[p][e]), scl_unpack(gv[p][e]), bmu[e], brs[e], bsc[e], bsh[e], bk1[e], bk2[e]);
+              o[e] = pack_bf16x2(d.x, d.y);
+            }
+            if (inside_cur & (1u << p)) *reinterpret_cast<u32x4*>(gt + p * 4096) = o;
+          }
+        };
+        if (a.relu == 0) transform(std::integral_constant<int, 0>{});
+        else if (a.relu == 1) transform(std::integral_constant<int, 1>{});
+        else transform(std::integral_constant<int, 2>{});
+      }
       lds_barrier();
       const int next = tile + t_step;
       const bool live = next < t_end;
       if (live) tc = decode(next);
-      issue_tile(tc, cur ^ 1, live);
+      inside_cur = issue_tile(tc, cur ^ 1, live);
 
       u32x2 fa[SWG_TH][2];
       u32x2 fb[2][2][2];
@@ -1021,6 +1092,9 @@
     for (int r = 0; r < 4; ++r) out[(size_t)(wave * 16 + lg * 4 + r) * K + (f >> 1) * 32 + (f & 1) * 16 + lr] = acc[f][r];
 }
 
+__global__ __launch_bounds__(256, 2) void conv_stem_wgrad_lean_kernel(const StemWgArgs a) { conv_stem_wgrad_lean_body<false>(a); }
+__global__ __launch_bounds__(256, 2) void conv_stem_wgrad_dxb_lean_kernel(const StemWgArgs a) { conv_stem_wgrad_lean_body<true>(a); }
+
 bool stem_wg_lean_serves(int N, int H, int W, int Ho, int Wo) {
   static const bool on = !(getenv("STP_STEM_WG_LEAN") && atoi(getenv("STP_STEM_WG_LEAN")) == 0);
   return on && !(W & 1) && (uint64_t)N * H * W * 8 < 0x80000000ull && (uint64_t)N * Ho * Wo * 128 < 0x80000000ull;
@@ -1029,12 +1103,19 @@
   const int64_t tiles = (int64_t)N * ((Ho + SWG_TH - 1) / SWG_TH) * ((Wo + SC_TW - 1) / SC_TW), b = (int64_t)stp_cu_count() * 2;
   return (int)(b < tiles ? b : tiles);
 }
-int stem_wg_lean_launch(const void* src, const void* dy, float* slabs, int N, int H, int W, int Ho, int Wo, hipStream_t s) {
+int stem_wg_lean_launch(const void* src, const void* dy, float* slabs, int N, int H, int W, int Ho, int Wo, const StemWgDxb* dxb, hipStream_t s) {
   StemWgArgs a;
   a.src = (const char*)src; a.dy = (const char*)dy; a.slabs = slabs;
   a.N = N; a.H = H; a.W = W; a.Ho = Ho; a.Wo = Wo;
   a.tiles_x = (Wo + SC_TW - 1) / SC_TW; a.tiles_y = (Ho + SWG_TH - 1) / SWG_TH; a.ntiles = N * a.tiles_x * a.tiles_y;
   a.src_bytes = (uint32_t)((uint64_t)N * H * W * 8); a.dy_bytes = (uint32_t)((uint64_t)N * Ho * Wo * 128);
+  a.bx = nullptr; a.mean = a.rstd = a.gamma = a.beta = a.sums = nullptr; a.inv_rows = 0.f; a.relu = 0; a.keep = nullptr;
+  if (dxb) {
+    if (!dxb->x || !dxb->mean || !dxb->rstd || !dxb->sums) return STP_E_BADARG;
+    a.bx = (const char*)dxb->x; a.mean = dxb->mean; a.rstd = dxb->rstd; a.gamma = dxb->gamma; a.beta = dxb->beta; a.sums = dxb->sums;
+    a.inv_rows = dxb->inv_rows; a.relu = dxb->relu; a.keep = dxb->keep;
+    return stp_launch_lds(conv_stem_wgrad_dxb_lean_kernel, dim3(stem_wg_lean_blocks(N, Ho, Wo)), dim3(256), 2 * SWG_BUF_DXB, s, a);
+  }
   hipLaunchKernelGGL(conv_stem_wgrad_lean_kernel, dim3(stem_wg_lean_blocks(N, Ho, Wo)), dim3(256), 2 * SWG_BUF, s, a);
   STP_LAUNCH_CHECK();
   return STP_OK;
diff --git a/segmentation_training_pipeline_amd/csrc/conv_sc_wgrad.hip b/segmentation_training_pipeline_amd/csrc/conv_sc_wgrad.hip
--- a/segmentation_training_pipeline_amd/csrc/conv_sc_wgrad.hip
+++ b/segmentation_training_pipeline_amd/csrc/conv_sc_wgrad.hip
@@ -315,9 +315,12 @@
          !p->src_bn_mean && stem_wg_lean_serves(p->N, p->Hv, p->Wv, p->Ho, p->Wo);
 }
 
+extern "C" int stp_wgrad_stem_dxb_ok(const stp_wgrad_params* p) { return p && stp_dtype_ok(p->dtype) && wgrad_stem_shape(p) ? 1 : 0; }
+
 extern "C" int stp_wgrad_sc_eligible(const stp_wgrad_params* p) {
   if (!p || !stp_dtype_ok(p->dtype)) return 0;
   if (wgrad_stem_shape(p)) return 1;
+  if (p->dyb_x) return 0;
   const int vec = p->dtype == STP_H16 ? 8 : 4;
   const bool c0ok = p->C0 == 16 || p->C0 == 32 || (p->C0 == 64 && vec == 8);
   const bool c1ok = p->C1 == 0 || p->C1 == 16 || p->C1 == 32 || (p->C1 == 64 && vec == 8);
@@ -392,7 +395,10 @@
 
 extern "C" int stp_wgrad_sc_partial(const stp_wgrad_params* p, void* workspace, void* stream) {
   if (!stp_wgrad_sc_eligible(p) || !p->src0 || !p->dy || !workspace || (p->C1 > 0 && !p->src1)) return STP_E_BADARG;
-  if (wgrad_stem_shape(p)) return stem_wg_lean_launch(p->src0, p->dy, (float*)workspace, p->N, p->Hv, p->Wv, p->Ho, p->Wo, (hipStream_t)stream);
+  if (wgrad_stem_shape(p)) {
+    const StemWgDxb dxb = {p->dyb_x, p->dyb_mean, p->dyb_rstd, p->dyb_gamma, p->dyb_beta, p->dyb_sums, p->dyb_inv_rows, p->dyb_relu, p->dyb_keep};
+    return stem_wg_lean_launch(p->src0, p->dy, (float*)workspace, p->N, p->Hv, p->Wv, p->Ho, p->Wo, p->dyb_x ? &dxb : nullptr, (hipStream_t)stream);
+  }
   ScWgArgs a;
   a.dy = (const char*)p->dy; a.slabs = (float*)workspace;
   a.N = p->N; a.H = p->Hv; a.W = p->Wv; a.Cout = p->Cout;
diff --git a/segmentation_training_pipeline_amd/csrc/conv_wgrad.hip b/segmentation_training_pipeline_amd/csrc/conv_wgrad.hip
--- a/segmentation_training_pipeline_amd/csrc/conv_wgrad.hip
+++ b/segmentation_training_pipeline_amd/csrc/conv_wgrad.hip
@@ -1313,6 +1313,7 @@
 extern "C" int stp_wgrad_sc_eligible(const stp_wgrad_params* p);
 extern "C" int stp_wgrad_sc_slabs(const stp_wgrad_params* p);
 extern "C" int stp_wgrad_sc_partial(const stp_wgrad_params* p, void* workspace, void* stream);
+extern "C" int stp_wgrad_stem_dxb_ok(const stp_wgrad_params* p);
 #define WG_TILE_SC 100
 
 static WgradPlan plan_wgrad(const stp_wgrad_params* p) {
@@ -1531,7 +1532,7 @@
 }
 
 static int wg_group_bm(const stp_wgrad_params* p) {
-  if (!p || !wgrad_row_eligible(p) || p->splits != 0) return 0;
+  if (!p || !wgrad_row_eligible(p) || p->splits != 0 || p->dyb_x) return 0;
   const int64_t lim = 1ll << 31;
   const int64_t P = (int64_t)p->N * p->Ho * p->Wo;
   if ((int64_t)p->N * p->Hs0 * p->Ws0 * p->C0 * 2 >= lim || (int64_t)p->N * p->Hv * p->Wv * p->C1 * 2 >= lim || P * p->Cout * 2 >= lim) return 0;
@@ -1770,6 +1771,7 @@
 
 extern "C" int stp_conv2d_wgrad_partial(const stp_wgrad_params* p, void* workspace, size_t workspace_bytes, int32_t variant,
                                         void* stream) {
+  if (p && p->dyb_x && !(variant == 0 && p->splits == 0 && stp_wgrad_stem_dxb_ok(p))) return STP_E_BADARG;
   if (p && variant == 0 && p->splits == 0 && stp_wgrad_sc_eligible(p)) {
     if (!workspace || stp_conv2d_wgrad_workspace_bytes(p) > workspace_bytes) return STP_E_WORKSPACE;
     return stp_wgrad_sc_partial(p, workspace, stream);
diff --git a/segmentation_training_pipeline_amd/graph.py b/segmentation_training_pipeline_amd/graph.py
--- a/segmentation_training_pipeline_amd/graph.py
+++ b/segmentation_training_pipeline_amd/graph.py
@@ -94,6 +94,7 @@
         self.fuse_bn_backward = os.environ.get("STP_FUSE_BN_BACKWARD", "1") != "0"
         self.fuse_bn_backward_last = os.environ.get("STP_FUSE_BN_BACKWARD_LAST", "1") != "0"
         self.fold_upsample_grad = os.environ.get("STP_FOLD_UPSAMPLE_GRAD", "1") != "0"
+        self.stem_dxb = os.environ.get("STP_STEM_DXB", "1") != "0"
         self.wgrad_group_gflop = float(os.environ.get("STP_WGRAD_GROUP_GFLOP", "300"))
         self.wgrad_lone_group_gflop = float(os.environ.get("STP_WGRAD_LONE_GROUP_GFLOP", "600"))
         self.reduce_batch = int(os.environ.get("STP_WGRAD_REDUCE_BATCH", "0"))
@@ -340,6 +341,14 @@
             rc = fn(*args, torch.cuda.current_stream().cuda_stream)
             if rc != 0:
                 raise _lib.StpError("%s failed with %d" % (rec[2], rc))
+        rec = t.meta.get("deferred_grad")
+        if rec is not None:
+            if t.grad is None:
+                t.grad = self._alloc((t.N, t.H, t.W, t.gradC))
+            fn, args = rec[0], rec[1]
+            rc = fn(*args[:2], t.grad.data_ptr(), *args[3:], torch.cuda.current_stream().cuda_stream)
+            if rc != 0:
+                raise _lib.StpError("%s failed with %d" % (rec[2], rc))
         return t
 
     def _scratch(self, nbytes):
@@ -519,6 +528,19 @@
             if (x.needs_grad and x.grad_ready and x.grad is not None and x.grad.data_ptr() in self._wgroup_reads and bslots is None
                     and out.meta.get("bnb") is not None):
                 dadd, x.grad = x.grad, None
+            if (self.stem_dxb and x.meta.get("stem_dxb") and x.meta.get("uses", 0) == 1 and not x.grad_ready and bslots is None
+                    and out.meta.get("bnb") is None and dadd is None):
+                ws = self._alloc((int(self.lib.stp_bn_workspace_bytes(Cn)) // 4,), torch.float32)
+                args = (x.buf.data_ptr(), out.grad.data_ptr(), None, self.cdt, x.rows, Cn, mean.data_ptr(), rstd.data_ptr(), gp, self._pptr(beta),
+                        self._gptr(gamma) if gamma else None, self._gptr(beta), int(relu), 0, ws.data_ptr(), ws.numel() * 4)
+                self._emit(self.bwd, "stp_bn_backward", *args)
+                keep = self._alloc((2 * Cn,), torch.float32)
+                x.meta["dxb"] = (out.grad, mean.data_ptr(), rstd.data_ptr(), gp, self._pptr(beta), int(relu),
+                                 int(self.lib.stp_bn_backward_sums(ws.data_ptr(), Cn)), 1.0 / x.rows, keep.data_ptr())
+                x.meta["deferred_grad"] = (self.lib.stp_bn_backward, args[:8] + (keep.data_ptr() if gp else None, keep.data_ptr() + 4 * Cn, None, None)
+                                           + args[12:], "stp_bn_backward")
+                x.grad_ready = True
+                return
             dx = self._gradbuf(x) if x.needs_grad else self._alloc((x.N, x.H, x.W, Cn))
             if bslots is not None:
                 self._emit(self.bwd, "stp_bn_backward_slots", x.buf.data_ptr(), out.grad.data_ptr(), dx.data_ptr(), self.cdt, x.rows, Cn,
@@ -1417,6 +1439,9 @@
             self.flops = float(flops_as)
         pl._emit_conv(pl.fwd, p, {"layer": self.name, "pass": "fwd", "flops": self.flops, "tile": int(pl.lib.stp_conv2d_tile_for(C.byref(p))),
                                   "src2": bool(self.C1 or self.upsample)})
+        if (pl.training and pl.stem_dxb and self.stem and self.w.trainable and self.b is None and not self.relu and residual is None
+                and src1 is None and self.CoutB == Cout and pl.lib.stp_wgrad_stem_dxb_ok(C.byref(self.wp))):
+            out.meta["stem_dxb"] = True
 
     def _weight_copies(self):
         pl, w, Cout, k, KWp, Cinp, Cin_master, param_cols = self.plan, self.w, self.Cout, self.k, self.KWp, self.Cinp, self.Cin_master, self.param_cols
@@ -1461,7 +1486,8 @@
         pl, out, residual, b = self.plan, self.out, self.residual, self.b
         if not out.needs_grad or not out.grad_ready:
             return
-        dy = self.dy = out.grad
+        dxb = out.meta.get("dxb")
+        dy = self.dy = out.grad if dxb is None else dxb[0]
         if self.relu:
             pl._guard_write(dy)
             pl._emit(pl.bwd, "stp_relu_bwd", out.buf.data_ptr(), dy.data_ptr(), out.rows * out.gradC, pl.cdt)
@@ -1494,6 +1520,10 @@
         else:
             wp.dw = pl._gptr(w)
         wp.src0, wp.src1, wp.dy = x.meta.get("src_override") or x.buf.data_ptr(), (src1.buf.data_ptr() if src1 is not None else None), self.dy.data_ptr()
+        dxb = self.out.meta.get("dxb")
+        if dxb is not None:
+            wp.dyb_x = self.out.buf.data_ptr()
+            wp.dyb_mean, wp.dyb_rstd, wp.dyb_gamma, wp.dyb_beta, wp.dyb_relu, wp.dyb_sums, wp.dyb_inv_rows, wp.dyb_keep = dxb[1:]
         cls = int(pl.lib.stp_wgrad_group_class(C.byref(wp))) if (pl.wgrad_group_gflop > 0 and not padded and gcols is None) else 0
         if cls:
             self._wgrad_join_group(cls)
diff --git a/segmentation_training_pipeline_amd/ops.py b/segmentation_training_pipeline_amd/ops.py
--- a/segmentation_training_pipeline_amd/ops.py
+++ b/segmentation_training_pipeline_amd/ops.py
@@ -143,6 +143,20 @@
     _lib.call("stp_bn_backward", ptr(x), ptr(dy), ptr(dx), dt(x), rows, Cn, ptr(mean), ptr(rstd), ptr(gamma), ptr(beta),
               ptr(dgamma), ptr(dbeta), int(relu), int(accumulate_dx), ptr(workspace),
               workspace.numel() * workspace.element_size(), stream())
+
+
+def bn_backward_sums(workspace, Cn):
+    return int(_lib.load().stp_bn_backward_sums(ptr(workspace), int(Cn)) or 0)
+
+
+def wgrad_stem_dxb_ok(p):
+    return bool(_lib.load().stp_wgrad_stem_dxb_ok(C.byref(p)))
+
+
+def wgrad_set_dxb(p, x, mean, rstd, gamma, beta, sums, inv_rows, relu, keep=None):
+    p.dyb_x, p.dyb_mean, p.dyb_rstd, p.dyb_gamma, p.dyb_beta = ptr(x), ptr(mean), ptr(rstd), ptr(gamma), ptr(beta)
+    p.dyb_sums, p.dyb_inv_rows, p.dyb_relu, p.dyb_keep = int(sums), float(inv_rows), int(relu), ptr(keep)
+    return p
 
 
 def bn_backward_fused(x, g, dx, rows, Cn, mean, rstd, gamma, partial, tiles, dgamma, dbeta, accumulate_dx, workspace):
```

Result: no change. 2575 images/sec, median of 6 (+0.7%).
